# NVlabs/WarpConvNet

Measured on AMD Instinct MI355X. Metric: M active voxels/sec fwd+bwd, SparseConv3d 64→128 k=3, 1/2/4/8 MI355X, higher is better.
Workload: dtype bf16; 1 GPU; configs[1]: one 1000000-voxel uniform (U) scene per GPU, SparseConv3d 64->128 k=3, bf16 autocast, kernel-map build + AB fwd + ABt dgrad + AtB wgrad per step; voxels_per_gpu=1000000, coord_order=generator, parallelism=dp1 (scene-sharded, grad all-reduce)

## Files before the change

### include/wcn.h

```cpp
#ifndef WCN_H_
#define WCN_H_

#include <stddef.h>
#include <stdint.h>

#ifdef __cplusplus
extern "C" {
#endif

typedef void* wcn_stream_t;

enum wcn_status {
  WCN_SUCCESS = 0,
  WCN_ERROR_PROBLEM_NOT_SUPPORTED = -1,
  WCN_ERROR_KERNEL_INITIALIZATION = -2,
  WCN_ERROR_KERNEL_EXECUTION = -3,
  WCN_ERROR_UNSUPPORTED_CONFIG = -4,
  WCN_ERROR_INVALID_PARAMETERS = -5,
  WCN_ERROR_MIXED_INPUT_UNSUPPORTED = -6
};

enum wcn_dtype { WCN_F32 = 0, WCN_F16 = 1, WCN_BF16 = 2 };

enum wcn_kmap_flag {
  WCN_FLAG_TABLE_FULL = 1,
  WCN_FLAG_COORD_RANGE = 2,
  WCN_FLAG_PAIR_OVERFLOW = 4,
  WCN_FLAG_DUPLICATE_COORD = 8,
  WCN_FLAG_NEED_STRICT = 16,
  WCN_FLAG_ROW_OVERFLOW = 32
};

int wcn_abi_version(void);
const char* wcn_status_string(int status);

int wcn_hash_prepare(void* slots, int64_t capacity, wcn_stream_t stream);
int wcn_hash_insert(void* slots, int64_t capacity, const int32_t* coords, int64_t n, int32_t* status,
                    wcn_stream_t stream);
int wcn_hash_search(const void* slots, int64_t capacity, const int32_t* queries, int64_t m,
                    int32_t* results, wcn_stream_t stream);

int32_t wcn_kmap_row_pitch(int32_t num_offsets);
int32_t wcn_kmap_mask_words(int32_t num_offsets);
int64_t wcn_kmap_num_blocks(int64_t m);
size_t wcn_kmap_counts_bytes(int64_t m, int32_t num_offsets);

int wcn_kmap_probe(const void* slots, int64_t capacity, const int32_t* query, int64_t m,
                   const int32_t ksize[3], const int32_t stride[3], const int32_t dilation[3],
                   int32_t* nbr, uint32_t* mask, wcn_stream_t stream);
int wcn_batch_indexed_coords(const int32_t* coords, int64_t n, int32_t num_dims, const int32_t* offsets,
                             int32_t num_batches, int32_t* out, wcn_stream_t stream);

int wcn_morton_code(const int32_t* coords, int64_t n, int32_t num_dims, const int32_t* origin, const int32_t axis[3],
                    int64_t* codes, wcn_stream_t stream);

size_t wcn_kmap_binned_workspace(int64_t n, int64_t max_blocks);
int wcn_kmap_binned_supported(const int32_t ksize[3], const int32_t dilation[3]);
int wcn_kmap_compact_supported(int32_t num_offsets);
int wcn_kmap_build_binned(const int32_t* coords, int64_t n, const int32_t ksize[3], const int32_t dilation[3],
                          int64_t max_blocks, int32_t strict, int32_t compact, void* workspace, size_t workspace_bytes,
                          int32_t* nbr, uint32_t* mask, int32_t* status, wcn_stream_t stream);
int wcn_kmap_densify(const int32_t* nbr_compact, int64_t m, int32_t num_offsets, int32_t* nbr, wcn_stream_t stream);
size_t wcn_kmap_tally_sort_workspace(int64_t m);
int wcn_kmap_tally_sort(uint32_t* mask, int32_t* nbr, int64_t m, int32_t num_offsets, int32_t* counts, int32_t* offsets,
                        int32_t* status, int32_t* host_mirror, int32_t* perm, void* sort_workspace,
                        size_t sort_workspace_bytes, const int32_t* coords, void* binned_workspace, int64_t binned_n,
                        int64_t max_blocks, int32_t compact, int32_t* in_maps, int32_t* out_maps, int64_t pair_capacity,
                        wcn_stream_t stream);
int wcn_kmap_count(const uint32_t* mask, int64_t m, int32_t num_offsets, int32_t* counts, wcn_stream_t stream);
int wcn_kmap_scan(int32_t* counts, int64_t num_blocks, int32_t num_offsets, int32_t* offsets,
                  wcn_stream_t stream);
int wcn_kmap_scan_to_host(int32_t* counts, int64_t num_blocks, int32_t num_offsets, int32_t* offsets, const int32_t* status,
                          int32_t* host_mirror, wcn_stream_t stream);
int wcn_kmap_scatter(const int32_t* nbr, const uint32_t* mask, int64_t m, int32_t num_offsets,
                     const int32_t* counts, const int32_t* offsets, int32_t* in_maps, int32_t* out_maps, int64_t pair_capacity,
                     int32_t* status, int32_t compact, wcn_stream_t stream);
int wcn_kmap_cells_build(const int32_t* coords, int64_t n, int64_t max_blocks, void* workspace, size_t workspace_bytes,
                         uint32_t* scratch, int32_t* status, wcn_stream_t stream);
int wcn_cells_stride_supported(const int32_t stride[3]);
int64_t wcn_cells_stride_tiles(int64_t n);
int wcn_cells_stride_count(const void* cells_workspace, int64_t n, int64_t max_blocks, const int32_t* coords,
                           const int32_t stride[3], uint64_t* flags, int32_t* counts, int32_t num_batches,
                           int32_t* out_offsets, wcn_stream_t stream);
int wcn_cells_stride_emit(const void* cells_workspace, int64_t n, int64_t max_blocks, const int32_t* coords,
                          const int32_t stride[3], const uint64_t* flags, const int32_t* counts, int32_t* out_coords,
                          int32_t* first_rows, int32_t* nbr, uint32_t* mask, wcn_stream_t stream);
int wcn_kmap_probe_cells(const void* cells_workspace, int64_t n_in, int64_t max_blocks, const int32_t* query, int64_t m,
                         const int32_t ksize[3], const int32_t stride[3], const int32_t dilation[3], int32_t* nbr,
                         uint32_t* mask, wcn_stream_t stream);
int wcn_kmap_transpose(const int32_t* nbr, int64_t m, int32_t num_offsets, int32_t* pair_table,
                       wcn_stream_t stream);
int wcn_kmap_reverse(const int32_t* in_maps, const int32_t* out_maps, const int32_t* offsets,
                     int32_t num_offsets, int64_t max_pairs, int64_t n_in, int32_t* rev_nbr,
                     uint32_t* rev_mask, wcn_stream_t stream);
int wcn_kmap_from_csr(const int32_t* in_maps, const int32_t* out_maps, const int32_t* offsets,
                      int32_t num_offsets, int64_t max_pairs, int64_t n_out, int32_t* nbr, uint32_t* mask,
                      wcn_stream_t stream);
size_t wcn_mask_argsort_workspace(int64_t n);
int wcn_mask_argsort(const uint32_t* mask, int32_t mask_words, int32_t num_bits, int64_t n, int32_t* perm,
                     void* workspace, size_t workspace_bytes, wcn_stream_t stream);
int wcn_mask_tile_order(const uint32_t* mask, int32_t mask_words, int32_t num_offsets, int64_t n, int32_t* perm,
                        void* workspace, size_t workspace_bytes, wcn_stream_t stream);

enum wcn_algo { WCN_ALGO_AUTO = 0, WCN_ALGO_REF = 1, WCN_ALGO_MFMA = 2 };

int wcn_mfma_gather_supported(int32_t cin, int32_t cout, int32_t num_offsets, int32_t dtype);
int wcn_mfma_wgrad_supported(int32_t cin, int32_t cout, int32_t dtype);
int wcn_conv_identity_supported(int32_t cin, int32_t cout, int32_t dtype);
int wcn_dense_rows_supported(int32_t cin, int32_t cout, int32_t dtype);
int wcn_dense_rows(const void* x, int32_t x_is_f32, const void* w, int32_t w_is_f32, int32_t w_transposed, const float* bias,
                   void* y, int64_t n, int32_t cin, int32_t cout, int32_t dtype, wcn_stream_t stream);

size_t wcn_packed_weight_bytes(int32_t num_offsets, int32_t cin, int32_t cout, int32_t dtype, int32_t transpose);
int wcn_pack_weight(const void* w, int32_t num_offsets, int32_t cin, int32_t cout, int32_t dtype,
                    int32_t transpose, int32_t flip, void* packed, size_t packed_bytes, wcn_stream_t stream);
int wcn_pack_weight_f32(const float* w, int32_t num_offsets, int32_t cin, int32_t cout, int32_t dtype, int32_t transpose,
                        int32_t flip, void* packed, size_t packed_bytes, wcn_stream_t stream);
int wcn_pack_weight_pair_supported(int32_t num_offsets, int32_t cin, int32_t cout, int32_t dtype);
int wcn_pack_weight_f32_pair(const float* w, int32_t num_offsets, int32_t cin, int32_t cout, int32_t dtype, int32_t flip_dgrad,
                             void* packed_fwd, size_t packed_fwd_bytes, void* packed_dgrad, size_t packed_dgrad_bytes,
                             wcn_stream_t stream);

int wcn_conv_compact_table_supported(int32_t cin, int32_t cout, int32_t num_offsets, int32_t dtype);
int wcn_conv_gather_gemm(const void* in, const void* w, void* out, const int32_t* nbr,
                         const uint32_t* mask, const int32_t* perm, const float* bias, int64_t n_in,
                         int64_t n_out, int32_t cin, int32_t cout, int32_t num_offsets, int32_t dtype,
                         int32_t algo, int32_t w_transposed, int32_t k_flip, wcn_stream_t stream);

int wcn_mfma_grouped_supported(int32_t cin_g, int32_t cout_g, int32_t num_offsets, int32_t dtype);
int wcn_pack_weight_grouped(const void* w, int32_t w_is_f32, int32_t num_offsets, int32_t groups, int32_t cin_g,
                            int32_t cout_g, int32_t dtype, int32_t transpose, int32_t flip, void* packed, wcn_stream_t stream);
int wcn_conv_gather_gemm_grouped(const void* in, const void* w_packed, void* out, const int32_t* nbr, const uint32_t* mask,
                                 const int32_t* perm, const float* bias, int64_t n_in, int64_t n_out, int32_t cin_g,
                                 int32_t cout_g, int32_t groups, int32_t num_offsets, int32_t dtype, wcn_stream_t stream);
int wcn_conv_gather_gemm_f32out(const void* in, const void* w_packed, float* out, const int32_t* nbr,
                                const uint32_t* mask, const int32_t* perm, const float* bias, int64_t n_in,
                                int64_t n_out, int32_t cin, int32_t cout, int32_t num_offsets, int32_t dtype,
                                wcn_stream_t stream);

int wcn_conv_gather_gemm_fused(const void* in, const void* w_packed, void* out, const int32_t* nbr, const uint32_t* mask,
                               const int32_t* perm, const float* bias, const float* scale, const float* shift,
                               const void* residual, int32_t relu, int64_t n_in, int64_t n_out, int32_t cin, int32_t cout,
                               int32_t num_offsets, int32_t dtype, wcn_stream_t stream);

size_t wcn_colsum_workspace(int32_t channels);
int wcn_colsum(const void* in, int64_t n, int32_t channels, int32_t dtype, float* out, void* workspace,
               size_t workspace_bytes, wcn_stream_t stream);

size_t wcn_conv_wgrad_workspace(int32_t num_offsets, int32_t cin, int32_t cout, int32_t algo);
int wcn_conv_wgrad(const void* x, const void* dy, float* dw, const int32_t* in_maps,
                   const int32_t* out_maps, const int32_t* offsets, int64_t n_in, int64_t n_out,
                   int32_t cin, int32_t cout, int32_t num_offsets, int32_t dtype, int32_t algo,
                   void* workspace, size_t workspace_bytes, wcn_stream_t stream);

int wcn_mfma_wgrad_bias_supported(int32_t cin, int32_t cout, int32_t dtype);
int wcn_conv_wgrad_bias(const void* x, const void* dy, float* dw, const int32_t* in_maps, const int32_t* out_maps,
                        const int32_t* offsets, int64_t n_in, int64_t n_out, int32_t cin, int32_t cout,
                        int32_t num_offsets, int32_t dtype, int32_t self_offset, float* bias_grad, void* workspace,
                        size_t workspace_bytes, wcn_stream_t stream);

int wcn_dwconv_gather(const void* in, const void* w, void* out, const int32_t* nbr, const float* bias, int64_t n_in,
                      int64_t n_out, int32_t channels, int32_t num_offsets, int32_t dtype, int32_t k_flip,
                      wcn_stream_t stream);
size_t wcn_dwconv_wgrad_workspace(int32_t num_offsets, int32_t channels);
int wcn_dwconv_wgrad(const void* x, const void* dy, float* dw, const int32_t* in_maps, const int32_t* out_maps,
                     const int32_t* offsets, int64_t n_in, int64_t n_out, int32_t channels, int32_t num_offsets,
                     int32_t dtype, void* workspace, size_t workspace_bytes, wcn_stream_t stream);

int wcn_knn_grid(const float* ref_sorted, const int32_t* ref_ids, const int32_t* cell_start, const float origin[3],
                 float cell_size, const int32_t dims[3], const float* query, int64_t num_query, int32_t k,
                 int64_t* out_index, float* out_dist2, wcn_stream_t stream);
int wcn_radius_grid_count(const float* ref_sorted, const int32_t* ref_ids, const int32_t* cell_start, const float origin[3],
                          float cell_size, const int32_t dims[3], const float* query, int64_t num_query, float radius,
                          int32_t* counts, wcn_stream_t stream);
int wcn_radius_grid_write(const float* ref_sorted, const int32_t* ref_ids, const int32_t* cell_start, const float origin[3],
                          float cell_size, const int32_t dims[3], const float* query, int64_t num_query, float radius,
                          const int64_t* splits, int32_t* out_index, float* out_dist, wcn_stream_t stream);
int wcn_segment_reduce(const void* in, const int64_t* row_splits, int64_t num_segments, int32_t channels, int32_t dtype,
                       int32_t op, void* out, int64_t* arg_rows, wcn_stream_t stream);

int wcn_pointconv_supported(int32_t cin, int32_t cq, int32_t nrel, int32_t hidden, int32_t cout, int32_t k,
                            int32_t linear_shortcut);
int64_t wcn_pointconv_packed_floats(int32_t ein, int32_t hidden, int32_t cout);
int64_t wcn_pointconv_grad_floats(int32_t ein, int32_t hidden, int32_t cout, int32_t linear_shortcut);
size_t wcn_pointconv_backward_workspace(int64_t n_query, int32_t k, int32_t ein, int32_t hidden, int32_t cout,
                                        int32_t linear_shortcut);
int wcn_pointconv_pack(const float* w1, const float* b1, const float* g1, const float* be1, const float* w2,
                       const float* b2, const float* g2, const float* be2, const float* ws, const float* bs, int32_t ein,
                       int32_t hidden, int32_t cout, float* packed, wcn_stream_t stream);
int wcn_pointconv_edge_forward(const float* in_feats, const float* q_feats, const float* in_xyz, const float* q_xyz,
                               const int32_t* nbr, int64_t n_query, int32_t k, int32_t cin, int32_t cq, int32_t nrel,
                               const float* packed, int32_t hidden, int32_t cout, float eps1, float eps2, int32_t mean,
                               int32_t linear_shortcut, float* out, wcn_stream_t stream);
int wcn_pointconv_edge_backward(const float* in_feats, const float* q_feats, const float* in_xyz, const float* q_xyz,
                                const int32_t* nbr, int64_t n_query, int32_t k, int32_t cin, int32_t cq, int32_t nrel,
                                const float* packed, int32_t hidden, int32_t cout, float eps1, float eps2, int32_t mean,
                                int32_t linear_shortcut, const float* grad_out, float* d_in, float* d_q, float* d_params,
                                void* workspace, size_t workspace_bytes, wcn_stream_t stream);
int wcn_pointconv_edge_backward_peredge(const float* in_feats, const float* q_feats, const float* in_xyz, const float* q_xyz,
                                        const int32_t* nbr, int64_t n_query, int32_t k, int32_t cin, int32_t cq, int32_t nrel,
                                        const float* packed, int32_t hidden, int32_t cout, float eps1, float eps2, int32_t mean,
                                        int32_t linear_shortcut, const float* grad_out, float* d_edge, float* d_q,
                                        float* d_params, void* workspace, size_t workspace_bytes, wcn_stream_t stream);

int wcn_pointconv_edge_forward_ragged(const float* in_feats, const float* q_feats, const float* in_xyz, const float* q_xyz,
                                      const int32_t* nbr, const int32_t* edge_q, const float* q_scale, int64_t n_edges,
                                      int64_t n_query, int32_t cin, int32_t cq, int32_t nrel, const float* packed,
                                      int32_t hidden, int32_t cout, float eps1, float eps2, int32_t linear_shortcut,
                                      float* out, wcn_stream_t stream);
int wcn_pointconv_edge_backward_ragged(const float* in_feats, const float* q_feats, const float* in_xyz, const float* q_xyz,
                                       const int32_t* nbr, const int32_t* edge_q, const float* q_scale, int64_t n_edges,
                                       int64_t n_query, int32_t cin, int32_t cq, int32_t nrel, const float* packed,
                                       int32_t hidden, int32_t cout, float eps1, float eps2, int32_t linear_shortcut,
                                       const float* grad_out, float* d_in, float* d_q, float* d_params, void* workspace,
                                       size_t workspace_bytes, wcn_stream_t stream);

int wcn_pool_gather(const void* in, const int32_t* tbl, int64_t n_in, int64_t n_out, int32_t channels, int32_t num_offsets,
                    int32_t dtype, int32_t op, void* out, int32_t* arg, int32_t* count, wcn_stream_t stream);
int wcn_pool_gather_scaled(const void* in, const int32_t* tbl, const float* scale, int64_t n_in, int64_t n_out,
                           int32_t channels, int32_t num_offsets, int32_t dtype, int32_t op, void* out, int32_t* arg,
                           int32_t* count, wcn_stream_t stream);
int wcn_pool_row_vec(const void* src, const void* dst, int32_t channels, int32_t dtype);
int wcn_pool_select(const void* dy, const int32_t* arg, const int32_t* tbl, int64_t n_in, int64_t n_out, int32_t channels,
                    int32_t num_offsets, int32_t dtype, void* dx, wcn_stream_t stream);

size_t wcn_bn_workspace(int32_t channels);
int32_t wcn_bn_max_channels(void);
int wcn_bn_stats_fold(const void* x, int64_t n, int32_t channels, int32_t dtype, const float* gamma, const float* beta,
                      float* running_mean, float* running_var, float momentum, float eps, float* mean, float* var,
                      float* rstd, float* scale, float* shift, int64_t* num_batches_tracked, void* workspace,
                      size_t workspace_bytes, wcn_stream_t stream);
int wcn_bn_fold(const float* running_mean, const float* running_var, const float* gamma, const float* beta, float eps,
                int32_t channels, float* mean, float* rstd, float* scale, float* shift, wcn_stream_t stream);
int wcn_bn_stats(const void* x, int64_t n, int32_t channels, int32_t dtype, float* mean, float* var, void* workspace,
                 size_t workspace_bytes, wcn_stream_t stream);
int wcn_bn_apply(const void* x, int64_t n, int32_t channels, int32_t dtype, const float* scale, const float* shift,
                 int32_t relu, void* y, wcn_stream_t stream);
int wcn_bn_backward_reduce(const void* dy, const void* x, const float* relu_scale, const float* relu_shift, int64_t n,
                           int32_t channels, int32_t dtype, const float* mean, const float* rstd, float* sum_dy,
                           float* sum_dy_xhat, void* workspace, size_t workspace_bytes, wcn_stream_t stream);
int wcn_bn_backward_apply(const void* dy, const void* x, const float* relu_scale, const float* relu_shift, int64_t n,
                          int32_t channels, int32_t dtype, const float* mean, const float* rstd, const float* gamma,
                          const float* sum_dy, const float* sum_dy_xhat, void* dx, wcn_stream_t stream);
int wcn_bn_apply_residual(const void* x, const void* residual, int64_t n, int32_t channels, int32_t dtype, const float* scale,
                          const float* shift, int32_t relu, void* y, wcn_stream_t stream);
int wcn_bn_backward_reduce_masked(const void* dy, const void* x, const void* z, int64_t n, int32_t channels, int32_t dtype,
                                  const float* mean, const float* rstd, float* sum_dy, float* sum_dy_xhat, void* workspace,
                                  size_t workspace_bytes, wcn_stream_t stream);
int wcn_bn_backward_apply_masked(const void* dy, const void* x, const void* z, int64_t n, int32_t channels, int32_t dtype,
                                 const float* mean, const float* rstd, const float* gamma, const float* sum_dy,
                                 const float* sum_dy_xhat, void* dx, void* dres, wcn_stream_t stream);

int wcn_bn_train_forward(const void* x, const void* residual, int64_t n, int32_t channels, int32_t dtype, const float* gamma,
                         const float* beta, float* running_mean, float* running_var, float momentum, float eps,
                         int64_t* num_batches_tracked, int32_t relu, float* stats, void* y, void* workspace,
                         size_t workspace_bytes, wcn_stream_t stream);
int wcn_bn_train_backward(const void* dy, const void* x, const void* z, int32_t relu, int64_t n, int32_t channels, int32_t dtype,
                          const float* stats, const float* gamma, int32_t training, float* sums, void* dx, void* dres,
                          void* workspace, size_t workspace_bytes, wcn_stream_t stream);
int wcn_bn_train_backward_ld(const void* dy, int64_t dy_ld, const void* x, const void* z, int32_t relu, int64_t n, int32_t channels,
                             int32_t dtype, const float* stats, const float* gamma, int32_t training, float* sums, void* dx,
                             void* dres, void* workspace, size_t workspace_bytes, wcn_stream_t stream);

int wcn_conv_bn_backward(const void* grad_out, const void* x, const void* y, const void* z, int32_t relu, const float* stats,
                         const float* gamma, int32_t training, float* sums, void* dy_conv, void* dres, const void* w_packed_dgrad,
                         const int32_t* rev_nbr, const uint32_t* rev_mask, const int32_t* rev_perm, int32_t flip, void* dx,
                         const int32_t* in_maps, const int32_t* out_maps, const int32_t* offsets, float* dw, void* wgrad_workspace,
                         size_t wgrad_workspace_bytes, int64_t n_in, int64_t n_out, int32_t cin, int32_t cout, int32_t num_offsets,
                         int32_t dtype, void* bn_workspace, size_t bn_workspace_bytes, wcn_stream_t stream);
int wcn_conv_bn_backward_ld(const void* grad_out, int64_t grad_out_ld, const void* x, const void* y, const void* z, int32_t relu,
                            const float* stats, const float* gamma, int32_t training, float* sums, void* dy_conv, void* dres,
                            const void* w_packed_dgrad, const int32_t* rev_nbr, const uint32_t* rev_mask, const int32_t* rev_perm,
                            int32_t flip, void* dx, const int32_t* in_maps, const int32_t* out_maps, const int32_t* offsets,
                            float* dw, void* wgrad_workspace, size_t wgrad_workspace_bytes, int64_t n_in, int64_t n_out,
                            int32_t cin, int32_t cout, int32_t num_offsets, int32_t dtype, void* bn_workspace,
                            size_t bn_workspace_bytes, wcn_stream_t stream);

int wcn_attn_varlen_supported(int32_t head_dim, int32_t dtype);
size_t wcn_attn_varlen_workspace_bytes(int64_t total, int32_t heads);
int wcn_attn_varlen_fwd(const void* qkv, const int32_t* cu_seqlens, int64_t num_seqs, int64_t total, int32_t heads,
                        int32_t head_dim, int32_t max_seqlen, float softmax_scale, int32_t dtype, void* out, float* lse,
                        wcn_stream_t stream);
int wcn_attn_varlen_bwd(const void* dout, const void* qkv, const void* out, const float* lse, const int32_t* cu_seqlens,
                        int64_t num_seqs, int64_t total, int32_t heads, int32_t head_dim, int32_t max_seqlen,
                        float softmax_scale, int32_t dtype, void* dqkv, void* workspace, size_t workspace_bytes,
                        wcn_stream_t stream);

int32_t wcn_attn_varlen_kv_splits(int64_t num_seqs, int32_t max_seqlen_q, int32_t max_seqlen_k, int32_t heads);
size_t wcn_attn_varlen_kv_workspace_bytes(int64_t total_q, int64_t total_k, int32_t heads, int32_t head_dim, int32_t q_splits);
int wcn_attn_varlen_kv_fwd(const void* q, int64_t q_stride, const void* k, const void* v, int64_t kv_stride,
                           const int32_t* cu_q, const int32_t* cu_k, int64_t num_seqs, int64_t total_q, int64_t total_k,
                           int32_t heads, int32_t head_dim, int32_t max_seqlen_q, int32_t max_seqlen_k, float softmax_scale,
                           int32_t dtype, void* out, float* lse, wcn_stream_t stream);
int wcn_attn_varlen_kv_bwd(const void* dout, const void* q, int64_t q_stride, const void* k, const void* v, int64_t kv_stride,
                           const void* out, const float* lse, const int32_t* cu_q, const int32_t* cu_k, int64_t num_seqs,
                           int64_t total_q, int64_t total_k, int32_t heads, int32_t head_dim, int32_t max_seqlen_q,
                           int32_t max_seqlen_k, float softmax_scale, int32_t dtype, void* dq, int64_t dq_stride, void* dk,
                           void* dv, int64_t dkv_stride, int32_t q_splits, void* workspace, size_t workspace_bytes,
                           wcn_stream_t stream);

enum wcn_slot_order { WCN_SLOT_X_FASTEST = 0, WCN_SLOT_Z_FASTEST = 1 };
int wcn_resample_pack(const void* src, const int32_t* tbl, int64_t n_src, int64_t n_parent, int32_t channels, int32_t n_per,
                      int32_t factor, int32_t pitch, int32_t slot_order, int32_t dtype, void* dst, wcn_stream_t stream);
int wcn_resample_unpack(const void* src, const int32_t* tbl, int64_t n_parent, int64_t n_dst, int32_t channels, int32_t n_per,
                        int32_t factor, int32_t pitch, int32_t slot_order, int32_t broadcast, int32_t dtype, void* dst,
                        wcn_stream_t stream);
size_t wcn_resample_expand_workspace(int64_t n_parent);
int wcn_resample_expand(const int32_t* parents, const void* mask, int32_t mask_dtype, int64_t n_parent, int32_t n_per,
                        int32_t factor, int32_t slot_order, int32_t num_batches, void* workspace, size_t workspace_bytes,
                        int32_t* out_offsets, int64_t capacity, int32_t* child_coords, int32_t* tbl, int32_t pitch,
                        wcn_stream_t stream);

int wcn_rope_table(const void* coords, int32_t coords_float, int64_t total, const float* origin, float bias,
                   const float* freqs, int32_t num_freqs, float* table, wcn_stream_t stream);
int wcn_qk_prologue_supported(int32_t head_dim, int32_t in_dtype, int32_t out_dtype);
size_t wcn_qk_prologue_workspace_bytes(int64_t total, int32_t heads, int32_t head_dim);
int wcn_qk_prologue_fwd(const void* qkv, int32_t in_dtype, int64_t total, int32_t heads, int32_t head_dim, const float* table,
                        int32_t rot_pairs, int32_t conjugate, const float* gamma_q, const float* gamma_k, void* out,
                        int32_t out_dtype, float* inv_norm, wcn_stream_t stream);
int wcn_qk_prologue_bwd(const void* dout, int32_t dout_dtype, const void* qkv, int32_t in_dtype, int64_t total, int32_t heads,
                        int32_t head_dim, const float* table, int32_t rot_pairs, const float* gamma_q, const float* gamma_k,
                        const float* inv_norm, void* dqkv, float* dgamma_q, float* dgamma_k, void* workspace,
                        size_t workspace_bytes, wcn_stream_t stream);

int wcn_adaln_supported(int32_t channels, int32_t dtype);
size_t wcn_adaln_workspace_bytes(int64_t rows, int64_t num_segs, int32_t channels);
int wcn_adaln_fwd(const void* x, const void* h, const float* gate, const float* shift, const float* scale, int64_t mod_ld,
                  const int32_t* cu, int64_t num_segs, int64_t rows, int32_t channels, float eps, int32_t dtype, void* x1,
                  void* y, float* stats, wcn_stream_t stream);
int wcn_adaln_bwd(const void* dx1, const void* dy, const void* x, const void* h, const float* gate, const float* scale,
                  int64_t mod_ld, const float* stats, const int32_t* cu, int64_t num_segs, int64_t rows, int32_t channels,
                  int32_t dtype, void* dx, void* dh, float* dgate, float* dshift, float* dscale, int64_t dmod_ld,
                  void* workspace, size_t workspace_bytes, wcn_stream_t stream);

int wcn_ln_act_supported(int32_t channels, int32_t dtype);
size_t wcn_ln_act_workspace_bytes(int64_t rows, int32_t channels);
int wcn_ln_act_fwd(const void* x, const float* weight, const float* bias, int64_t rows, int32_t channels, float eps,
                   int32_t act, int32_t dtype, void* y, float* stats, wcn_stream_t stream);
int wcn_ln_act_bwd(const void* dy, const void* x, const float* weight, const float* bias, const float* stats, int64_t rows,
                   int32_t channels, int32_t act, int32_t dtype, void* dx, float* dweight, float* dbias, void* workspace,
                   size_t workspace_bytes, wcn_stream_t stream);
int wcn_channel_spread(const void* x, const void* h, int64_t rows, int32_t cx, int32_t r, float alpha, int32_t dtype,
                       void* out, wcn_stream_t stream);
int wcn_channel_fold(const void* x, const void* h, int64_t rows, int32_t cout, int32_t g, float alpha, int32_t dtype,
                     void* out, wcn_stream_t stream);

int32_t wcn_window_group_max_segment(void);
size_t wcn_window_group_workspace_bytes(int64_t n, int64_t num_bins);
int wcn_window_group(const int32_t* coords, int64_t n, const int32_t* batch_offsets, int32_t num_batches,
                     const int32_t window[3], const int32_t shift[3], const int32_t min_coord[3], const int32_t grid_shape[3],
                     int64_t* codes, int64_t* perm, int64_t* inverse_perm, int32_t* cu_seqlens, int64_t* counts,
                     int32_t* summary, void* workspace, size_t workspace_bytes, wcn_stream_t stream);

int32_t wcn_csr_chunk_rows(void);
int wcn_voxel_keys(const float* points, int64_t n, const int32_t* batch_offsets, int32_t num_batches, float inv_voxel_size,
                   int64_t* keys, int32_t* status, wcn_stream_t stream);
size_t wcn_voxel_map_workspace_bytes(int64_t n);
int wcn_voxel_map(const int64_t* sorted_keys, const int64_t* perm, int64_t n, int32_t num_batches, int64_t* unique_keys,
                  int32_t* unique_coords, int64_t* csr_offsets, int64_t* to_orig, int64_t* to_unique,
// ... 171 lines not shown
```

### warpconvnet_amd/_lib.py

```python
import ctypes
import os
import subprocess
import threading
from ctypes import c_char_p, c_int, c_int32, c_int64, c_size_t, c_void_p
from typing import Optional

import torch

_CSRC = os.path.join(os.path.dirname(os.path.abspath(__file__)), "csrc")
LIB_PATH = os.environ.get("WARPCONVNET_AMD_LIB") or os.path.join(_CSRC, "libwcn_hip.so")

WCN_F32, WCN_F16, WCN_BF16 = 0, 1, 2
WCN_ALGO_AUTO, WCN_ALGO_REF, WCN_ALGO_MFMA = 0, 1, 2
WCN_FLAG_TABLE_FULL, WCN_FLAG_COORD_RANGE, WCN_FLAG_PAIR_OVERFLOW, WCN_FLAG_DUPLICATE_COORD = 1, 2, 4, 8
WCN_FLAG_NEED_STRICT = 16
WCN_FLAG_ROW_OVERFLOW = 32
WCN_SLOT_X_FASTEST, WCN_SLOT_Z_FASTEST = 0, 1
WCN_MASK_U8 = 3
WCN_GRID_KEY_CELL, WCN_GRID_KEY_CORNER = 0, 1
WCN_SEG_MOMENTS, WCN_SEG_RANGE, WCN_SEG_DOT = 0, 1, 2
WCN_SEG_ADD, WCN_SEG_SUB, WCN_SEG_MUL, WCN_SEG_DIV, WCN_SEG_NORM, WCN_SEG_NORM_BWD = 0, 1, 2, 3, 4, 5
WCN_FPS_AUTO, WCN_FPS_RESIDENT, WCN_FPS_STREAMED = 0, 1, 2
WCN_ATTN_AUTO, WCN_ATTN_ONE_WAVE, WCN_ATTN_SHARED = 0, 1, 2

_I32P = c_void_p
_3I = c_int32 * 3
_EC_LISTS = [c_void_p, c_int64, c_void_p, c_int64, c_void_p, c_void_p, c_int32, c_int64, c_int64, c_int64, c_int32]

SIGNATURES = {
    "wcn_abi_version": (c_int, []),
    "wcn_status_string": (c_char_p, [c_int]),
    "wcn_hash_prepare": (c_int, [c_void_p, c_int64, c_void_p]),
    "wcn_hash_insert": (c_int, [c_void_p, c_int64, c_void_p, c_int64, c_void_p, c_void_p]),
    "wcn_hash_search": (c_int, [c_void_p, c_int64, c_void_p, c_int64, c_void_p, c_void_p]),
    "wcn_kmap_row_pitch": (c_int32, [c_int32]),
    "wcn_kmap_mask_words": (c_int32, [c_int32]),
    "wcn_kmap_num_blocks": (c_int64, [c_int64]),
    "wcn_kmap_probe": (
        c_int,
        [c_void_p, c_int64, c_void_p, c_int64, _3I, _3I, _3I, c_void_p, c_void_p, c_void_p],
    ),
    "wcn_batch_indexed_coords": (c_int, [c_void_p, c_int64, c_int32, c_void_p, c_int32, c_void_p, c_void_p]),
    "wcn_bn_workspace": (c_size_t, [c_int32]),
    "wcn_bn_max_channels": (c_int32, []),
    "wcn_bn_stats": (c_int, [c_void_p, c_int64, c_int32, c_int32, c_void_p, c_void_p, c_void_p, c_size_t, c_void_p]),
    "wcn_bn_stats_fold": (c_int, [c_void_p, c_int64, c_int32, c_int32, c_void_p, c_void_p, c_void_p, c_void_p, ctypes.c_float,
                                  ctypes.c_float, c_void_p, c_void_p, c_void_p, c_void_p, c_void_p, c_void_p, c_void_p, c_size_t,
                                  c_void_p]),
    "wcn_bn_fold": (c_int, [c_void_p, c_void_p, c_void_p, c_void_p, ctypes.c_float, c_int32, c_void_p, c_void_p, c_void_p,
                            c_void_p, c_void_p]),
    "wcn_bn_apply": (c_int, [c_void_p, c_int64, c_int32, c_int32, c_void_p, c_void_p, c_int32, c_void_p, c_void_p]),
    "wcn_bn_backward_reduce": (c_int, [c_void_p, c_void_p, c_void_p, c_void_p, c_int64, c_int32, c_int32, c_void_p, c_void_p,
                                       c_void_p, c_void_p, c_void_p, c_size_t, c_void_p]),
    "wcn_bn_backward_apply": (c_int, [c_void_p, c_void_p, c_void_p, c_void_p, c_int64, c_int32, c_int32, c_void_p, c_void_p,
                                      c_void_p, c_void_p, c_void_p, c_void_p, c_void_p]),
    "wcn_bn_apply_residual": (c_int, [c_void_p, c_void_p, c_int64, c_int32, c_int32, c_void_p, c_void_p, c_int32, c_void_p,
                                      c_void_p]),
    "wcn_bn_backward_reduce_masked": (c_int, [c_void_p, c_void_p, c_void_p, c_int64, c_int32, c_int32, c_void_p, c_void_p,
                                              c_void_p, c_void_p, c_void_p, c_size_t, c_void_p]),
    "wcn_bn_backward_apply_masked": (c_int, [c_void_p, c_void_p, c_void_p, c_int64, c_int32, c_int32, c_void_p, c_void_p,
                                             c_void_p, c_void_p, c_void_p, c_void_p, c_void_p, c_void_p]),
    "wcn_bn_train_forward": (c_int, [c_void_p, c_void_p, c_int64, c_int32, c_int32, c_void_p, c_void_p, c_void_p, c_void_p,
                                     ctypes.c_float, ctypes.c_float, c_void_p, c_int32, c_void_p, c_void_p, c_void_p, c_size_t,
                                     c_void_p]),
    "wcn_bn_train_backward": (c_int, [c_void_p, c_void_p, c_void_p, c_int32, c_int64, c_int32, c_int32, c_void_p, c_void_p,
                                      c_int32, c_void_p, c_void_p, c_void_p, c_void_p, c_size_t, c_void_p]),
    "wcn_bn_train_backward_ld": (c_int, [c_void_p, c_int64, c_void_p, c_void_p, c_int32, c_int64, c_int32, c_int32, c_void_p, c_void_p,
                                         c_int32, c_void_p, c_void_p, c_void_p, c_void_p, c_size_t, c_void_p]),
    "wcn_conv_bn_backward_ld": (c_int, [c_void_p, c_int64, c_void_p, c_void_p, c_void_p, c_int32, c_void_p, c_void_p, c_int32, c_void_p,
                                        c_void_p, c_void_p, c_void_p, c_void_p, c_void_p, c_void_p, c_int32, c_void_p, c_void_p, c_void_p,
                                        c_void_p, c_void_p, c_void_p, c_size_t, c_int64, c_int64, c_int32, c_int32, c_int32, c_int32,
                                        c_void_p, c_size_t, c_void_p]),
    "wcn_conv_bn_backward": (c_int, [c_void_p, c_void_p, c_void_p, c_void_p, c_int32, c_void_p, c_void_p, c_int32, c_void_p, c_void_p,
                                     c_void_p, c_void_p, c_void_p, c_void_p, c_void_p, c_int32, c_void_p, c_void_p, c_void_p, c_void_p,
                                     c_void_p, c_void_p, c_size_t, c_int64, c_int64, c_int32, c_int32, c_int32, c_int32, c_void_p,
                                     c_size_t, c_void_p]),
    "wcn_pool_gather": (c_int, [c_void_p, c_void_p, c_int64, c_int64, c_int32, c_int32, c_int32, c_int32, c_void_p, c_void_p,
                                c_void_p, c_void_p]),
    "wcn_pool_gather_scaled": (c_int, [c_void_p, c_void_p, c_void_p, c_int64, c_int64, c_int32, c_int32, c_int32, c_int32, c_void_p,
                                       c_void_p, c_void_p, c_void_p]),
    "wcn_pool_row_vec": (c_int, [c_void_p, c_void_p, c_int32, c_int32]),
    "wcn_pool_select": (c_int, [c_void_p, c_void_p, c_void_p, c_int64, c_int64, c_int32, c_int32, c_int32, c_void_p, c_void_p]),
    "wcn_morton_code": (c_int, [c_void_p, c_int64, c_int32, c_void_p, c_void_p, c_void_p, c_void_p]),
    "wcn_kmap_counts_bytes": (c_size_t, [c_int64, c_int32]),
    "wcn_kmap_binned_workspace": (c_size_t, [c_int64, c_int64]),
    "wcn_kmap_binned_supported": (c_int, [_3I, _3I]),
    "wcn_kmap_build_binned": (
        c_int,
        [c_void_p, c_int64, _3I, _3I, c_int64, c_int32, c_int32, c_void_p, c_size_t, c_void_p, c_void_p, c_void_p, c_void_p],
    ),
    "wcn_kmap_compact_supported": (c_int, [c_int32]),
    "wcn_kmap_densify": (c_int, [c_void_p, c_int64, c_int32, c_void_p, c_void_p]),
    "wcn_kmap_tally_sort_workspace": (c_size_t, [c_int64]),
    "wcn_kmap_tally_sort": (
        c_int,
        [c_void_p, c_void_p, c_int64, c_int32, c_void_p, c_void_p, c_void_p, c_void_p, c_void_p, c_void_p, c_size_t,
         c_void_p, c_void_p, c_int64, c_int64, c_int32, c_void_p, c_void_p, c_int64, c_void_p],
    ),
    "wcn_kmap_count": (c_int, [c_void_p, c_int64, c_int32, c_void_p, c_void_p]),
    "wcn_kmap_scan": (c_int, [c_void_p, c_int64, c_int32, c_void_p, c_void_p]),
    "wcn_kmap_scan_to_host": (c_int, [c_void_p, c_int64, c_int32, c_void_p, c_void_p, c_void_p, c_void_p]),
    "wcn_kmap_scatter": (
        c_int,
        [c_void_p, c_void_p, c_int64, c_int32, c_void_p, c_void_p, c_void_p, c_void_p, c_int64, c_void_p, c_int32, c_void_p],
    ),
    "wcn_kmap_cells_build": (c_int, [c_void_p, c_int64, c_int64, c_void_p, c_size_t, c_void_p, c_void_p, c_void_p]),
    "wcn_cells_stride_supported": (c_int, [_3I]),
    "wcn_cells_stride_tiles": (c_int64, [c_int64]),
    "wcn_cells_stride_count": (c_int, [c_void_p, c_int64, c_int64, c_void_p, _3I, c_void_p, c_void_p, c_int32, c_void_p,
                                       c_void_p]),
    "wcn_cells_stride_emit": (c_int, [c_void_p, c_int64, c_int64, c_void_p, _3I, c_void_p, c_void_p, c_void_p, c_void_p,
                                      c_void_p, c_void_p, c_void_p]),
    "wcn_kmap_probe_cells": (c_int, [c_void_p, c_int64, c_int64, c_void_p, c_int64, _3I, _3I, _3I, c_void_p, c_void_p,
                                     c_void_p]),
    "wcn_kmap_transpose": (c_int, [c_void_p, c_int64, c_int32, c_void_p, c_void_p]),
    "wcn_kmap_reverse": (
        c_int,
        [c_void_p, c_void_p, c_void_p, c_int32, c_int64, c_int64, c_void_p, c_void_p, c_void_p],
    ),
    "wcn_kmap_from_csr": (
        c_int,
        [c_void_p, c_void_p, c_void_p, c_int32, c_int64, c_int64, c_void_p, c_void_p, c_void_p],
    ),
    "wcn_mask_argsort_workspace": (c_size_t, [c_int64]),
    "wcn_mask_argsort": (c_int, [c_void_p, c_int32, c_int32, c_int64, c_void_p, c_void_p, c_size_t, c_void_p]),
    "wcn_mask_tile_order": (c_int, [c_void_p, c_int32, c_int32, c_int64, c_void_p, c_void_p, c_size_t, c_void_p]),
    "wcn_mfma_gather_supported": (c_int, [c_int32, c_int32, c_int32, c_int32]),
    "wcn_mfma_wgrad_supported": (c_int, [c_int32, c_int32, c_int32]),
    "wcn_conv_identity_supported": (c_int, [c_int32, c_int32, c_int32]),
    "wcn_dense_rows_supported": (c_int, [c_int32, c_int32, c_int32]),
    "wcn_dense_rows": (
        c_int,
        [c_void_p, c_int32, c_void_p, c_int32, c_int32, c_void_p, c_void_p, c_int64, c_int32, c_int32, c_int32, c_void_p],
    ),
    "wcn_packed_weight_bytes": (c_size_t, [c_int32, c_int32, c_int32, c_int32, c_int32]),
    "wcn_pack_weight": (
        c_int,
        [c_void_p, c_int32, c_int32, c_int32, c_int32, c_int32, c_int32, c_void_p, c_size_t, c_void_p],
    ),
    "wcn_pack_weight_f32": (
        c_int,
        [c_void_p, c_int32, c_int32, c_int32, c_int32, c_int32, c_int32, c_void_p, c_size_t, c_void_p],
    ),
    "wcn_pack_weight_pair_supported": (c_int, [c_int32, c_int32, c_int32, c_int32]),
    "wcn_conv_compact_table_supported": (c_int, [c_int32, c_int32, c_int32, c_int32]),
    "wcn_pack_weight_f32_pair": (c_int, [c_void_p, c_int32, c_int32, c_int32, c_int32, c_int32, c_void_p, c_size_t, c_void_p, c_size_t,
                                         c_void_p]),
    "wcn_conv_gather_gemm": (
        c_int,
        [c_void_p, c_void_p, c_void_p, c_void_p, c_void_p, c_void_p, c_void_p, c_int64, c_int64, c_int32, c_int32,
         c_int32, c_int32, c_int32, c_int32, c_int32, c_void_p],
    ),
    "wcn_mfma_grouped_supported": (c_int, [c_int32, c_int32, c_int32, c_int32]),
    "wcn_pack_weight_grouped": (
        c_int,
        [c_void_p, c_int32, c_int32, c_int32, c_int32, c_int32, c_int32, c_int32, c_int32, c_void_p, c_void_p],
    ),
    "wcn_conv_gather_gemm_grouped": (
        c_int,
        [c_void_p, c_void_p, c_void_p, c_void_p, c_void_p, c_void_p, c_void_p, c_int64, c_int64, c_int32, c_int32,
         c_int32, c_int32, c_int32, c_void_p],
    ),
    "wcn_conv_gather_gemm_f32out": (
        c_int,
        [c_void_p, c_void_p, c_void_p, c_void_p, c_void_p, c_void_p, c_void_p, c_int64, c_int64, c_int32, c_int32,
         c_int32, c_int32, c_void_p],
    ),
# ... 102 lines not shown
    ),
    "wcn_attn_varlen_kv_bwd_v": (
        c_int,
        [c_void_p, c_void_p, c_int64, c_void_p, c_void_p, c_int64, c_void_p, c_void_p, c_void_p, c_void_p, c_int64, c_int64,
         c_int64, c_int32, c_int32, c_int32, c_int32, ctypes.c_float, c_int32, c_void_p, c_int64, c_void_p, c_void_p, c_int64,
         c_int32, c_void_p, c_size_t, c_int32, c_void_p],
    ),
    "wcn_attn_varlen_k_splits": (c_int32, [c_int64, c_int32, c_int32, c_int32, c_int32]),
    "wcn_attn_varlen_ksplit_workspace_bytes": (c_size_t, [c_int64, c_int64, c_int32, c_int32, c_int32, c_int32, c_int32]),
    "wcn_attn_varlen_kv_fwd_s": (
        c_int,
        [c_void_p, c_int64, c_void_p, c_void_p, c_int64, c_void_p, c_void_p, c_int64, c_int64, c_int64, c_int32, c_int32,
         c_int32, c_int32, ctypes.c_float, c_int32, c_void_p, c_void_p, c_int32, c_int32, c_void_p, c_size_t, c_void_p],
    ),
    "wcn_attn_varlen_kv_bwd_s": (
        c_int,
        [c_void_p, c_void_p, c_int64, c_void_p, c_void_p, c_int64, c_void_p, c_void_p, c_void_p, c_void_p, c_int64, c_int64,
         c_int64, c_int32, c_int32, c_int32, c_int32, ctypes.c_float, c_int32, c_void_p, c_int64, c_void_p, c_void_p, c_int64,
         c_int32, c_int32, c_void_p, c_size_t, c_int32, c_void_p],
    ),
    "wcn_rope_table": (c_int, [c_void_p, c_int32, c_int64, c_void_p, ctypes.c_float, c_void_p, c_int32, c_void_p, c_void_p]),
    "wcn_rope_table_axes": (c_int, [c_void_p, c_int32, c_int64, c_void_p, ctypes.c_float, c_void_p, _3I, c_void_p, c_void_p]),
    "wcn_qk_prologue_supported": (c_int, [c_int32, c_int32, c_int32]),
    "wcn_qk_prologue_workspace_bytes": (c_size_t, [c_int64, c_int32, c_int32]),
    "wcn_qk_prologue_fwd": (
        c_int,
        [c_void_p, c_int32, c_int64, c_int32, c_int32, c_void_p, c_int32, c_int32, c_void_p, c_void_p, c_void_p, c_int32,
         c_void_p, c_void_p],
    ),
    "wcn_qk_prologue_bwd": (
        c_int,
        [c_void_p, c_int32, c_void_p, c_int32, c_int64, c_int32, c_int32, c_void_p, c_int32, c_void_p, c_void_p, c_void_p,
         c_void_p, c_void_p, c_void_p, c_void_p, c_size_t, c_void_p],
    ),
    "wcn_adaln_supported": (c_int, [c_int32, c_int32]),
    "wcn_adaln_workspace_bytes": (c_size_t, [c_int64, c_int64, c_int32]),
    "wcn_adaln_fwd": (
        c_int,
        [c_void_p] * 5 + [c_int64, c_void_p, c_int64, c_int64, c_int32, ctypes.c_float, c_int32, c_void_p, c_void_p, c_void_p,
                          c_void_p],
    ),
    "wcn_adaln_bwd": (
        c_int,
        [c_void_p] * 6 + [c_int64, c_void_p, c_void_p, c_int64, c_int64, c_int32, c_int32] + [c_void_p] * 5 +
        [c_int64, c_void_p, c_size_t, c_void_p],
    ),
    "wcn_ln_act_supported": (c_int, [c_int32, c_int32]),
    "wcn_ln_act_workspace_bytes": (c_size_t, [c_int64, c_int32]),
    "wcn_ln_act_fwd": (c_int, [c_void_p] * 3 + [c_int64, c_int32, ctypes.c_float, c_int32, c_int32, c_void_p, c_void_p,
                                                 c_void_p]),
    "wcn_ln_act_bwd": (c_int, [c_void_p] * 5 + [c_int64, c_int32, c_int32, c_int32] + [c_void_p] * 4 + [c_size_t, c_void_p]),
    "wcn_channel_spread": (c_int, [c_void_p, c_void_p, c_int64, c_int32, c_int32, ctypes.c_float, c_int32, c_void_p,
                                   c_void_p]),
    "wcn_channel_fold": (c_int, [c_void_p, c_void_p, c_int64, c_int32, c_int32, ctypes.c_float, c_int32, c_void_p, c_void_p]),
    "wcn_window_group_max_segment": (c_int32, []),
    "wcn_window_group_workspace_bytes": (c_size_t, [c_int64, c_int64]),
    "wcn_window_group": (c_int, [c_void_p, c_int64, c_void_p, c_int32, _3I, _3I, _3I, _3I] + [c_void_p] * 7 +
                         [c_size_t, c_void_p]),
    "wcn_csr_chunk_rows": (c_int32, []),
    "wcn_voxel_keys": (c_int, [c_void_p, c_int64, c_void_p, c_int32, ctypes.c_float, c_void_p, c_void_p, c_void_p]),
    "wcn_voxel_map_workspace_bytes": (c_size_t, [c_int64]),
    "wcn_voxel_map": (c_int, [c_void_p, c_void_p, c_int64, c_int32] + [c_void_p] * 7 + [c_void_p, c_size_t, c_void_p]),
    "wcn_csr_gather_reduce_workspace_bytes": (c_size_t, [c_int64, c_int32, c_int32]),
    "wcn_csr_gather_reduce": (
        c_int,
        [c_void_p, c_int64, c_int64, c_void_p, c_void_p, c_int64, c_int64, c_int32, c_int32, c_int32, c_int64, c_void_p,
         c_void_p, c_void_p, c_size_t, c_void_p],
    ),
    "wcn_row_spread": (c_int, [c_void_p, c_void_p, c_int64, c_int64, c_int32, c_void_p, c_int32, c_int64, c_int32, c_void_p,
                               c_void_p, c_int32, c_void_p, c_void_p]),
    "wcn_resample_pack": (c_int, [c_void_p, c_void_p, c_int64, c_int64, c_int32, c_int32, c_int32, c_int32, c_int32, c_int32,
                                  c_void_p, c_void_p]),
    "wcn_resample_unpack": (c_int, [c_void_p, c_void_p, c_int64, c_int64, c_int32, c_int32, c_int32, c_int32, c_int32, c_int32,
                                    c_int32, c_void_p, c_void_p]),
    "wcn_resample_expand_workspace": (c_size_t, [c_int64]),
    "wcn_resample_expand": (c_int, [c_void_p, c_void_p, c_int32, c_int64, c_int32, c_int32, c_int32, c_int32, c_void_p, c_size_t,
                                    c_void_p, c_int64, c_void_p, c_void_p, c_int32, c_void_p]),
    "wcn_mfma_wgrad_bias_supported": (c_int, [c_int32, c_int32, c_int32]),
    "wcn_conv_wgrad_bias": (
        c_int,
        [c_void_p, c_void_p, c_void_p, c_void_p, c_void_p, c_void_p, c_int64, c_int64, c_int32, c_int32, c_int32,
         c_int32, c_int32, c_void_p, c_void_p, c_size_t, c_void_p],
    ),
    "wcn_lattice_chunk_rows": (c_int32, []),
    "wcn_hash128_insert": (c_int, [c_void_p, c_void_p, c_int64, c_void_p, c_int64, c_int32, c_void_p, c_void_p]),
    "wcn_hash128_search": (c_int, [c_void_p, c_void_p, c_int64, c_void_p, c_void_p, c_int64, c_int32, c_int32, c_void_p,
                                   c_void_p]),
    "wcn_permuto_simplex": (c_int, [c_void_p, c_int64, c_int32, ctypes.c_float * 6] + [c_void_p] * 6),
    "wcn_grid_corners": (c_int, [c_void_p, c_int64, c_int32] + [c_void_p] * 7),
    "wcn_lattice_map_workspace_bytes": (c_size_t, [c_int64]),
    "wcn_lattice_map": (c_int, [c_void_p, c_void_p, c_void_p, c_int64, c_int32] + [c_void_p] * 5 + [c_size_t, c_void_p]),
    "wcn_lattice_plan_items": (c_int64, [c_int64]),
    "wcn_lattice_plan_ints": (c_int64, [c_int64]),
    "wcn_lattice_plan": (c_int, [c_void_p, c_int64, c_int64, c_void_p, c_void_p]),
    "wcn_lattice_splat": (c_int, [c_void_p] * 4 + [c_int64, c_int64, c_int32, c_int32, ctypes.c_float] + [c_void_p] * 4),
    "wcn_lattice_blur": (c_int, [c_void_p] * 3 + [ctypes.c_float] * 3 + [c_int64, c_int32, c_void_p, c_void_p]),
    "wcn_lattice_slice": (c_int, [c_void_p] * 3 + [c_int64, c_int32, c_int64, c_int32, ctypes.c_float, c_void_p, c_void_p]),
    "wcn_lattice_max_grid": (c_int32, []),
    "wcn_lattice_row_grid": (c_int32, [c_int64, c_int32]),
    "wcn_bilateral_matvec": (c_int, [c_void_p, c_int32, c_int64, c_int32] + [ctypes.c_float] * 3 + [c_void_p, c_void_p,
                                                                                                   ctypes.c_float] + [c_void_p] * 5),
    "wcn_bilateral_pcg": (c_int, [c_void_p, c_int32, c_int64, c_int32] + [ctypes.c_float] * 3 + [c_void_p] * 3 + [ctypes.c_float] +
                          [c_void_p] * 5 + [c_int32, ctypes.c_double, c_void_p]),
    "wcn_bilateral_knn_weights": (c_int, [c_void_p] * 5 + [c_int64, c_int64, c_int32, c_int32, c_int32, ctypes.c_float,
                                                           ctypes.c_float, c_void_p, c_void_p]),
    "wcn_grid_max_grid": (c_int32, []),
    "wcn_grid_chunk_points": (c_int32, []),
    "wcn_grid_point_keys": (c_int, [c_void_p, c_int64, c_void_p, c_int32, _3I, ctypes.c_float * 3, ctypes.c_float * 3, c_int32,
                                    c_void_p, c_void_p, c_void_p]),
    "wcn_grid_sample": (c_int, [c_void_p, c_int64 * 5, _3I, c_int32, c_int32, c_int64, c_void_p, c_void_p, c_void_p, c_int64,
                                c_void_p, c_int64, c_int64, c_void_p]),
    "wcn_grid_sample_backward_workspace_bytes": (c_size_t, [c_int64, c_int32]),
    "wcn_grid_sample_backward": (c_int, [c_void_p, c_int64, c_int64, c_int64 * 5, _3I, c_int32, c_int32, c_int64, c_void_p,
                                         c_void_p, c_void_p, c_void_p, c_int64, c_int64, c_void_p, c_void_p, c_size_t,
                                         c_void_p]),
    "wcn_seg_chunk_rows": (c_int32, []),
    "wcn_seg_max_grid": (c_int32, []),
    "wcn_seg_stats_workspace_bytes": (c_size_t, [c_int64, c_int64, c_int32, c_int32]),
    "wcn_seg_stats": (c_int, [c_int32] + [c_void_p] * 4 + [c_int64, c_int64, c_int32, c_int32] + [c_void_p] * 5 +
                      [c_size_t, c_void_p]),
    "wcn_seg_apply": (c_int, [c_int32] + [c_void_p] * 3 + [c_int32] + [c_void_p] * 7 + [c_int64, c_int64, c_int32, c_int32,
                                                                                       c_void_p, c_void_p]),
    "wcn_fps_resident_max_points": (c_int64, []),
    "wcn_fps_block_threads": (c_int32, []),
    "wcn_fps_blocks_per_segment": (c_int32, []),
    "wcn_fps_max_grid": (c_int32, []),
    "wcn_fps_workspace_bytes": (c_size_t, [c_int64, c_int64, c_int32]),
    "wcn_fps": (c_int, [c_void_p, c_void_p, c_int64, c_void_p, c_int64, c_int64, c_int32, c_int64, c_void_p, c_int32, c_void_p,
                        c_size_t, c_void_p, c_void_p]),
    "wcn_fdg_supported": (c_int, [c_int32, c_int32]),
    "wcn_fdg_workspace": (c_size_t, [c_int64]),
    "wcn_fdg_count": (c_int, [c_void_p, c_int32, c_void_p, c_int64, c_void_p, c_int32, c_void_p, c_size_t, c_void_p, c_void_p]),
    "wcn_fdg_emit": (c_int, [c_void_p, c_int32, c_void_p, c_void_p, c_int64, c_void_p, c_int32, c_void_p, c_int32, c_void_p,
                             c_int32, ctypes.c_float, ctypes.c_float * 3, c_void_p, c_size_t, c_int64, c_void_p, c_void_p,
                             c_void_p, c_void_p]),
    "wcn_pad_max_grid": (c_int32, []),
    "wcn_pad_block_threads": (c_int32, []),
    "wcn_pad_repack": (c_int, [c_void_p, c_void_p, c_void_p, c_int64, c_void_p, c_int64, c_int64, c_void_p, c_int64, c_int64,
                               c_int64, c_int32, ctypes.c_uint64, c_void_p]),
    "wcn_seg_bmm_max_channels": (c_int32, []),
    "wcn_seg_bmm_tile_rows": (c_int32, []),
    "wcn_seg_bmm_chunk_rows": (c_int32, []),
    "wcn_seg_bmm_workspace_bytes": (c_size_t, [c_int64, c_int64, c_int32, c_int32, c_int32]),
    "wcn_seg_bmm": (c_int, [c_void_p, c_void_p, c_void_p, c_int64, c_int64, c_int32, c_int32, c_int32, c_int32, c_void_p,
                            c_void_p, c_size_t, c_void_p]),
    "wcn_seg_bmm_wgrad": (c_int, [c_void_p, c_void_p, c_void_p, c_int64, c_int64, c_int32, c_int32, c_int32, c_void_p,
                                  c_void_p, c_size_t, c_void_p]),
    "wcn_edgeconv_max_channels": (c_int32, []),
    "wcn_edgeconv_sum_blocks": (c_int32, []),
    "wcn_edgeconv_arg_bytes": (c_int32, [c_int64]),
    "wcn_edgeconv_sums_workspace_bytes": (c_size_t, [c_int32]),
    "wcn_edgeconv_backward_input_workspace_bytes": (c_size_t, [c_int64, c_int32]),
    "wcn_edgeconv_stats": (c_int, _EC_LISTS + [c_void_p, c_void_p, c_void_p, c_size_t, c_void_p]),
    "wcn_edgeconv_forward": (c_int, _EC_LISTS + [c_void_p, c_void_p, ctypes.c_float, c_void_p, c_void_p, c_int32, c_void_p]),
    "wcn_edgeconv_backward_sums": (c_int, _EC_LISTS + [c_void_p] * 4 + [ctypes.c_float, c_void_p, c_void_p, c_int32, c_void_p,
                                                                        c_void_p, c_void_p, c_size_t, c_void_p]),
    "wcn_edgeconv_backward_query": (c_int, _EC_LISTS + [c_void_p] * 6 + [ctypes.c_float, c_void_p, c_void_p, c_int32, c_void_p,
                                                                         c_void_p]),
    "wcn_edgeconv_backward_input": (c_int, _EC_LISTS + [c_void_p] * 3 + [c_void_p] * 6 +
                                    [ctypes.c_float, c_void_p, c_void_p, c_int32, c_void_p, c_void_p, c_size_t, c_void_p]),
}

_LIB = None


class _GuardedLib:

    def __init__(self, handle: ctypes.CDLL):
        self._h = handle

    def __getattr__(self, name):
        fn = getattr(self._h, name)
        argtypes = fn.argtypes or []
        if not argtypes or argtypes[-1] is not c_void_p or name in _HOST_ONLY or _single_gpu():
            setattr(self, name, fn)
            return fn

        def guarded(*args, _fn=fn):
            dev = getattr(_CALL_DEVICE, "dev", None)
            if dev is None or dev == torch.cuda.current_device():
                return _fn(*args)
            with torch.cuda.device(dev):
                return _fn(*args)

        guarded.__name__ = name
        setattr(self, name, guarded)
        return guarded


def _single_gpu() -> bool:
    try:
        return torch.cuda.is_available() and torch.cuda.device_count() == 1
    except Exception:
        return False


_HOST_ONLY = {"wcn_status_string"}
_CALL_DEVICE = threading.local()


def build(verbose: bool = False) -> str:
    cmd = ["make", "-C", _CSRC, "-j", str(min(8, os.cpu_count() or 1))]
    res = subprocess.run(cmd, capture_output=True, text=True)
    if res.returncode != 0:
        raise RuntimeError(f"building libwcn_hip.so failed:\n{res.stdout[-4000:]}\n{res.stderr[-4000:]}")
    if verbose:
        print(res.stdout[-2000:])
    return LIB_PATH


def lib() -> ctypes.CDLL:
    global _LIB
    if _LIB is None:
        if not os.path.exists(LIB_PATH):
            raise RuntimeError(
                f"{LIB_PATH} not found: the HIP extension is not built. Run "
                "`python -c 'import __graft_entry__ as g; g.build()'` (or `make -C warpconvnet_amd/csrc`). "
                "There is no CPU fallback for the HIP paths."
            )
        handle = ctypes.CDLL(LIB_PATH)
        for name, (restype, argtypes) in SIGNATURES.items():
            fn = getattr(handle, name)
            fn.restype = restype
            fn.argtypes = argtypes
        _LIB = _GuardedLib(handle)
    return _LIB


def status_string(code: int) -> str:
    return lib().wcn_status_string(int(code)).decode()


def check(code: int, what: str) -> None:
    if code != 0:
        raise RuntimeError(f"{what} error: {status_string(code)} ({code})")


def ptr(t: Optional[torch.Tensor]) -> Optional[int]:
    if t is None:
        return None
    return t.data_ptr()


_RAW_STREAM = getattr(torch._C, "_cuda_getCurrentRawStream", None)


def stream_handle(device: torch.device) -> int:
    idx = device.index
    if idx is None:
        idx = torch.cuda.current_device()
    _CALL_DEVICE.dev = idx
    if _RAW_STREAM is not None:
        return _RAW_STREAM(idx)
    return torch.cuda.current_stream(device).cuda_stream


def dtype_code(dtype: torch.dtype) -> int:
    if dtype == torch.float32:
        return WCN_F32
    if dtype == torch.float16:
        return WCN_F16
    if dtype == torch.bfloat16:
        return WCN_BF16
    raise TypeError(f"unsupported feature dtype {dtype} (supported: float32, float16, bfloat16)")


def torch_dtype(code: int) -> torch.dtype:
    return {WCN_F32: torch.float32, WCN_F16: torch.float16, WCN_BF16: torch.bfloat16}[code]


def i3(v) -> "ctypes.Array":
    return _3I(int(v[0]), int(v[1]), int(v[2]))


def require_gpu_tensor(t: torch.Tensor, name: str) -> None:
    if not t.is_cuda:
        raise RuntimeError(f"{name} must live on a GPU for the HIP path (got {t.device}); there is no CPU fallback")
    if not t.is_contiguous():
        raise RuntimeError(f"{name} must be contiguous")
```

### warpconvnet_amd/csrc/conv_api.hip

```cpp
#include "gather_gemm.h"

namespace wcn {
int conv_gather_gemm_ref(const void* in, const void* w, void* out, const int32_t* nbr, const float* bias, int64_t n_out,
                         int cin, int cout, int K, int dtype, int w_transposed, int k_flip, hipStream_t s);
size_t colsum_workspace(int c);
int colsum(const void* in, int64_t n, int c, int dtype, float* out, void* workspace, size_t workspace_bytes, hipStream_t s);
int conv_wgrad_ref(const void* x, const void* dy, float* dw, const int32_t* in_maps, const int32_t* out_maps,
                   const int32_t* offsets, int cin, int cout, int K, int dtype, hipStream_t s);
bool mfma_wgrad_supported(int cin, int cout, int dtype);
size_t wgrad_mfma_workspace(int K, int cin, int cout);
bool mfma_wgrad_bias_supported(int cin, int cout, int dtype);
int conv_wgrad_mfma(const void* x, const void* dy, float* dw, const int32_t* in_maps, const int32_t* out_maps,
                    const int32_t* offsets, int cin, int cout, int K, int dtype, void* workspace, size_t workspace_bytes,
                    int cs_k, float* bias_grad, int64_t pair_bound, hipStream_t s);
int dwconv_gather(const void* in, const void* w, void* out, const int32_t* tbl, const float* bias, int64_t n_out, int C,
                  int K, int dtype, int k_flip, hipStream_t s);
size_t dwconv_wgrad_workspace(int K, int C);
int dwconv_wgrad(const void* x, const void* dy, float* dw, const int32_t* in_maps, const int32_t* out_maps,
                 const int32_t* offsets, int C, int K, int dtype, void* workspace, size_t workspace_bytes, hipStream_t s);
int knn_grid(const float* ref, const int32_t* ref_id, const int32_t* cell_start, const float origin[3], float h,
             const int32_t dims[3], const float* query, int64_t m, int k, int64_t* out_idx, float* out_d2, hipStream_t s);
int radius_grid_count(const float* ref, const int32_t* ref_id, const int32_t* cell_start, const float origin[3], float h,
                      const int32_t dims[3], const float* query, int64_t m, float radius, int32_t* counts, hipStream_t s);
int radius_grid_write(const float* ref, const int32_t* ref_id, const int32_t* cell_start, const float origin[3], float h,
                      const int32_t dims[3], const float* query, int64_t m, float radius, const int64_t* splits,
                      int32_t* out_idx, float* out_dist, hipStream_t s);
int segment_reduce(const void* in, const int64_t* splits, int64_t m, int c, int dtype, int op, void* out, int64_t* arg,
                   hipStream_t s);
}

using namespace wcn;

static inline size_t dtype_size(int dtype) { return dtype == WCN_F32 ? 4 : 2; }

extern "C" {

int wcn_mfma_gather_supported(int32_t cin, int32_t cout, int32_t num_offsets, int32_t dtype) {
  return mfma_gather_supported(cin, cout, num_offsets, dtype) ? 1 : 0;
}
int wcn_conv_identity_supported(int32_t cin, int32_t cout, int32_t dtype) {
  return gather_gemm_cs_supported(cin, cout, 1, dtype) ? 1 : 0;
}
int wcn_mfma_wgrad_supported(int32_t cin, int32_t cout, int32_t dtype) {
  return mfma_wgrad_supported(cin, cout, dtype) ? 1 : 0;
}

size_t wcn_packed_weight_bytes(int32_t num_offsets, int32_t cin, int32_t cout, int32_t dtype, int32_t transpose) {
  (void)transpose;
  if (num_offsets < 1 || cin < 1 || cout < 1 || !dtype_ok(dtype)) return 0;
  return (size_t)num_offsets * ((cin + 63) / 64 * 64) * cout * dtype_size(dtype);
}

int wcn_pack_weight(const void* w, int32_t num_offsets, int32_t cin, int32_t cout, int32_t dtype, int32_t transpose,
                    int32_t flip, void* packed, size_t packed_bytes, wcn_stream_t stream) {
  if (!w || !packed || num_offsets < 1 || cin < 1 || cout < 1) return WCN_ERROR_INVALID_PARAMETERS;
  if (packed_bytes < wcn_packed_weight_bytes(num_offsets, cin, cout, dtype, transpose)) return WCN_ERROR_INVALID_PARAMETERS;
  return pack_weight_mfma(w, 0, num_offsets, cin, cout, dtype, transpose, flip, packed, (hipStream_t)stream);
}

int wcn_pack_weight_f32(const float* w, int32_t num_offsets, int32_t cin, int32_t cout, int32_t dtype, int32_t transpose,
                        int32_t flip, void* packed, size_t packed_bytes, wcn_stream_t stream) {
  if (!w || !packed || num_offsets < 1 || cin < 1 || cout < 1) return WCN_ERROR_INVALID_PARAMETERS;
  if (packed_bytes < wcn_packed_weight_bytes(num_offsets, cin, cout, dtype, transpose)) return WCN_ERROR_INVALID_PARAMETERS;
  return pack_weight_mfma(w, 1, num_offsets, cin, cout, dtype, transpose, flip, packed, (hipStream_t)stream);
}

static bool compact_table_ok(int cin, int cout, int K, int dtype) {
  return wcn_kmap_compact_supported(K) && gather_gemm_cs_supported(cin, cout, K, dtype);
}
int wcn_conv_compact_table_supported(int32_t cin, int32_t cout, int32_t num_offsets, int32_t dtype) {
  return compact_table_ok(cin, cout, num_offsets, dtype) ? 1 : 0;
}

int wcn_pack_weight_pair_supported(int32_t num_offsets, int32_t cin, int32_t cout, int32_t dtype) {
  return (gather_gemm_cs_supported(cin, cout, num_offsets, dtype) && gather_gemm_cs_supported(cout, cin, num_offsets, dtype)) ? 1 : 0;
}

int wcn_pack_weight_f32_pair(const float* w, int32_t num_offsets, int32_t cin, int32_t cout, int32_t dtype, int32_t flip_dgrad,
                             void* packed_fwd, size_t packed_fwd_bytes, void* packed_dgrad, size_t packed_dgrad_bytes,
                             wcn_stream_t stream) {
  if (!w || !packed_fwd || !packed_dgrad || num_offsets < 1 || cin < 1 || cout < 1) return WCN_ERROR_INVALID_PARAMETERS;
  if (!wcn_pack_weight_pair_supported(num_offsets, cin, cout, dtype)) return WCN_ERROR_UNSUPPORTED_CONFIG;
  if (packed_fwd_bytes < wcn_packed_weight_bytes(num_offsets, cin, cout, dtype, 0) ||
      packed_dgrad_bytes < wcn_packed_weight_bytes(num_offsets, cout, cin, dtype, 1))
    return WCN_ERROR_INVALID_PARAMETERS;
  return pack_weight_cs_pair(w, num_offsets, cin, cout, dtype, flip_dgrad, packed_fwd, packed_dgrad, (hipStream_t)stream);
}

int wcn_conv_gather_gemm(const void* in, const void* w, void* out, const int32_t* nbr, const uint32_t* mask,
                         const int32_t* perm, const float* bias, int64_t n_in, int64_t n_out, int32_t cin,
                         int32_t cout, int32_t num_offsets, int32_t dtype, int32_t algo, int32_t w_transposed,
                         int32_t k_flip, wcn_stream_t stream) {
  if (n_in < 0 || n_out < 0 || cin < 1 || cout < 1 || num_offsets < 1 || !dtype_ok(dtype))
    return WCN_ERROR_INVALID_PARAMETERS;
  if (n_out == 0) return WCN_SUCCESS;
  const bool identity = !nbr && !mask && !perm && num_offsets == 1 && algo == WCN_ALGO_MFMA && n_in == n_out &&
                        gather_gemm_cs_supported(cin, cout, 1, dtype);
// ... 12 lines not shown
    default:
      return WCN_ERROR_INVALID_PARAMETERS;
  }
}

int wcn_mfma_grouped_supported(int32_t cin_g, int32_t cout_g, int32_t num_offsets, int32_t dtype) {
  return mfma_grouped_supported(cin_g, cout_g, num_offsets, dtype) ? 1 : 0;
}

int wcn_pack_weight_grouped(const void* w, int32_t w_is_f32, int32_t num_offsets, int32_t groups, int32_t cin_g,
                            int32_t cout_g, int32_t dtype, int32_t transpose, int32_t flip, void* packed, wcn_stream_t stream) {
  if (!w || !packed || num_offsets < 1 || groups < 1 || cin_g < 1 || cout_g < 1) return WCN_ERROR_INVALID_PARAMETERS;
  return pack_weight_grouped(w, w_is_f32, num_offsets, groups, cin_g, cout_g, dtype, transpose, flip, packed,
                             (hipStream_t)stream);
}

int wcn_conv_gather_gemm_grouped(const void* in, const void* w_packed, void* out, const int32_t* nbr, const uint32_t* mask,
                                 const int32_t* perm, const float* bias, int64_t n_in, int64_t n_out, int32_t cin_g,
                                 int32_t cout_g, int32_t groups, int32_t num_offsets, int32_t dtype, wcn_stream_t stream) {
  if (n_in < 0 || n_out < 0 || cin_g < 1 || cout_g < 1 || groups < 1 || num_offsets < 1) return WCN_ERROR_INVALID_PARAMETERS;
  if (n_out == 0) return WCN_SUCCESS;
  if (!w_packed || !out || !nbr || !mask || (n_in > 0 && !in)) return WCN_ERROR_INVALID_PARAMETERS;
  ConvEpilogue epi;
  epi.bias = bias;
  return conv_gather_gemm_grouped(in, w_packed, out, nbr, mask, perm, epi, n_out, cin_g, cout_g, groups, num_offsets, dtype,
                                  (hipStream_t)stream);
}

int wcn_conv_gather_gemm_f32out(const void* in, const void* w, float* out, const int32_t* nbr, const uint32_t* mask,
                                const int32_t* perm, const float* bias, int64_t n_in, int64_t n_out, int32_t cin,
                                int32_t cout, int32_t num_offsets, int32_t dtype, wcn_stream_t stream) {
  if (n_in < 0 || n_out < 0 || cin < 1 || cout < 1 || num_offsets < 1 || (dtype != WCN_F16 && dtype != WCN_BF16))
    return WCN_ERROR_INVALID_PARAMETERS;
  if (n_out == 0) return WCN_SUCCESS;
  if (!w || !out || !nbr || (!mask && !compact_table_ok(cin, cout, num_offsets, dtype)) || (n_in > 0 && !in))
    return WCN_ERROR_INVALID_PARAMETERS;
  ConvEpilogue epi;
  epi.bias = bias;
  return conv_gather_gemm_mfma(in, w, nullptr, nbr, mask, perm, epi, n_out, cin, cout, num_offsets, dtype, out,
                               (hipStream_t)stream);
}

int wcn_conv_gather_gemm_fused(const void* in, const void* w_packed, void* out, const int32_t* nbr, const uint32_t* mask,
                               const int32_t* perm, const float* bias, const float* scale, const float* shift,
                               const void* residual, int32_t relu, int64_t n_in, int64_t n_out, int32_t cin, int32_t cout,
                               int32_t num_offsets, int32_t dtype, wcn_stream_t stream) {
  if (n_in < 0 || n_out < 0 || cin < 1 || cout < 1 || num_offsets < 1 || (dtype != WCN_F16 && dtype != WCN_BF16) ||
      ((scale == nullptr) != (shift == nullptr)))
    return WCN_ERROR_INVALID_PARAMETERS;
  if (n_out == 0) return WCN_SUCCESS;
  if (!w_packed || !out || !nbr || (!mask && !compact_table_ok(cin, cout, num_offsets, dtype)) || (n_in > 0 && !in) || residual == out)
    return WCN_ERROR_INVALID_PARAMETERS;
  ConvEpilogue epi;
  epi.bias = bias; epi.scale = scale; epi.shift = shift; epi.residual = residual; epi.relu = relu ? 1 : 0;
  return conv_gather_gemm_mfma(in, w_packed, out, nbr, mask, perm, epi, n_out, cin, cout, num_offsets, dtype, nullptr,
                               (hipStream_t)stream);
}

size_t wcn_colsum_workspace(int32_t channels) { return channels > 0 ? colsum_workspace(channels) : 0; }

int wcn_colsum(const void* in, int64_t n, int32_t channels, int32_t dtype, float* out, void* workspace,
               size_t workspace_bytes, wcn_stream_t stream) {
  if (n < 0 || channels < 1 || !dtype_ok(dtype) || !out) return WCN_ERROR_INVALID_PARAMETERS;
  if (n > 0 && !in) return WCN_ERROR_INVALID_PARAMETERS;
  return colsum(in, n, channels, dtype, out, workspace, workspace_bytes, (hipStream_t)stream);
}

size_t wcn_conv_wgrad_workspace(int32_t num_offsets, int32_t cin, int32_t cout, int32_t algo) {
  if (algo == WCN_ALGO_MFMA) return wgrad_mfma_workspace(num_offsets, cin, cout);
  return 256;
}

int wcn_conv_wgrad(const void* x, const void* dy, float* dw, const int32_t* in_maps, const int32_t* out_maps,
                   const int32_t* offsets, int64_t n_in, int64_t n_out, int32_t cin, int32_t cout, int32_t num_offsets,
                   int32_t dtype, int32_t algo, void* workspace, size_t workspace_bytes, wcn_stream_t stream) {
  if (n_in < 0 || n_out < 0 || cin < 1 || cout < 1 || num_offsets < 1 || !dtype_ok(dtype) || !dw || !offsets)
    return WCN_ERROR_INVALID_PARAMETERS;
  hipStream_t s = (hipStream_t)stream;
  switch (algo) {
    case WCN_ALGO_REF:
      return conv_wgrad_ref(x, dy, dw, in_maps, out_maps, offsets, cin, cout, num_offsets, dtype, s);
    case WCN_ALGO_MFMA:
      return conv_wgrad_mfma(x, dy, dw, in_maps, out_maps, offsets, cin, cout, num_offsets, dtype, workspace,
                             workspace_bytes, -1, nullptr, (int64_t)num_offsets * (n_in < n_out ? n_in : n_out), s);
    default:
      return WCN_ERROR_INVALID_PARAMETERS;
  }
}

int wcn_conv_bn_backward(const void* grad_out, const void* x, const void* y, const void* z, int32_t relu, const float* stats,
                         const float* gamma, int32_t training, float* sums, void* dy_conv, void* dres, const void* w_packed_dgrad,
                         const int32_t* rev_nbr, const uint32_t* rev_mask, const int32_t* rev_perm, int32_t flip, void* dx,
                         const int32_t* in_maps, const int32_t* out_maps, const int32_t* offsets, float* dw, void* wgrad_workspace,
                         size_t wgrad_workspace_bytes, int64_t n_in, int64_t n_out, int32_t cin, int32_t cout, int32_t num_offsets,
                         int32_t dtype, void* bn_workspace, size_t bn_workspace_bytes, wcn_stream_t stream) {
  return wcn_conv_bn_backward_ld(grad_out, 0, x, y, z, relu, stats, gamma, training, sums, dy_conv, dres, w_packed_dgrad, rev_nbr,
                                 rev_mask, rev_perm, flip, dx, in_maps, out_maps, offsets, dw, wgrad_workspace, wgrad_workspace_bytes,
                                 n_in, n_out, cin, cout, num_offsets, dtype, bn_workspace, bn_workspace_bytes, stream);
}

int wcn_conv_bn_backward_ld(const void* grad_out, int64_t grad_out_ld, const void* x, const void* y, const void* z, int32_t relu,
                            const float* stats, const float* gamma, int32_t training, float* sums, void* dy_conv, void* dres,
                            const void* w_packed_dgrad, const int32_t* rev_nbr, const uint32_t* rev_mask, const int32_t* rev_perm,
                            int32_t flip, void* dx, const int32_t* in_maps, const int32_t* out_maps, const int32_t* offsets,
                            float* dw, void* wgrad_workspace, size_t wgrad_workspace_bytes, int64_t n_in, int64_t n_out,
                            int32_t cin, int32_t cout, int32_t num_offsets, int32_t dtype, void* bn_workspace,
                            size_t bn_workspace_bytes, wcn_stream_t stream) {
  if (!dy_conv || (dtype != WCN_F16 && dtype != WCN_BF16)) return WCN_ERROR_INVALID_PARAMETERS;
  int rc = wcn_bn_train_backward_ld(grad_out, grad_out_ld, y, z, relu, n_out, cout, dtype, stats, gamma, training, sums, dy_conv, dres,
                                    bn_workspace, bn_workspace_bytes, stream);
  if (rc != WCN_SUCCESS) return rc;
  if (dx) {
    if (!w_packed_dgrad || !rev_nbr) return WCN_ERROR_INVALID_PARAMETERS;
    rc = wcn_conv_gather_gemm(dy_conv, w_packed_dgrad, dx, rev_nbr, rev_mask, rev_perm, nullptr, n_out, n_in, cout, cin, num_offsets,
                              dtype, WCN_ALGO_MFMA, 1, flip, stream);
    if (rc != WCN_SUCCESS) return rc;
  }
  if (dw)
    rc = wcn_conv_wgrad(x, dy_conv, dw, in_maps, out_maps, offsets, n_in, n_out, cin, cout, num_offsets, dtype, WCN_ALGO_MFMA,
                        wgrad_workspace, wgrad_workspace_bytes, stream);
  return rc;
}

int wcn_mfma_wgrad_bias_supported(int32_t cin, int32_t cout, int32_t dtype) {
  return mfma_wgrad_bias_supported(cin, cout, dtype) ? 1 : 0;
}

int wcn_conv_wgrad_bias(const void* x, const void* dy, float* dw, const int32_t* in_maps, const int32_t* out_maps,
                        const int32_t* offsets, int64_t n_in, int64_t n_out, int32_t cin, int32_t cout,
                        int32_t num_offsets, int32_t dtype, int32_t self_offset, float* bias_grad, void* workspace,
                        size_t workspace_bytes, wcn_stream_t stream) {
  if (n_in < 0 || n_out < 0 || cin < 1 || cout < 1 || num_offsets < 1 || !dtype_ok(dtype) || !dw || !offsets || !bias_grad)
    return WCN_ERROR_INVALID_PARAMETERS;
  if (self_offset < 0 || self_offset >= num_offsets) return WCN_ERROR_INVALID_PARAMETERS;
  return conv_wgrad_mfma(x, dy, dw, in_maps, out_maps, offsets, cin, cout, num_offsets, dtype, workspace, workspace_bytes,
                         self_offset, bias_grad, (int64_t)num_offsets * (n_in < n_out ? n_in : n_out), (hipStream_t)stream);
}

int wcn_dwconv_gather(const void* in, const void* w, void* out, const int32_t* nbr, const float* bias, int64_t n_in,
                      int64_t n_out, int32_t channels, int32_t num_offsets, int32_t dtype, int32_t k_flip,
                      wcn_stream_t stream) {
  if (n_in < 0 || n_out < 0 || channels < 1 || num_offsets < 1 || !dtype_ok(dtype)) return WCN_ERROR_INVALID_PARAMETERS;
  if (n_out == 0) return WCN_SUCCESS;
  if (!w || !out || !nbr || (n_in > 0 && !in)) return WCN_ERROR_INVALID_PARAMETERS;
  return dwconv_gather(in, w, out, nbr, bias, n_out, channels, num_offsets, dtype, k_flip, (hipStream_t)stream);
}

size_t wcn_dwconv_wgrad_workspace(int32_t num_offsets, int32_t channels) {
  return (num_offsets > 0 && channels > 0) ? dwconv_wgrad_workspace(num_offsets, channels) : 0;
}

int wcn_dwconv_wgrad(const void* x, const void* dy, float* dw, const int32_t* in_maps, const int32_t* out_maps,
                     const int32_t* offsets, int64_t n_in, int64_t n_out, int32_t channels, int32_t num_offsets,
                     int32_t dtype, void* workspace, size_t workspace_bytes, wcn_stream_t stream) {
  if (n_in < 0 || n_out < 0 || channels < 1 || num_offsets < 1 || !dtype_ok(dtype) || !dw || !offsets)
    return WCN_ERROR_INVALID_PARAMETERS;
  return dwconv_wgrad(x, dy, dw, in_maps, out_maps, offsets, channels, num_offsets, dtype, workspace, workspace_bytes,
                      (hipStream_t)stream);
}

int wcn_knn_grid(const float* ref_sorted, const int32_t* ref_ids, const int32_t* cell_start, const float origin[3],
                 float cell_size, const int32_t dims[3], const float* query, int64_t num_query, int32_t k,
                 int64_t* out_index, float* out_dist2, wcn_stream_t stream) {
  if (num_query < 0 || !origin || !dims) return WCN_ERROR_INVALID_PARAMETERS;
  if (num_query == 0) return WCN_SUCCESS;
  if (!ref_sorted || !ref_ids || !cell_start || !query || !out_index) return WCN_ERROR_INVALID_PARAMETERS;
  return knn_grid(ref_sorted, ref_ids, cell_start, origin, cell_size, dims, query, num_query, k, out_index, out_dist2,
                  (hipStream_t)stream);
}

int wcn_radius_grid_count(const float* ref_sorted, const int32_t* ref_ids, const int32_t* cell_start, const float origin[3],
                          float cell_size, const int32_t dims[3], const float* query, int64_t num_query, float radius,
                          int32_t* counts, wcn_stream_t stream) {
  if (num_query < 0 || !origin || !dims) return WCN_ERROR_INVALID_PARAMETERS;
  if (num_query == 0) return WCN_SUCCESS;
  if (!ref_sorted || !ref_ids || !cell_start || !query || !counts) return WCN_ERROR_INVALID_PARAMETERS;
  return radius_grid_count(ref_sorted, ref_ids, cell_start, origin, cell_size, dims, query, num_query, radius, counts,
                           (hipStream_t)stream);
}

int wcn_radius_grid_write(const float* ref_sorted, const int32_t* ref_ids, const int32_t* cell_start, const float origin[3],
                          float cell_size, const int32_t dims[3], const float* query, int64_t num_query, float radius,
                          const int64_t* splits, int32_t* out_index, float* out_dist, wcn_stream_t stream) {
  if (num_query < 0 || !origin || !dims) return WCN_ERROR_INVALID_PARAMETERS;
  if (num_query == 0) return WCN_SUCCESS;
  if (!ref_sorted || !ref_ids || !cell_start || !query || !splits || !out_index) return WCN_ERROR_INVALID_PARAMETERS;
  return radius_grid_write(ref_sorted, ref_ids, cell_start, origin, cell_size, dims, query, num_query, radius, splits,
                           out_index, out_dist, (hipStream_t)stream);
}

int wcn_segment_reduce(const void* in, const int64_t* row_splits, int64_t num_segments, int32_t channels, int32_t dtype,
                       int32_t op, void* out, int64_t* arg_rows, wcn_stream_t stream) {
  if (num_segments < 0 || channels < 0 || !dtype_ok(dtype)) return WCN_ERROR_INVALID_PARAMETERS;
  if (num_segments == 0 || channels == 0) return WCN_SUCCESS;
  if (!row_splits || !out) return WCN_ERROR_INVALID_PARAMETERS;
  return segment_reduce(in, row_splits, num_segments, channels, dtype, op, out, arg_rows, (hipStream_t)stream);
}

}
```

### warpconvnet_amd/csrc/kmap_bucket.hip

```cpp
#include "kmap_cells.h"
#include "mask_sort.h"

namespace wcn {

constexpr int kTileRows = 256;
constexpr int kBkThreads = 256;
constexpr int kTallyThreads = (kRsTile / kTileRows) * 64;
constexpr int kStageCap = 3072;

static_assert(kRsTile % kTileRows == 0, "a sort tile is a whole number of bucket tiles");
static_assert(kBkThreads == kRsThreads, "the scan launch runs rs_scan_body (mask_sort.h) in its digit workgroups");

__device__ __noinline__ void repair_row(int64_t row, const int4* __restrict__ coords, const CellTable& t, uint32_t cmask,
                                        int kp, int mw, int32_t* __restrict__ nbr, uint32_t* __restrict__ mask,
                                        int32_t* __restrict__ status) {
  const int4 c = coords[row];
  const int id = block_id_of(t.slots, cmask, c);
  const int w = id >= 0 ? t.cells[(int64_t)id * kCells + cell_of(c)] : -1;
  const bool compact = kp < 0;
  kp &= 0x7FFFFFFF;
  if (w >= 0 && w != row && !(mask[(int64_t)w * mw + (mw - 1)] & kMaskUnwritten)) {
    atomicOr(status, (int)(WCN_FLAG_DUPLICATE_COORD | (w > row ? WCN_FLAG_NEED_STRICT : 0)));
    for (int k = 0; k < kp; ++k) nbr[row * kp + k] = nbr[(int64_t)w * kp + k];
    for (int q = 0; q < mw; ++q) mask[row * mw + q] = mask[(int64_t)w * mw + q];
  } else {
    for (int k = 0; k < kp; ++k) nbr[row * kp + k] = compact ? 0 : -1;
    for (int q = 0; q < mw; ++q) mask[row * mw + q] = 0u;
  }
}

template <bool HIST, bool REPAIR>
__global__ __launch_bounds__(kTallyThreads) void kmap_tally_kernel(uint32_t* __restrict__ mask, int32_t* __restrict__ nbr,
                                                                int64_t m, int K, int kp, int mw, int64_t ntile,
                                                                int32_t* __restrict__ counts, int32_t* __restrict__ ticket,
                                                                int nblk_sort, int32_t* __restrict__ dcounts,
                                                                const int4* __restrict__ coords, CellTable t,
                                                                uint32_t cmask, int32_t* __restrict__ status, int kc,
                                                                int sort_shift, int sort_bits) {
  __shared__ int s_hist[kRsMaxBins];
  const int sort_bins = 1 << sort_bits;
  const int tid = threadIdx.x, lane = tid & 63, wave = tid >> 6;
  if (HIST) {
    for (int i = tid; i < sort_bins; i += kTallyThreads) s_hist[i] = 0;
    __syncthreads();
  }
  if (blockIdx.x == 0 && tid == 0) *ticket = 0;
  constexpr int kTilesPerBlock = kRsTile / kTileRows;
  for (int tt = 0; tt < 1; ++tt) {
    const int64_t tile = (int64_t)blockIdx.x * kTilesPerBlock + wave;
    if (tile >= ntile) break;
    const int64_t row0 = tile * kTileRows;
    uint32_t last[kTileRows / 64];
#pragma unroll
    for (int sb = 0; sb < kTileRows / 64; ++sb) {
      const int64_t row = row0 + sb * 64 + lane;
      last[sb] = row < m ? mask[row * mw + (mw - 1)] : 0u;
    }
    if (REPAIR) {
#pragma unroll
      for (int sb = 0; sb < kTileRows / 64; ++sb) {
        const int64_t row = row0 + sb * 64 + lane;
        if (last[sb] & kMaskUnwritten) {
          repair_row(row, coords, t, cmask, kp, mw, nbr, mask, status);
          last[sb] = mask[row * mw + (mw - 1)];
        }
      }
    }
    for (int w = 0; w < mw; ++w) {
      const int kend = (K - w * 32) < 32 ? (K - w * 32) : 32;
      int mine = 0;
#pragma unroll
      for (int sb = 0; sb < kTileRows / 64; ++sb) {
        const int64_t row = row0 + sb * 64 + lane;
        const uint32_t bits = (w == mw - 1) ? last[sb] : (row < m ? mask[row * mw + w] : 0u);
        if (HIST && w == 0 && row < m) atomicAdd(&s_hist[rs_digit(tile_key(bits, kc), sort_shift, sort_bits)], 1);
        for (int b = 0; b < kend; ++b) {
          const int c = __popcll(__ballot((bits >> b) & 1u));
          if (lane == b) mine += c;
        }
      }
      if (lane < kend) counts[(int64_t)(w * 32 + lane) * ntile + tile] = mine;
    }
  }
  if (HIST) {
    __syncthreads();
    if ((int)blockIdx.x < nblk_sort)
      for (int i = tid; i < sort_bins; i += kTallyThreads) dcounts[(int64_t)blockIdx.x * sort_bins + i] = s_hist[i];
  }
}

__global__ __launch_bounds__(kBkThreads) void kmap_scan_kernel(int32_t* __restrict__ counts, int64_t ntile, int K,
                                                               int32_t* __restrict__ totals, int32_t* __restrict__ ticket,
                                                               int32_t* __restrict__ offsets,
                                                               const int32_t* __restrict__ status,
                                                               int32_t* __restrict__ mirror, int32_t* __restrict__ dcounts,
                                                               int nblk_sort, int32_t* __restrict__ dtotals, int sort_bins) {
  __shared__ int s_wave[kBkThreads / 64];
  __shared__ int s_last;
  const int tid = threadIdx.x;
  if ((int)blockIdx.x >= K) {
    __shared__ int s_cols[kBkThreads];
    rs_scan_body(dcounts, dtotals, nblk_sort, sort_bins, (int)blockIdx.x - K, reinterpret_cast<char*>(s_cols));
    return;
  }
  const int total = scan_counts_in_place<kBkThreads, 16>(counts + (int64_t)blockIdx.x * ntile, ntile, s_wave);
  if (tid == 0) {
    __hip_atomic_store(&totals[blockIdx.x], total, __ATOMIC_RELAXED, __HIP_MEMORY_SCOPE_AGENT);
    __threadfence();
    s_last = (atomicAdd(ticket, 1) == K - 1);
  }
  __syncthreads();
  if (!s_last) return;
  __threadfence();
  int carry = 0;
  for (int base = 0; base < K; base += kBkThreads) {
    const int k = base + tid;
    const int v = k < K ? __hip_atomic_load(&totals[k], __ATOMIC_RELAXED, __HIP_MEMORY_SCOPE_AGENT) : 0;
    int trip;
    const int o = carry + block_excl_scan<kBkThreads>(v, s_wave, &trip) + v;
    if (k < K) {
      offsets[k + 1] = o;
      if (mirror) mirror[k + 1] = o;
    }
    carry += trip;
    __syncthreads();
  }
  if (tid == 0) {
    offsets[0] = 0;
    if (mirror) {
      mirror[0] = 0;
      mirror[K + 1] = status ? __hip_atomic_load(status, __ATOMIC_RELAXED, __HIP_MEMORY_SCOPE_AGENT) : 0;
      __threadfence_system();
      __hip_atomic_store(&mirror[K + 2], 1, __ATOMIC_RELEASE, __HIP_MEMORY_SCOPE_SYSTEM);
    }
  }
}

struct KsArgs {
  const int32_t* nbr;
  const uint32_t* mask;
  int64_t m;
  int K, kp, mw;
  int64_t ntile;
  const int32_t* counts;
  const int32_t* offsets;
  int32_t* in_maps;
  int32_t* out_maps;
  int64_t pair_capacity;
  int32_t* status;
  int compact;
};
static KsArgs ks_args(const int32_t* nbr, const uint32_t* mask, int64_t m, int32_t K, const int32_t* counts,
                      const int32_t* offsets, int32_t* in_maps, int32_t* out_maps, int64_t pair_capacity, int32_t* status,
                      int compact) {
  KsArgs q;
  q.compact = compact;
  q.nbr = nbr; q.mask = mask; q.m = m; q.K = K; q.kp = wcn_kmap_row_pitch(K); q.mw = wcn_kmap_mask_words(K);
  q.ntile = wcn_kmap_num_blocks(m); q.counts = counts; q.offsets = offsets; q.in_maps = in_maps; q.out_maps = out_maps;
  q.pair_capacity = pair_capacity; q.status = status;
  return q;
}

__device__ __forceinline__ void place_pair(int32_t* __restrict__ in_maps, int32_t* __restrict__ out_maps, int64_t pos,
                                           int64_t pair_capacity, int in_row, int out_row, bool& overflow) {
  if (pos < pair_capacity) {
    in_maps[pos] = in_row;
    out_maps[pos] = out_row;
  } else {
    overflow = true;
  }
}

constexpr size_t kKsLds = (size_t)2 * kStageCap * 4 + 32 * 8 + (size_t)(kBkThreads / 64) * 32 * 12 + 36 * 4 + kStageCap;

__device__ __forceinline__ void kmap_scatter_body(const KsArgs& q, int64_t tile_id, char* smem) {
  const int32_t* __restrict__ nbr = q.nbr;
  const uint32_t* __restrict__ mask = q.mask;
  const int64_t m = q.m, ntile = q.ntile, pair_capacity = q.pair_capacity;
  const int K = q.K, kp = q.kp, mw = q.mw;
  const int32_t* __restrict__ counts = q.counts;
  const int32_t* __restrict__ offsets = q.offsets;
  int32_t* __restrict__ in_maps = q.in_maps;
  int32_t* __restrict__ out_maps = q.out_maps;
  int32_t* s_in = reinterpret_cast<int32_t*>(smem);
  int32_t* s_out = s_in + kStageCap;
  int64_t* s_gbase = reinterpret_cast<int64_t*>(s_out + kStageCap);
  unsigned long long(*s_ball)[32] = reinterpret_cast<unsigned long long(*)[32]>(s_gbase + 32);
  int(*s_cnt)[32] = reinterpret_cast<int(*)[32]>(s_ball + kBkThreads / 64);
// ... 174 lines not shown
  const bool staged = total <= kStageCap;
  bool overflow = false;
  const int c = lane & 3;
#pragma unroll
  for (int j = 0; j < 4; ++j) {
    const int r = (lane >> 2) + 16 * j;
    uint32_t rem = s_rowmask[wave * 64 + r];
    for (int sk = 4 * c - 1; sk > 0; --sk) rem &= rem - 1u;
    const unsigned long long below = (1ull << r) - 1ull;
    const int vals[4] = {piece[j].x, piece[j].y, piece[j].z, piece[j].w};
#pragma unroll
    for (int t = 0; t < 4; ++t) {
      if (c == 0 && t == 0) continue;
      if (rem == 0u) break;
      const int b = __builtin_ctz(rem);
      rem &= rem - 1u;
      const uint4 slot = *reinterpret_cast<const uint4*>(&s_wb[wave][b]);
      const unsigned long long ball = ((unsigned long long)slot.y << 32) | slot.x;
      const int at = (int)slot.z + __popcll(ball & below);
      if (staged) {
        s_pair[at] = make_uint2((uint32_t)vals[t], (uint32_t)(((wave * 64 + r) << 8) | b));
      } else {
        place_pair(in_maps, out_maps, s_delta[b] + at, pair_capacity, vals[t], (int32_t)(row0 + r), overflow);
      }
    }
  }
  __syncthreads();
  if (staged) {
    for (int e = tid; e < total; e += kBkThreads) {
      const uint2 pr = s_pair[e];
      const int64_t pos = s_delta[pr.y & 31u] + e;
      if (pos < pair_capacity) {
        in_maps[pos] = (int32_t)pr.x;
        out_maps[pos] = (int32_t)(tile_row0 + (pr.y >> 8));
      } else {
        overflow = true;
      }
    }
  }
  if (overflow) atomicOr(q.status, (int)WCN_FLAG_PAIR_OVERFLOW);
}

__global__ __launch_bounds__(kBkThreads) void kmap_scatter_kernel(KsArgs q) {
  extern __shared__ char s_ks[];
  kmap_scatter_body(q, blockIdx.x, s_ks);
}

static void launch_scatter(const KsArgs& q, hipStream_t s) {
  const dim3 grid((unsigned)ceil_div(q.m, kTileRows)), block(kBkThreads);
  if (q.compact) hipLaunchKernelGGL(kmap_scatter_compact_kernel, grid, block, kKcLds, s, q);
  else hipLaunchKernelGGL(kmap_scatter_kernel, grid, block, kKsLds, s, q);
}

__global__ __launch_bounds__(256) void kmap_densify_kernel(const int32_t* __restrict__ nbrc, int64_t m, int kp,
                                                           int32_t* __restrict__ nbr) {
  const int cols4 = kp >> 2;
  const int64_t e = (int64_t)blockIdx.x * blockDim.x + threadIdx.x;
  if (e >= m * cols4) return;
  const int64_t row = e / cols4;
  const int c = (int)(e - row * cols4);
  const int32_t* src = nbrc + row * kCompactPitch;
  uint32_t bits = (uint32_t)src[0];
  if (__popc(bits) > kCompactIds) bits = 0u;
  int at = 1 + __popc(bits & ((1u << (4 * c)) - 1u));
  int v[4];
#pragma unroll
  for (int t = 0; t < 4; ++t) {
    const bool has = (bits >> (4 * c + t)) & 1u;
    v[t] = has ? src[at] : -1;
    at += has ? 1 : 0;
  }
  *reinterpret_cast<int4*>(nbr + row * kp + 4 * c) = make_int4(v[0], v[1], v[2], v[3]);
}

}

using namespace wcn;

extern "C" {

int64_t wcn_kmap_num_blocks(int64_t m) { return (ceil_div(m > 0 ? m : 0, kTileRows) + 3) & ~(int64_t)3; }

size_t wcn_kmap_counts_bytes(int64_t m, int32_t num_offsets) {
  return ((size_t)num_offsets * (size_t)(wcn_kmap_num_blocks(m) + 1) + 64) * 4;
}

static void launch_tally(uint32_t* mask, int32_t* nbr, int64_t m, int K, int32_t* counts, bool hist, int nblk_sort,
                         int32_t* dcounts, const int32_t* coords, const CellTable* cells, int32_t* status, int kc, int sort_shift,
                         int sort_bits, hipStream_t s, bool compact = false) {
  const int kp = compact ? (kCompactPitch | kCompactFlag) : wcn_kmap_row_pitch(K), mw = wcn_kmap_mask_words(K);
  const int64_t ntile = wcn_kmap_num_blocks(m);
  int32_t* ticket = counts + (int64_t)K * (ntile + 1);
  const dim3 grid((unsigned)ceil_div(m, kRsTile)), block(kTallyThreads);
  CellTable none{};
  const CellTable& t = cells ? *cells : none;
  const uint32_t cmask = cells ? (uint32_t)(cells->capacity - 1) : 0u;
#define WCN_TALLY(H, R)                                                                                                \
  hipLaunchKernelGGL((kmap_tally_kernel<H, R>), grid, block, 0, s, mask, nbr, m, K, kp, mw, ntile, counts, ticket,       \
                     nblk_sort, dcounts, (const int4*)coords, t, cmask, status, kc, sort_shift, sort_bits)
  if (hist && cells) WCN_TALLY(true, true);
  else if (hist) WCN_TALLY(true, false);
  else if (cells) WCN_TALLY(false, true);
  else WCN_TALLY(false, false);
#undef WCN_TALLY
}

static void launch_scan(int32_t* counts, int64_t ntile, int K, int32_t* offsets, const int32_t* status, int32_t* mirror,
                        int nblk_sort, int32_t* dcounts, int32_t* dtotals, int sort_bins, hipStream_t s) {
  int32_t* totals = counts + (int64_t)K * ntile;
  int32_t* ticket = totals + K;
  hipLaunchKernelGGL(kmap_scan_kernel, dim3((unsigned)(K + (nblk_sort > 0 ? (sort_bins + kRsScanCols - 1) / kRsScanCols : 0))), dim3(kBkThreads), 0,
                     s, counts, ntile, K, totals, ticket, offsets, status, mirror, dcounts, nblk_sort, dtotals, sort_bins);
}

int wcn_kmap_count(const uint32_t* mask, int64_t m, int32_t num_offsets, int32_t* counts, wcn_stream_t stream) {
  if (m < 0 || !valid_k(num_offsets)) return WCN_ERROR_INVALID_PARAMETERS;
  if (m == 0) return WCN_SUCCESS;
  if (!mask || !counts) return WCN_ERROR_INVALID_PARAMETERS;
  launch_tally(const_cast<uint32_t*>(mask), nullptr, m, num_offsets, counts, false, 0, nullptr, nullptr, nullptr, nullptr, 0, 0,
               kRsBits, (hipStream_t)stream);
  return launch_status();
}

static int scan_impl(int32_t* counts, int64_t num_blocks, int32_t K, int32_t* offsets, const int32_t* status,
                     int32_t* mirror, wcn_stream_t stream) {
  if (num_blocks < 0 || (num_blocks & 3) || !valid_k(K) || !offsets || !counts) return WCN_ERROR_INVALID_PARAMETERS;
  launch_scan(counts, num_blocks, K, offsets, status, mirror, 0, nullptr, nullptr, 0, (hipStream_t)stream);
  return launch_status();
}

int wcn_kmap_scan(int32_t* counts, int64_t num_blocks, int32_t num_offsets, int32_t* offsets, wcn_stream_t stream) {
  return scan_impl(counts, num_blocks, num_offsets, offsets, nullptr, nullptr, stream);
}

int wcn_kmap_scan_to_host(int32_t* counts, int64_t num_blocks, int32_t num_offsets, int32_t* offsets, const int32_t* status,
                          int32_t* host_mirror, wcn_stream_t stream) {
  if (!host_mirror) return WCN_ERROR_INVALID_PARAMETERS;
  return scan_impl(counts, num_blocks, num_offsets, offsets, status, host_mirror, stream);
}

size_t wcn_kmap_tally_sort_workspace(int64_t m) { return wcn_mask_argsort_workspace(m); }

int wcn_kmap_tally_sort(uint32_t* mask, int32_t* nbr, int64_t m, int32_t num_offsets, int32_t* counts, int32_t* offsets,
                        int32_t* status, int32_t* host_mirror, int32_t* perm, void* sort_workspace,
                        size_t sort_workspace_bytes, const int32_t* coords, void* binned_workspace, int64_t binned_n,
                        int64_t max_blocks, int32_t compact, int32_t* in_maps, int32_t* out_maps, int64_t pair_capacity,
                        wcn_stream_t stream) {
  if (m < 0 || !valid_k(num_offsets) || !counts || !offsets || !status) return WCN_ERROR_INVALID_PARAMETERS;
  if (pair_capacity < 0 || ((in_maps == nullptr) != (out_maps == nullptr))) return WCN_ERROR_INVALID_PARAMETERS;
  if (compact && !wcn_kmap_compact_supported(num_offsets)) return WCN_ERROR_INVALID_PARAMETERS;
  hipStream_t s = (hipStream_t)stream;
  if (m == 0) {
    if (hipMemsetAsync(offsets, 0, (size_t)(num_offsets + 1) * 4, s) != hipSuccess) return WCN_ERROR_KERNEL_EXECUTION;
    if (host_mirror) {
      if (hipMemsetAsync(host_mirror, 0, (size_t)(num_offsets + 1) * 4, s) != hipSuccess ||
          hipMemcpyAsync(host_mirror + num_offsets + 1, status, 4, hipMemcpyDeviceToHost, s) != hipSuccess)
        return WCN_ERROR_KERNEL_EXECUTION;
    }
    return WCN_SUCCESS;
  }
  if (m >= (1ll << 31) || !mask || !nbr || !perm || !sort_workspace ||
      sort_workspace_bytes < wcn_kmap_tally_sort_workspace(m))
    return WCN_ERROR_INVALID_PARAMETERS;
  if (binned_workspace && (!coords || binned_n != m || max_blocks < 1)) return WCN_ERROR_INVALID_PARAMETERS;
  const int kc = tile_key_centre(num_offsets, wcn_kmap_mask_words(num_offsets));
  const SortPlan plan = sort_plan(sort_workspace, m, num_offsets < 32 ? num_offsets : 32, kc > 0);
  CellTable cells{};
// ... 40 lines not shown
```

### warpconvnet_amd/csrc/wgrad_mfma.hip

```cpp
#include "wcn_common.h"

namespace wcn {

typedef __attribute__((ext_vector_type(8))) __bf16 bf16x8;
typedef __attribute__((ext_vector_type(8))) _Float16 f16x8;
typedef __attribute__((ext_vector_type(4))) short s16x4;
typedef __attribute__((ext_vector_type(8))) short s16x8;
typedef __attribute__((ext_vector_type(16))) float f32x16;

constexpr int kWgradGrid = 512;
constexpr int kPairs = 64;
constexpr int kZeroPage = 1024;
__device__ uint4 g_wgrad_zero_page[64];

template <typename T> struct WFrag;
template <> struct WFrag<__bf16> {
  static __device__ __forceinline__ f32x16 mfma(s16x8 a, s16x8 b, f32x16 c) {
    return __builtin_amdgcn_mfma_f32_32x32x16_bf16(__builtin_bit_cast(bf16x8, a), __builtin_bit_cast(bf16x8, b), c, 0, 0, 0);
  }
};
template <> struct WFrag<_Float16> {
  static __device__ __forceinline__ f32x16 mfma(s16x8 a, s16x8 b, f32x16 c) {
    return __builtin_amdgcn_mfma_f32_32x32x16_f16(__builtin_bit_cast(f16x8, a), __builtin_bit_cast(f16x8, b), c, 0, 0, 0);
  }
};

template <int CH>
__device__ __forceinline__ int chunk_swizzle(int p) {
  if (CH >= 16) return (p & 3) << 2;
  if (CH == 8) return ((p >> 1) & 1) << 2;
  return 0;
}

template <int CH>
__device__ __forceinline__ s16x8 read_frag_tr(const char* tile, int p0, int c0, int lane) {
  const int g = lane >> 4, i = lane & 15;
  const int col = c0 + 16 * (g & 1) + 4 * (i & 3);
  const int chunk = col >> 3, within = (col & 7) * 2;
  s16x8 out;
#pragma unroll
  for (int t = 0; t < 2; ++t) {
    const int p = p0 + 8 * (g >> 1) + 4 * t + (i >> 2);
    const char* addr = tile + p * (CH * 16) + ((chunk ^ chunk_swizzle<CH>(p)) << 4) + within;
    const s16x4 v = __builtin_amdgcn_ds_read_tr16_b64_v4i16((s16x4 __attribute__((address_space(3)))*)addr);
    out[4 * t + 0] = v[0]; out[4 * t + 1] = v[1]; out[4 * t + 2] = v[2]; out[4 * t + 3] = v[3];
  }
  return out;
}

template <typename T> __device__ __forceinline__ s16x8 ones_row_frag(int lane) {
  const short one = sizeof(T) == 2 && __is_same(T, __bf16) ? (short)0x3F80 : (short)0x3C00;
  const short v = ((lane & 31) == 0) ? one : (short)0;
  s16x8 f;
#pragma unroll
  for (int q = 0; q < 8; ++q) f[q] = v;
  return f;
}

constexpr int kStages = 3;
constexpr int kIdxSlots = 4;

template <typename T, int CIT, int COT>
struct Wgrad {
  static constexpr int CHX = CIT / 8;
  static constexpr int CHY = COT / 8;
  static constexpr int XT_BYTES = kPairs * CIT * 2;
  static constexpr int YT_BYTES = kPairs * COT * 2;
  static constexpr int STAGE_BYTES = XT_BYTES + YT_BYTES;
  static constexpr int X_UNITS = XT_BYTES / 1024, Y_UNITS = YT_BYTES / 1024;
  static constexpr int DATA_OPS = (X_UNITS + Y_UNITS) / 4;
  static constexpr int MBLK = CIT / 32, NBLK = COT / 32;
  static constexpr int BLOCKS = MBLK * NBLK;
  static constexpr bool GRID = (MBLK % 2 == 0) && (NBLK % 2 == 0);
  static constexpr int MB = GRID ? MBLK / 2 : 1, NB = GRID ? NBLK / 2 : 1;
  static constexpr int PER_WAVE = GRID ? MB * NB : (BLOCKS + 3) / 4;
  static constexpr int IDX_BYTES = kIdxSlots * 2 * kPairs * 4;
  static constexpr size_t LDS_BYTES = (size_t)kStages * STAGE_BYTES + IDX_BYTES;
  static_assert(CIT % 32 == 0 && COT % 32 == 0, "tile must be a multiple of 32 channels");
  static_assert(X_UNITS % 4 == 0 && Y_UNITS % 4 == 0, "every wave must issue the same number of DMA instructions");
};

template <typename T, int CIT, int COT, bool CS>
__global__ __launch_bounds__(256, 2) void wgrad_mfma_kernel(const T* __restrict__ x, const T* __restrict__ dy,
                                                         const int32_t* __restrict__ in_maps,
                                                         const int32_t* __restrict__ out_maps,
                                                         const int32_t* __restrict__ offsets, int K, int cin, int cout,
                                                         const char* __restrict__ zero_page, float* __restrict__ slabs,
                                                         float* __restrict__ cs_slabs, int cs_k) {
  typedef Wgrad<T, CIT, COT> W;
  extern __shared__ __attribute__((aligned(16))) char smem[];
  char* s_idx = smem + (size_t)kStages * W::STAGE_BYTES;
  const int tid = threadIdx.x, lane = tid & 63, wave = tid >> 6;
  const int G = gridDim.x, g = blockIdx.x;
  const int tiles_co = cout / COT;
  const int ci0 = (blockIdx.y / tiles_co) * CIT, co0 = (blockIdx.y % tiles_co) * COT;

  const int64_t L = offsets[K];
  int64_t Q = (L + G - 1) / G;
  Q = ((Q + kPairs - 1) / kPairs) * kPairs;
  const int64_t r_begin = (int64_t)g * Q;
  const int64_t r_end = (r_begin + Q < L) ? (r_begin + Q) : L;
  if (r_begin >= r_end) return;

  int k = 0;
  {
    int lo = 0, hi = K;
    while (hi - lo > 1) {
      const int mid = (lo + hi) >> 1;
      if ((int64_t)offsets[mid] <= r_begin) lo = mid; else hi = mid;
    }
    k = lo;
  }

  static_assert(!CS || W::GRID, "the fused bias gradient needs the 2 x 2 wave layout");
  f32x16 acc[W::PER_WAVE];
  f32x16 acc1[CS ? W::NB : 1];
  auto zero_acc = [&]() {
#pragma unroll
    for (int j = 0; j < W::PER_WAVE; ++j)
#pragma unroll
      for (int q = 0; q < 16; ++q) acc[j][q] = 0.f;
    if (CS) {
#pragma unroll
      for (int b = 0; b < W::NB; ++b)
#pragma unroll
        for (int q = 0; q < 16; ++q) acc1[b][q] = 0.f;
    }
  };
  const bool cs_tile = CS && (blockIdx.y / tiles_co) == 0;
  const s16x8 ones = ones_row_frag<T>(lane);
  auto flush = [&](int kk) {
    float* slab = slabs + (int64_t)(g + kk) * cin * cout;
    const int h = lane >> 5, n = lane & 31;
#pragma unroll
    for (int j = 0; j < W::PER_WAVE; ++j) {
      const int blk = W::GRID ? ((wave >> 1) * W::MB + j / W::NB) * W::NBLK + (wave & 1) * W::NB + j % W::NB
                              : wave + 4 * j;
      if (blk < W::BLOCKS) {
        const int a = blk / W::NBLK, b = blk % W::NBLK;
#pragma unroll
        for (int q = 0; q < 16; ++q) {
          const int ci = ci0 + a * 32 + (q & 3) + 8 * (q >> 2) + 4 * h;
          const int co = co0 + b * 32 + n;
          slab[(int64_t)ci * cout + co] = acc[j][q];
        }
      }
    }
  };

  auto dma_idx = [&](int st, int64_t seg_begin, int64_t seg_end) {
    char* slot = s_idx + (size_t)(st % kIdxSlots) * (2 * kPairs * 4);
    int64_t p = seg_begin + (int64_t)st * kPairs + wave * 16 + (lane & 15);
    if (p >= seg_end) p = seg_end - 1;
    const uint32_t d_in = __builtin_amdgcn_readfirstlane(lds_addr_of(slot + wave * 64));
    const uint32_t d_out = __builtin_amdgcn_readfirstlane(lds_addr_of(slot + kPairs * 4 + wave * 64));
    if (lane < 16) {
      glds4(in_maps + p, d_in);
      glds4(out_maps + p, d_out);
    }
  };
  auto dma_data = [&](int st, int64_t seg_begin, int64_t seg_end) {
    char* xt = smem + (size_t)(st % kStages) * W::STAGE_BYTES;
    char* yt = xt + W::XT_BYTES;
    const int* idx_in = reinterpret_cast<const int*>(s_idx + (size_t)(st % kIdxSlots) * (2 * kPairs * 4));
    const int* idx_out = idx_in + kPairs;
    const int64_t p0 = seg_begin + (int64_t)st * kPairs;
#pragma unroll
    for (int it = 0; it < W::X_UNITS / 4; ++it) {
      const int u = it * 4 + wave;
      const int piece = u * 64 + lane;
      const int p = piece / W::CHX, qs = piece % W::CHX;
      const int q = qs ^ chunk_swizzle<W::CHX>(p);
      const char* src = zero_page;
      if (p0 + p < seg_end) src = reinterpret_cast<const char*>(x + (int64_t)idx_in[p] * cin + ci0) + q * 16;
      glds16(src, __builtin_amdgcn_readfirstlane(lds_addr_of(xt + u * 1024)));
    }
#pragma unroll
    for (int it = 0; it < W::Y_UNITS / 4; ++it) {
      const int u = it * 4 + wave;
      const int piece = u * 64 + lane;
      const int p = piece / W::CHY, qs = piece % W::CHY;
      const int q = qs ^ chunk_swizzle<W::CHY>(p);
      const char* src = zero_page;
      if (p0 + p < seg_end) src = reinterpret_cast<const char*>(dy + (int64_t)idx_out[p] * cout + co0) + q * 16;
      glds16(src, __builtin_amdgcn_readfirstlane(lds_addr_of(yt + u * 1024)));
    }
  };
  auto compute = [&](int st, bool do_cs) {
    const char* xt = smem + (size_t)(st % kStages) * W::STAGE_BYTES;
    const char* yt = xt + W::XT_BYTES;
#pragma unroll
    for (int ks = 0; ks < kPairs / 16; ++ks) {
      if constexpr (W::GRID) {
        s16x8 af[W::MB], bf[W::NB];
#pragma unroll
        for (int a = 0; a < W::MB; ++a) af[a] = read_frag_tr<W::CHX>(xt, ks * 16, ((wave >> 1) * W::MB + a) * 32, lane);
#pragma unroll
        for (int b = 0; b < W::NB; ++b) bf[b] = read_frag_tr<W::CHY>(yt, ks * 16, ((wave & 1) * W::NB + b) * 32, lane);
#pragma unroll
        for (int a = 0; a < W::MB; ++a)
#pragma unroll
          for (int b = 0; b < W::NB; ++b) acc[a * W::NB + b] = WFrag<T>::mfma(af[a], bf[b], acc[a * W::NB + b]);
        if (CS && do_cs && (wave >> 1) == 0) {
#pragma unroll
          for (int b = 0; b < W::NB; ++b) acc1[b] = WFrag<T>::mfma(ones, bf[b], acc1[b]);
        }
      } else {
#pragma unroll
        for (int j = 0; j < W::PER_WAVE; ++j) {
          const int blk = wave + 4 * j;
          if (blk < W::BLOCKS) {
            const s16x8 af = read_frag_tr<W::CHX>(xt, ks * 16, (blk / W::NBLK) * 32, lane);
            const s16x8 bf = read_frag_tr<W::CHY>(yt, ks * 16, (blk % W::NBLK) * 32, lane);
            acc[j] = WFrag<T>::mfma(af, bf, acc[j]);
          }
        }
      }
    }
  };
  auto barrier = [&]() {
    asm volatile("s_waitcnt lgkmcnt(0)" ::: "memory");
    __builtin_amdgcn_s_barrier();
  };

  int64_t pos = r_begin;
  while (pos < r_end) {
    while ((int64_t)offsets[k + 1] <= pos) ++k;
    const int64_t seg_end = ((int64_t)offsets[k + 1] < r_end) ? (int64_t)offsets[k + 1] : r_end;
    const int nsteps = (int)((seg_end - pos + kPairs - 1) / kPairs);
    const bool do_cs = cs_tile && k == cs_k;
    zero_acc();
    dma_idx(0, pos, seg_end);
    if (nsteps > 1) dma_idx(1, pos, seg_end);
    if (nsteps > 2) dma_idx(2, pos, seg_end);
    wait_vmcnt<0>();
    barrier();
    dma_data(0, pos, seg_end);
    if (nsteps > 1) {
      dma_data(1, pos, seg_end);
      wait_vmcnt<W::DATA_OPS>();
    } else {
      wait_vmcnt<0>();
    }
    barrier();
    for (int i = 0; i < nsteps; ++i) {
      if (i + 3 < nsteps) dma_idx(i + 3, pos, seg_end);
      const bool more = i + 2 < nsteps;
      if (more) dma_data(i + 2, pos, seg_end);
      compute(i, do_cs);
      if (more) {
        wait_vmcnt<W::DATA_OPS>();
      } else {
        wait_vmcnt<0>();
      }
      barrier();
    }
    flush(k);
    if (CS && do_cs && (wave >> 1) == 0 && lane < 32) {
#pragma unroll
      for (int b = 0; b < W::NB; ++b)
        cs_slabs[(int64_t)g * cout + co0 + ((wave & 1) * W::NB + b) * 32 + lane] = acc1[b][0];
    }
    pos = seg_end;
  }
}

__global__ __launch_bounds__(256) void wgrad_reduce_kernel(const float* __restrict__ slabs,
                                                           const int32_t* __restrict__ offsets, int K, int64_t ce, int G,
                                                           float* __restrict__ dw, const float* __restrict__ cs_slabs,
                                                           int cs_k, int cout, float* __restrict__ bias_grad) {
  __shared__ float4 s_part[16][16];
  const int part = threadIdx.x >> 4, el = threadIdx.x & 15;
  const int64_t e = (int64_t)blockIdx.x * 64 + el * 4;
  const int k = blockIdx.y;
  const int64_t L = offsets[K];
  int64_t Q = (L + G - 1) / G;
  Q = ((Q + kPairs - 1) / kPairs) * kPairs;
  if (k == K) {
    const int co = blockIdx.x * 4 + (threadIdx.x >> 6), lane = threadIdx.x & 63;
    if (co >= cout) return;
    const int64_t b = offsets[cs_k], en = offsets[cs_k + 1];
    float s = 0.f;
    if (en > b && Q > 0) {
      const int g_lo = (int)(b / Q), g_hi = (int)((en - 1) / Q);
      for (int g = g_lo + lane; g <= g_hi; g += 64) s += cs_slabs[(int64_t)g * cout + co];
    }
#pragma unroll
    for (int d = 32; d >= 1; d >>= 1) s += __shfl_xor(s, d);
    if (lane == 0) bias_grad[co] = s;
    return;
  }
  const int64_t b = offsets[k], en = offsets[k + 1];
  float4 s = make_float4(0.f, 0.f, 0.f, 0.f);
  if (e < ce && en > b && Q > 0) {
    const int g_lo = (int)(b / Q), g_hi = (int)((en - 1) / Q);
    for (int g = g_lo + part; g <= g_hi; g += 16) {
      const float4 v = *reinterpret_cast<const float4*>(slabs + (int64_t)(g + k) * ce + e);
      s.x += v.x; s.y += v.y; s.z += v.z; s.w += v.w;
    }
  }
  s_part[part][el] = s;
  __syncthreads();
  if (part == 0 && e < ce) {
    float4 t = s_part[0][el];
#pragma unroll
    for (int p = 1; p < 16; ++p) {
      const float4 v = s_part[p][el];
      t.x += v.x; t.y += v.y; t.z += v.z; t.w += v.w;
    }
    *reinterpret_cast<float4*>(dw + (int64_t)k * ce + e) = t;
  }
}

static int wgrad_tile(int c) {
  if (c % 128 == 0) return 128;
  if (c % 96 == 0) return 96;
  if (c % 64 == 0) return 64;
  if (c % 32 == 0) return 32;
  return 0;
}

bool mfma_wgrad_supported(int cin, int cout, int dtype) {
  if (dtype != WCN_F16 && dtype != WCN_BF16) return false;
  return wgrad_tile(cin) != 0 && wgrad_tile(cout) != 0;
}

bool mfma_wgrad_bias_supported(int cin, int cout, int dtype) {
  if (!mfma_wgrad_supported(cin, cout, dtype)) return false;
  return (wgrad_tile(cin) / 32) % 2 == 0 && (wgrad_tile(cout) / 32) % 2 == 0;
}

size_t wgrad_mfma_workspace(int K, int cin, int cout) {
  return (size_t)kZeroPage + (size_t)(kWgradGrid + K) * cin * cout * sizeof(float) + (size_t)kWgradGrid * cout * sizeof(float);
}

static int wgrad_ranges(int64_t pair_bound, int tiles) {
#ifdef WCN_WGRAD_FIXED_G
  return kWgradGrid;
#endif
  if (pair_bound <= 0) return kWgradGrid;
  int64_t g = (pair_bound + 511) / 512;
  const int64_t g_min = (kWgradGrid + tiles - 1) / tiles;
  if (g < g_min) g = g_min;
  if (g > kWgradGrid) g = kWgradGrid;
  return (int)g;
}

template <typename T, int CIT, int COT>
static int launch_wgrad(const void* x, const void* dy, float* dw, const int32_t* in_maps, const int32_t* out_maps,
                        const int32_t* offsets, int cin, int cout, int K, void* workspace, int cs_k, float* bias_grad,
                        int64_t pair_bound, hipStream_t s) {
  typedef Wgrad<T, CIT, COT> W;
  static unsigned long long attr_done = 0ull;
  const int rc = once_per_device(attr_done, [] {
    if (hipFuncSetAttribute(reinterpret_cast<const void*>(wgrad_mfma_kernel<T, CIT, COT, false>),
                            hipFuncAttributeMaxDynamicSharedMemorySize, (int)W::LDS_BYTES) != hipSuccess)
      return false;
    if constexpr (W::GRID) {
      if (hipFuncSetAttribute(reinterpret_cast<const void*>(wgrad_mfma_kernel<T, CIT, COT, true>),
                              hipFuncAttributeMaxDynamicSharedMemorySize, (int)W::LDS_BYTES) != hipSuccess)
        return false;
    }
    return true;
  });
  if (rc != WCN_SUCCESS) return rc;
  static char* zero_pages[64] = {};
  int dev = 0;
  if (hipGetDevice(&dev) != hipSuccess) return WCN_ERROR_KERNEL_INITIALIZATION;
  char* zero_page = (dev >= 0 && dev < 64) ? __atomic_load_n(&zero_pages[dev], __ATOMIC_RELAXED) : nullptr;
  if (!zero_page) {
    if (hipGetSymbolAddress((void**)&zero_page, HIP_SYMBOL(g_wgrad_zero_page)) != hipSuccess)
      return WCN_ERROR_KERNEL_INITIALIZATION;
    if (dev >= 0 && dev < 64) __atomic_store_n(&zero_pages[dev], zero_page, __ATOMIC_RELAXED);
  }
  float* slabs = (float*)((char*)workspace + kZeroPage);
  float* cs_slabs = slabs + (size_t)(kWgradGrid + K) * cin * cout;
  const int G = wgrad_ranges(pair_bound, (cin / CIT) * (cout / COT));
  const dim3 grid(G, (cin / CIT) * (cout / COT));
  if (bias_grad) {
    if constexpr (W::GRID) {
      hipLaunchKernelGGL((wgrad_mfma_kernel<T, CIT, COT, true>), grid, dim3(256), W::LDS_BYTES, s, (const T*)x,
                         (const T*)dy, in_maps, out_maps, offsets, K, cin, cout, (const char*)zero_page, slabs, cs_slabs,
                         cs_k);
    } else {
      return WCN_ERROR_UNSUPPORTED_CONFIG;
    }
  } else {
    hipLaunchKernelGGL((wgrad_mfma_kernel<T, CIT, COT, false>), grid, dim3(256), W::LDS_BYTES, s, (const T*)x,
                       (const T*)dy, in_maps, out_maps, offsets, K, cin, cout, (const char*)zero_page, slabs, nullptr, -1);
  }
  const int64_t ce = (int64_t)cin * cout;
  const unsigned gx = (unsigned)ceil_div(ce, 64);
  if (bias_grad && (int64_t)gx * 4 < cout) return WCN_ERROR_UNSUPPORTED_CONFIG;
  hipLaunchKernelGGL(wgrad_reduce_kernel, dim3(gx, bias_grad ? K + 1 : K), dim3(256), 0, s, (const float*)slabs, offsets, K, ce,
                     G, dw, (const float*)cs_slabs, cs_k, cout, bias_grad);
  return launch_status();
}

template <typename T, int CIT>
static int dispatch_wgrad_co(int cot, const void* x, const void* dy, float* dw, const int32_t* in_maps,
                             const int32_t* out_maps, const int32_t* offsets, int cin, int cout, int K, void* workspace,
                             int cs_k, float* bias_grad, int64_t pair_bound, hipStream_t s) {
  switch (cot) {
    case 32: return launch_wgrad<T, CIT, 32>(x, dy, dw, in_maps, out_maps, offsets, cin, cout, K, workspace, cs_k, bias_grad, pair_bound, s);
    case 64: return launch_wgrad<T, CIT, 64>(x, dy, dw, in_maps, out_maps, offsets, cin, cout, K, workspace, cs_k, bias_grad, pair_bound, s);
    case 96: return launch_wgrad<T, CIT, 96>(x, dy, dw, in_maps, out_maps, offsets, cin, cout, K, workspace, cs_k, bias_grad, pair_bound, s);
    default: return launch_wgrad<T, CIT, 128>(x, dy, dw, in_maps, out_maps, offsets, cin, cout, K, workspace, cs_k, bias_grad, pair_bound, s);
  }
}

template <typename T>
static int dispatch_wgrad(const void* x, const void* dy, float* dw, const int32_t* in_maps, const int32_t* out_maps,
                          const int32_t* offsets, int cin, int cout, int K, void* workspace, int cs_k, float* bias_grad,
                          int64_t pair_bound, hipStream_t s) {
  const int cot = wgrad_tile(cout);
  int cit = wgrad_tile(cin);
  if (cit == 128) cit = 64;
  switch (cit) {
    case 32: return dispatch_wgrad_co<T, 32>(cot, x, dy, dw, in_maps, out_maps, offsets, cin, cout, K, workspace, cs_k, bias_grad, pair_bound, s);
    case 64: return dispatch_wgrad_co<T, 64>(cot, x, dy, dw, in_maps, out_maps, offsets, cin, cout, K, workspace, cs_k, bias_grad, pair_bound, s);
    case 96: return dispatch_wgrad_co<T, 96>(cot, x, dy, dw, in_maps, out_maps, offsets, cin, cout, K, workspace, cs_k, bias_grad, pair_bound, s);
    default: return dispatch_wgrad_co<T, 128>(cot, x, dy, dw, in_maps, out_maps, offsets, cin, cout, K, workspace, cs_k, bias_grad, pair_bound, s);
  }
}

int conv_wgrad_mfma(const void* x, const void* dy, float* dw, const int32_t* in_maps, const int32_t* out_maps,
                    const int32_t* offsets, int cin, int cout, int K, int dtype, void* workspace, size_t workspace_bytes,
                    int cs_k, float* bias_grad, int64_t pair_bound, hipStream_t s) {
  if (!mfma_wgrad_supported(cin, cout, dtype)) return WCN_ERROR_UNSUPPORTED_CONFIG;
  if (bias_grad && (!mfma_wgrad_bias_supported(cin, cout, dtype) || cs_k < 0 || cs_k >= K)) return WCN_ERROR_UNSUPPORTED_CONFIG;
  if (!workspace || workspace_bytes < wgrad_mfma_workspace(K, cin, cout)) return WCN_ERROR_INVALID_PARAMETERS;
  return with_dtype16(dtype, [&](auto t) {
    return dispatch_wgrad<decltype(t)>(x, dy, dw, in_maps, out_maps, offsets, cin, cout, K, workspace, cs_k, bias_grad, pair_bound,
                                       s);
  });
}

}
```

### warpconvnet_amd/geometry/coords/search/search_results.py

```python
from typing import List, Literal, Optional, Tuple

import torch
from torch import Tensor


class RealSearchResult:

    def __init__(self, *args):
        if len(args) == 2:
            self.neighbor_indices = args[0].long()
            self.neighbor_row_splits = args[1].long()
        elif len(args) == 1:
            knn = args[0]
            assert isinstance(knn, Tensor) and knn.ndim == 2, "expected an [M, k] index tensor"
            M, k = knn.shape
            self.neighbor_indices = knn.long()
            self.neighbor_row_splits = torch.arange(0, M * k + 1, k, device=knn.device, dtype=torch.long)
        else:
            raise ValueError("RealSearchResult takes (indices, row_splits) or a single [M, k] tensor")
        self.neighbor_distances = None
        self._transposed = None

    def to(self, device):
        self.neighbor_indices = self.neighbor_indices.to(device)
        self.neighbor_row_splits = self.neighbor_row_splits.to(device)
        self._transposed = None
        return self

    def transposed(self, num_inputs: int):
        if self._transposed is None or self._transposed[0] != int(num_inputs):
            import importlib

            edge_conv = importlib.import_module("warpconvnet_amd.nn.functional.edge_conv")
            uniform = self.neighbor_indices.ndim == 2
            view = edge_conv.transposed_lists(self.neighbor_indices, int(num_inputs),
                                              None if uniform else self.neighbor_row_splits)
            self._transposed = (int(num_inputs), view)
        return self._transposed[1]

    def __repr__(self):
        return (
            f"{self.__class__.__name__}(neighbor_indices={tuple(self.neighbor_indices.shape)}, "
            f"neighbor_row_splits={tuple(self.neighbor_row_splits.shape)})"
        )


class IntSearchResult:

    def __init__(
        self,
        in_maps: Tensor,
        out_maps: Tensor,
        offsets: Tensor,
        identity_map_index: Optional[int] = None,
    ):
        offsets_cpu = offsets.detach().cpu()
        assert len(in_maps) == len(out_maps) == int(offsets_cpu[-1]), (
            f"in_maps ({len(in_maps)}), out_maps ({len(out_maps)}) and offsets[-1] ({int(offsets_cpu[-1])}) disagree"
        )
        self._in_maps = in_maps
        self._out_maps = out_maps
        self._offsets = offsets_cpu
        self._lazy_pairs = None
        self._num_offsets = len(offsets_cpu) - 1
        self._init_tables()
        self.identity_map_index = identity_map_index

    def _init_tables(self):
        self._nbr_dense: Optional[Tensor] = None
        self._nbrc: Optional[Tensor] = None
        self._mask: Optional[Tensor] = None
        self._perm: Optional[Tensor] = None
        self._offsets_dev: Optional[Tensor] = None
        self._symmetric: bool = False
        self._self_exact: bool = False
        self._has_duplicates: bool = False
        self._dup_symmetric: bool = False
        self._rev: Optional[Tuple[Tensor, Tensor, Tensor]] = None
        self._num_in: Optional[int] = None
        self._num_out: Optional[int] = None
        self._pair_table_cache: Optional[Tensor] = None
        self._validate_fn = None
        self._stride_window = False
        self._validating = False
        self._identity: Optional[int] = None
        self._validate_error: Optional[Exception] = None
        self._on_invalid = None
        self._twin = None
        self._device: Optional[torch.device] = None
        self._kernel_size: Optional[Tuple[int, ...]] = None
        self._hashtable = None
        self._keepalive = None
        self._pool_swapped: Optional["IntSearchResult"] = None

    @property
    def has_tables(self) -> bool:
        return self._nbr_dense is not None or self._nbrc is not None

    @property
    def _nbr(self) -> Optional[Tensor]:
        if self._nbr_dense is None and self._nbrc is not None:
            from warpconvnet_amd import _lib

            c = self._nbrc
            K = self._num_offsets
            dense = torch.empty((c.shape[0], _lib.lib().wcn_kmap_row_pitch(K)), dtype=torch.int32, device=c.device)
            _lib.check(_lib.lib().wcn_kmap_densify(_lib.ptr(c), c.shape[0], K, _lib.ptr(dense), _lib.stream_handle(c.device)),
                       "wcn_kmap_densify")
            self._nbr_dense = dense
        return self._nbr_dense

    @_nbr.setter
    def _nbr(self, value: Optional[Tensor]) -> None:
        self._nbr_dense = value
        self._nbrc = None

    @classmethod
    def _blank(cls, num_offsets: int, device) -> "IntSearchResult":
        self = object.__new__(cls)
        self._in_maps = self._out_maps = None
        self._offsets = None
        self._lazy_pairs = None
        self._num_offsets = num_offsets
        self._init_tables()
        self._device = torch.device(device)
        self.identity_map_index = None
        return self

    @classmethod
    def _from_deferred_pairs(cls, scatter, offsets_host: Tensor, device, identity_map_index: Optional[int]) -> "IntSearchResult":
        self = cls._blank(len(offsets_host) - 1, device)
        self._offsets = offsets_host.detach().cpu()
        self._lazy_pairs = scatter
        self.identity_map_index = identity_map_index
        return self

    @property
    def identity_map_index(self) -> Optional[int]:
        if (self._validate_fn is not None or self._validate_error is not None) and not self._validating:
            self.validate()
        return self._identity

    @identity_map_index.setter
    def identity_map_index(self, value: Optional[int]) -> None:
        self._identity = value

    def validate(self) -> bool:
        if self._validate_error is not None:
            raise self._validate_error
        fn = self._validate_fn
        if fn is None or self._validating:
            return False
        self._validating = True
        try:
            rebuilt = bool(fn(self))
        except Exception as e:
# ... 114 lines not shown
```

### warpconvnet_amd/geometry/coords/search/torch_discrete.py

```python
import ctypes
import os
from typing import Literal, Optional, Sequence, Tuple

import numpy as np
import torch

from warpconvnet_amd.utils.compile_guard import eager_unless_compiling
from torch import Tensor

from warpconvnet_amd import _lib
from warpconvnet_amd.geometry.coords.search.cell_handle import attach_cells, cells_of, stride_map_of
from warpconvnet_amd.geometry.coords.search.packed_hashmap import PackedHashTable, _next_power_of_2
from warpconvnet_amd.geometry.coords.search.search_results import IntSearchResult
from warpconvnet_amd.utils.ntuple import ntuple


@torch.no_grad()
def kernel_offsets_from_size(
    kernel_size: Tuple[int, ...],
    kernel_dilation: Tuple[int, ...],
    center_offset: Optional[Tuple[int, ...]] = None,
    device: Optional[torch.device] = None,
) -> Tensor:
    assert len(kernel_size) == len(kernel_dilation)
# ... 282 lines not shown
                                        stream),
                "wcn_kmap_build_binned",
            )
        elif prebuilt is not None:
            nbr, mask = prebuilt
        elif cells is not None:
            _lib.check(
                L.wcn_kmap_probe_cells(_lib.ptr(cells[0]), N, cells[2], _lib.ptr(out_coords), M, _lib.i3(ksize), _lib.i3(stride),
                                       _lib.i3(dilation), _lib.ptr(nbr), _lib.ptr(mask), stream),
                "wcn_kmap_probe_cells",
            )
        else:
            table = PackedHashTable(max(16, 2 * N), device=dev)
            table._launch_insert(in_coords, meta[K + 1 :])
            _lib.check(
                L.wcn_kmap_probe(_lib.ptr(table.slots_tensor), table.capacity, _lib.ptr(out_coords), M, _lib.i3(ksize),
                                 _lib.i3(stride), _lib.i3(dilation), _lib.ptr(nbr), _lib.ptr(mask), stream),
                "wcn_kmap_probe",
            )
        meta_host = torch.empty(K + 3, dtype=torch.int32, pin_memory=True)
        ready = ctypes.c_int32.from_address(meta_host.data_ptr() + 4 * (K + 2))
        ready.value = 0
        sort_bytes = L.wcn_kmap_tally_sort_workspace(M)
        sort_ws = torch.empty(sort_bytes, dtype=torch.uint8, device=dev)
        spec_capacity = max(int(spec_capacity), 0) if M > 0 else 0
        spec_in = torch.empty(spec_capacity, dtype=torch.int32, device=dev) if spec_capacity else None
        spec_out = torch.empty(spec_capacity, dtype=torch.int32, device=dev) if spec_capacity else None
        _lib.check(
            L.wcn_kmap_tally_sort(_lib.ptr(mask), _lib.ptr(nbr), M, K, _lib.ptr(block_counts), _lib.ptr(meta),
                                  _lib.ptr(meta[K + 1 :]), ctypes.c_void_p(meta_host.data_ptr()), _lib.ptr(perm),
                                  _lib.ptr(sort_ws), sort_bytes, _lib.ptr(in_coords) if use_binned else None,
                                  _lib.ptr(bin_ws), N if use_binned else 0, max_blocks if use_binned else 0, int(compact),
                                  _lib.ptr(spec_in), _lib.ptr(spec_out), spec_capacity, stream),
            "wcn_kmap_tally_sort",
        )
        event = torch.cuda.Event()
        event.record(torch.cuda.current_stream(dev))
        return dict(nbr=nbr, mask=mask, perm=perm, block_counts=block_counts, meta=meta, meta_host=meta_host, ready=ready,
                    event=event, table=table, keep=(bin_ws, sort_ws, cells), max_blocks=max_blocks, compact=compact,
                    spec_pairs=(spec_in, spec_out, spec_capacity) if spec_capacity else None)

    def scatter(b, capacity):
        capacity = max(int(capacity), 0)
        in_maps = torch.empty(capacity, dtype=torch.int32, device=dev)
        out_maps = torch.empty(capacity, dtype=torch.int32, device=dev)
        _lib.check(
            L.wcn_kmap_scatter(_lib.ptr(b["nbr"]), _lib.ptr(b["mask"]), M, K, _lib.ptr(b["block_counts"]), _lib.ptr(b["meta"]),
                               _lib.ptr(in_maps), _lib.ptr(out_maps), capacity, _lib.ptr(b["meta"][K + 1 :]), int(b["compact"]),
                               _lib.stream_handle(dev)),
            "wcn_kmap_scatter",
        )
        return in_maps, out_maps, capacity

    def settle(b):
        rebuilt = False
        while True:
            if M > 0:
                for _ in range(_SPIN_POLLS):
                    if b["ready"].value:
                        break
            if not b["ready"].value:
                b["event"].synchronize()
            flags = int(b["meta_host"][K + 1])
            if use_binned and (flags & _lib.WCN_FLAG_TABLE_FULL) and state["max_blocks"] < N:
                hints.div = 4 if hints.div > 4 else 1
                state["max_blocks"] = max(1024, N // 4) if hints.div == 4 and state["max_blocks"] < max(1024, N // 4) else N
            elif use_binned and (flags & _lib.WCN_FLAG_ROW_OVERFLOW) and state["compact"]:
                hints.observe_row_overflow(K)
                state["compact"] = False
            elif use_binned and (flags & _lib.WCN_FLAG_NEED_STRICT) and not state["strict"]:
                state["strict"] = 1
            else:
                return b, flags, rebuilt
            hints.stats["rebuilds"] += 1
            b, rebuilt = launch(), True

    def attach_tables(result, b):
        result._nbr, result._mask, result._perm = None, b["mask"], b["perm"]
        if b["compact"]:
            result._nbrc = b["nbr"]
        else:
            result._nbr = b["nbr"]
        result._offsets_dev = b["meta"][: K + 1]
        result._hashtable = b["table"]
        result._keepalive = b

    def finalize(result, b, flags):
        PackedHashTable.raise_for_flags(flags, N, table_capacity)
        offsets_host = torch.from_numpy(b["meta_host"].numpy()[: K + 1].copy())
        pair_capacity = int(offsets_host[-1])
        has_duplicates = bool(flags & _lib.WCN_FLAG_DUPLICATE_COORD)
        identity = K // 2 if (odd and unit_stride and N == M) else None
        if has_duplicates and same_tensor:
            identity = None
        hints.observe_pairs(M, pair_capacity, K)
        if use_binned and not (flags & (_lib.WCN_FLAG_TABLE_FULL | _lib.WCN_FLAG_NEED_STRICT | _lib.WCN_FLAG_ROW_OVERFLOW)):
            attach_cells(in_coords, b["keep"][0], N, b["max_blocks"])
            if batch_indexed_in_coords is not in_coords and batch_indexed_in_coords.data_ptr() == in_coords.data_ptr():
                attach_cells(batch_indexed_in_coords, b["keep"][0], N, b["max_blocks"])
        attach_tables(result, b)
        result._offsets = offsets_host
        result.identity_map_index = identity
        result._device = torch.device(dev)
        spec = b.get("spec_pairs")
        if spec is not None and spec[2] < pair_capacity:
            spec = None
            hints.stats["pair_rewrites"] += 1
        if spec is not None:
            in_full, out_full, cap = spec
            if cap > 2 * pair_capacity + 65536:
                in_full, out_full = in_full[:pair_capacity].clone(), out_full[:pair_capacity].clone()
            result._in_maps, result._out_maps = in_full[:pair_capacity], out_full[:pair_capacity]
            result._lazy_pairs = None
            b["spec_pairs"] = None
        elif need_pairs:
            result._in_maps, result._out_maps = scatter(b, pair_capacity)[:2]
            result._lazy_pairs = None
        else:
            result._in_maps = result._out_maps = None
            result._lazy_pairs = lambda: scatter(b, pair_capacity)[:2]
        result._symmetric = bool(same_tensor and odd and unit_stride and not has_duplicates)
        result._self_exact = result._symmetric
        result._has_duplicates = bool(same_tensor and has_duplicates)
        result._dup_symmetric = bool(result._has_duplicates and odd and unit_stride)

    result = IntSearchResult._blank(K, dev)
    result._num_in, result._num_out = N, M
    result._kernel_size = ksize
    result._stride_window = prebuilt is not None
    spec = 0
    if optimistic and need_pairs and M > 0:
        spec = min(N, K * M) if prebuilt is not None else hints.pair_capacity(M, K)
    hints.stats["builds"] += 1
    first = launch(spec)
    if optimistic:
        if need_pairs and first.get("spec_pairs") is None:
            first["spec_pairs"] = scatter(first, 0)
        attach_tables(result, first)

        def validate_fn(res, b=first):
            b2, flags, rebuilt = settle(b)
            finalize(res, b2, flags)
            return rebuilt

        result._validate_fn = validate_fn
        return result
    b, flags, _ = settle(first)
    finalize(result, b, flags)
    return result
```

### warpconvnet_amd/nn/functional/sparse_conv/block.py

```python
import os
from typing import Optional

import torch
from torch import Tensor
from torch.autograd import Function

from warpconvnet_amd import _lib
from warpconvnet_amd.dist import claim_grad_slot
from warpconvnet_amd.nn.functional.normalizations import (bn_affine_grads, bn_backward, bn_forward, bn_grad_rows, bn_module_state,
                                                          bn_workspace)

from .detail import hip_gemm


_OBSERVER = None


class _Plan:

    __slots__ = ("km", "num_in", "num_out", "cin", "cout", "K", "code", "relu", "bn")


class _ConvBnAct(Function):

    @staticmethod
    def forward(ctx, x: Tensor, w: Tensor, gamma: Optional[Tensor], beta: Optional[Tensor], plan: _Plan,
                residual: Optional[Tensor] = None) -> Tensor:
        L = _lib.lib()
        dev = x.device
        stream = _lib.stream_handle(dev)
        km, M, cin, cout, K, code = plan.km, plan.num_out, plan.cin, plan.cout, plan.K, plan.code
        wp = hip_gemm.pack_weight(w, False, False, dtype=x.dtype,
                                  dgrad_flip=hip_gemm.predict_dgrad_flip(km) if ctx.needs_input_grad[0] else None)
        y = torch.empty((M, cout), dtype=x.dtype, device=dev)
        xp, wpp, yp = _lib.ptr(x), _lib.ptr(wp), _lib.ptr(y)

        def launch():
            tb, mk = hip_gemm.own_tables(km, cin, cout, K, x.dtype)
            _lib.check(L.wcn_conv_gather_gemm(xp, wpp, yp, _lib.ptr(tb), _lib.ptr(mk), _lib.ptr(km._perm), None,
                                              plan.num_in, M, cin, cout, K, code, _lib.WCN_ALGO_MFMA, 0, 0, stream),
                       "wcn_conv_gather_gemm")

        launch()
        if km.validate():
            launch()
        if _OBSERVER is not None:
            _OBSERVER("forward", dict(x=x, w=w, km=km, y=y, num_in=plan.num_in, num_out=M))
        out, stats = bn_forward(y, residual, gamma, beta, plan.bn, plan.relu)
        ctx.has_res = residual is not None
        if ctx.has_res and plan.relu:
            ctx.save_for_backward(x, w, y, stats, gamma, out)
        else:
            ctx.save_for_backward(x, w, y, stats, gamma)
        ctx.plan = plan
        ctx.gdtype = gamma.dtype if gamma is not None else None
        ctx.bdtype = beta.dtype if beta is not None else None
        return out

    @staticmethod
    def backward(ctx, grad_out: Tensor):
        saved = ctx.saved_tensors
        x, w, y, stats, gamma = saved[:5]
        z = saved[5] if len(saved) > 5 else None
        plan = ctx.plan
        km, M, cin, cout, K, code = plan.km, plan.num_out, plan.cin, plan.cout, plan.K, plan.code
        L = _lib.lib()
        dev = y.device
        stream = _lib.stream_handle(dev)
        need_dx, need_dw = ctx.needs_input_grad[0], ctx.needs_input_grad[1]
        need_dres = ctx.has_res and ctx.needs_input_grad[5]
        if km._has_duplicates or not (need_dx or need_dw):
            dyc, sums, dres = bn_backward(grad_out, y, z if ctx.has_res else None, stats, gamma, plan.relu, plan.bn[0],
                                          need_dx or need_dw, need_dres)
            dx = hip_gemm.hip_dgrad(dyc, w, km, plan.num_in, "auto") if need_dx else None
            dw = hip_gemm.hip_wgrad(x, dyc, km, (K, cin, cout), "auto").to(w.dtype) if need_dw else None
            if _OBSERVER is not None:
                _OBSERVER("backward", dict(x=x, w=w, km=km, dy=dyc, dx=dx, dw=dw, num_in=plan.num_in, num_out=M))
            dgamma, dbeta = bn_affine_grads(ctx, sums, 2)
            ctx.plan = None
            return dx, dw, dgamma, dbeta, None, dres
        g, g_ld = bn_grad_rows(grad_out, y)
        masked = z is not None and plan.relu
        sums = torch.empty((2, cout), dtype=torch.float32, device=dev)
        dyc = torch.empty_like(y)
        dres = torch.empty_like(y) if (masked and need_dres) else None
        tbl = msk = perm = wpd = dx = None
        flip = False
        if need_dx:
            tbl, msk, perm, flip = hip_gemm.dgrad_tables(km, plan.num_in, cout, cin, K, y.dtype)
            wpd = hip_gemm.pack_weight(w, True, flip, dtype=y.dtype)
            dx = torch.empty((plan.num_in, cin), dtype=y.dtype, device=dev)
        dw = wws = None
        ws_bytes = 0
        if need_dw:
            slot = getattr(w, "_wcn_grad_slot", None)
            if slot is not None and slot.dtype == torch.float32 and slot.shape == w.shape:
                slot = claim_grad_slot(w)
            else:
                slot = None
            if slot is not None:
                dw = slot.detach()
            else:
                dw = torch.empty((K, cin, cout), dtype=torch.float32, device=dev)
            ws_bytes = hip_gemm._wgrad_workspace(K, cin, cout, _lib.WCN_ALGO_MFMA)
            wws = torch.empty(ws_bytes, dtype=torch.uint8, device=dev)
        bws = bn_workspace(cout, dev)
        _lib.check(L.wcn_conv_bn_backward_ld(
            _lib.ptr(g), g_ld, _lib.ptr(x), _lib.ptr(y), _lib.ptr(z) if masked else None, int(plan.relu), stats.data_ptr(), _lib.ptr(gamma),
            int(plan.bn[0]), sums.data_ptr(), _lib.ptr(dyc), _lib.ptr(dres), _lib.ptr(wpd), _lib.ptr(tbl), _lib.ptr(msk),
            _lib.ptr(perm), int(flip), _lib.ptr(dx), _lib.ptr(km.in_maps_device) if need_dw else None,
            _lib.ptr(km.out_maps_device) if need_dw else None, _lib.ptr(km._offsets_dev) if need_dw else None, _lib.ptr(dw),
            _lib.ptr(wws), ws_bytes, plan.num_in, M, cin, cout, K, code, _lib.ptr(bws), bws.numel(), stream), "wcn_conv_bn_backward_ld")
        if need_dres and not masked:
            dres = g
        if dw is not None and dw.dtype != w.dtype:
            dw = dw.to(w.dtype)
        if _OBSERVER is not None:
            _OBSERVER("backward", dict(x=x, w=w, km=km, dy=dyc, dx=dx, dw=dw, num_in=plan.num_in, num_out=M))
        dgamma, dbeta = bn_affine_grads(ctx, sums, 2)
        ctx.plan = None
        return dx, dw, dgamma, dbeta, None, dres


class _PointwiseBnAct(Function):

    @staticmethod
    def forward(ctx, x: Tensor, w: Tensor, gamma: Optional[Tensor], beta: Optional[Tensor], plan: _Plan) -> Tensor:
        from .pointwise import dense_rows, narrow_rows

        y = narrow_rows(x, w, False, dtype=_lib.torch_dtype(plan.code)) if x.dtype == torch.float32 else dense_rows(x, w, False)
        if y is None:
            xc = x if x.dtype == _lib.torch_dtype(plan.code) else x.to(_lib.torch_dtype(plan.code))
            y = xc @ (w[0] if w.dtype == xc.dtype else w[0].to(xc.dtype))
        out, stats = bn_forward(y, None, gamma, beta, plan.bn, plan.relu)
        ctx.save_for_backward(x, y, stats, gamma, w)
        ctx.plan, ctx.wdtype = plan, w.dtype
        ctx.gdtype = gamma.dtype if gamma is not None else None
        ctx.bdtype = beta.dtype if beta is not None else None
        return out

    @staticmethod
    def backward(ctx, grad_out: Tensor):
        from .pointwise import dense_wgrad

        x, y, stats, gamma, w3 = ctx.saved_tensors
        plan = ctx.plan
        need_dx, need_dw = ctx.needs_input_grad[0], ctx.needs_input_grad[1]
        dyc, sums, _ = bn_backward(grad_out, y, None, stats, gamma, plan.relu, plan.bn[0], need_dx or need_dw)
        dx = dw = None
        if need_dx:
            from .pointwise import dense_rows

            dx = dense_rows(dyc, w3, True)
            if dx is None:
                dx = dyc @ (w3[0] if w3.dtype == dyc.dtype else w3[0].to(dyc.dtype)).t()
        if need_dw:
            dw = dense_wgrad(x, dyc).unsqueeze(0)
            if dw.dtype != ctx.wdtype:
                dw = dw.to(ctx.wdtype)
        dgamma, dbeta = bn_affine_grads(ctx, sums, 2)
        ctx.plan = None
        return dx, dw, dgamma, dbeta, None


def _static_ok(conv, norm) -> int:
    from warpconvnet_amd.nn.functional.sparse_conv.helper import STRIDED_CONV_MODE
    from warpconvnet_amd.nn.modules.sparse_conv import SpatiallySparseConv

    if type(norm) is not torch.nn.BatchNorm1d or not isinstance(conv, SpatiallySparseConv):
        return 0
    if conv.groups != 1 or conv.bias is not None or conv.generative or conv.weight.ndim != 3:
        return 0
    if conv.num_spatial_dims != 3 or conv.order is not None or conv.compute_dtype is not None:
        return 0
    if conv.stride_mode != STRIDED_CONV_MODE.STRIDE_ONLY:
        return 0
    for a in (conv.fwd_algo, conv.dgrad_algo, conv.wgrad_algo):
        if str(getattr(a, "value", a)).lower() not in ("auto", "hip_mfma"):
            return 0
    if conv.weight.dtype != torch.float32 or norm.num_features != conv.out_channels:
        return 0
    if all(k == 1 for k in conv.kernel_size):
        return 2 if all(s == 1 for s in conv.stride) and not conv.transposed else 0
    return 3 if conv.transposed else 1


def conv_bn_act(x, conv, norm, relu: bool, residual=None, out_spatial=None):
    from warpconvnet_amd.geometry.types.voxels import Voxels
    from warpconvnet_amd.nn.functional.sparse_conv.helper import generate_output_coords_and_kernel_map, wrap_conv_output

    if os.environ.get("WARPCONVNET_AMD_FUSED_BLOCK", "1") == "0":
        return None
    ok = conv.__dict__.get("_wcn_block_ok")
    if ok is None or ok[0] is not norm:
        ok = conv.__dict__["_wcn_block_ok"] = (norm, _static_ok(conv, norm))
# ... 78 lines not shown
```

### warpconvnet_amd/nn/functional/sparse_conv/detail/hip_gemm.py

```python
import functools
from typing import Optional, Tuple

import torch
from torch import Tensor

from warpconvnet_amd import _lib
from warpconvnet_amd.geometry.coords.search.search_results import IntSearchResult
from warpconvnet_amd.geometry.coords.search.torch_discrete import attach_tables_from_csr, reverse_tables


def _prep(t: Tensor, name: str) -> Tensor:
    t = t.contiguous()
    _lib.require_gpu_tensor(t, name)
    return t


_FP16_RESCALE_TARGET = 32768.0


@functools.lru_cache(maxsize=None)
def _gather_ok(cin: int, cout: int, K: int, code: int) -> bool:
    return bool(_lib.lib().wcn_mfma_gather_supported(cin, cout, K, code))


@functools.lru_cache(maxsize=None)
def _wgrad_ok(cin: int, cout: int, code: int) -> bool:
    return bool(_lib.lib().wcn_mfma_wgrad_supported(cin, cout, code))


@functools.lru_cache(maxsize=None)
def _wgrad_bias_ok(cin: int, cout: int, code: int) -> bool:
    return bool(_lib.lib().wcn_mfma_wgrad_bias_supported(cin, cout, code))


@functools.lru_cache(maxsize=None)
def _wgrad_workspace(K: int, cin: int, cout: int, code: int) -> int:
    return int(_lib.lib().wcn_conv_wgrad_workspace(K, cin, cout, code))


_FP16_RESCALE_MIN_EXP = -126.0


def fp16_safe_cast(t: Tensor) -> Tuple[Tensor, Tensor]:
    if t.numel() == 0:
        return t.half(), torch.ones((), dtype=torch.float32, device=t.device)
    m = t.abs().max().float()
    exp = torch.ceil(torch.log2(m / _FP16_RESCALE_TARGET))
    exp = torch.where(m == 0, torch.zeros_like(exp), torch.clamp(exp, min=_FP16_RESCALE_MIN_EXP))
    return (t * torch.exp2(-exp)).half(), torch.exp2(exp)


def _via_fp16(a: Tensor, b: Tensor, launch) -> Tensor:
    a16, sa = fp16_safe_cast(a)
    b16, sb = fp16_safe_cast(b)
    return launch(a16, b16) * (sa * sb)


_NATIVE, _REF, _VIA_FP16, _PADDED = "native", "ref", "via_fp16", "padded"
_MFMA_COUTS = (16, 32, 48, 64, 96, 128, 160, 192, 256, 384, 512)


def _code16(dtype: torch.dtype) -> int:
    return _lib.WCN_F16 if dtype == torch.float32 else _lib.dtype_code(dtype)


def _resolve(algo: str, ok: bool, what: str, shape: str):
    if algo == "hip_mfma" and not ok:
        raise RuntimeError(f"hip_mfma {what}: {_lib.status_string(-4)} ({shape})")
    return (_NATIVE, _lib.WCN_ALGO_MFMA) if ok and algo != "hip_ref" else (_REF, _lib.WCN_ALGO_REF)


@functools.lru_cache(maxsize=None)
def _gather_plan(algo: str, kin: int, kout: int, K: int, dtype: torch.dtype, on_gpu: bool):
    if algo == "auto" and on_gpu and not _gather_ok(kin, kout, K, _code16(dtype)) and dtype in (torch.float16, torch.bfloat16):
        kin_p = max(32, (kin + 31) // 32 * 32)
        for kout_p in _MFMA_COUTS:
            if kout_p >= kout and _gather_ok(kin_p, kout_p, K, _lib.dtype_code(dtype)):
                return _PADDED, _lib.WCN_ALGO_MFMA, kin_p, kout_p
    if dtype == torch.float32 and algo != "hip_ref" and _gather_ok(kin, kout, K, _lib.WCN_F16):
        return _VIA_FP16, _lib.WCN_ALGO_MFMA, kin, kout
    return _resolve(algo, _gather_ok(kin, kout, K, _lib.dtype_code(dtype)), "error",
                    f"cin={kin}, cout={kout}, K={K}, {dtype}") + (kin, kout)

# ... 210 lines not shown
    ws_bytes = L.wcn_colsum_workspace(c)
    ws = torch.empty(ws_bytes, dtype=torch.uint8, device=t.device)
    _lib.check(
        L.wcn_colsum(_lib.ptr(t), n, c, _lib.dtype_code(t.dtype), _lib.ptr(out), _lib.ptr(ws), ws_bytes,
                     _lib.stream_handle(t.device)),
        "wcn_colsum",
    )
    return out


def _dgrad_pair_lists(dy: Tensor, w: Tensor, kernel_map: IntSearchResult, num_in: int) -> Tensor:
    K, cin, cout = w.shape
    dx = torch.zeros(num_in, cin, dtype=torch.float32, device=dy.device)
    wf = w.float()
    for k in range(K):
        in_map, out_map = kernel_map[k]
        if in_map.shape[0]:
            dx.index_add_(0, in_map.long(), dy[out_map.long()].float() @ wf[k].T)
    return dx.to(dy.dtype)


def _dgrad_duplicates(dy: Tensor, w: Tensor, kernel_map: IntSearchResult, num_in: int, algo: str) -> Tensor:
    K = len(kernel_map)
    n = num_in
    winner = kernel_map._nbr[:, K // 2].long()
    dyp = torch.zeros((n, dy.shape[1]), dtype=torch.float32, device=dy.device).index_add_(0, winner, dy.float()).to(dy.dtype)
    shadow = IntSearchResult._blank(K, dy.device)
    shadow._nbr, shadow._mask, shadow._perm = kernel_map._nbr, kernel_map._mask, kernel_map._perm
    shadow._nbrc = kernel_map._nbrc
    shadow._offsets_dev, shadow._offsets = kernel_map._offsets_dev, kernel_map._offsets
    shadow._symmetric, shadow._has_duplicates = True, False
    shadow._in_maps, shadow._out_maps = kernel_map._in_maps, kernel_map._out_maps
    dx = hip_dgrad(dyp, w, shadow, n, algo)
    keep = winner == torch.arange(n, device=dy.device)
    return dx * keep.unsqueeze(1).to(dx.dtype)


def hip_dgrad(grad_output: Tensor, weight: Tensor, kernel_map: IntSearchResult, num_in_coords: int,
              algo: str = "auto") -> Tensor:
    dy, w = _prep(grad_output, "grad_output"), _prep(weight, "weight")
    if dy.dtype != w.dtype and not master_weight_ok(dy.dtype, w, algo, True):
        raise RuntimeError(f"hip dgrad error: {_lib.status_string(-6)} ({dy.dtype} vs {w.dtype})")
    K, cin, cout = w.shape
    kernel_map.validate()
    if kernel_map._has_duplicates:
        if kernel_map._dup_symmetric and kernel_map.has_tables and dy.shape[0] == num_in_coords:
            return _dgrad_duplicates(dy, w, kernel_map, num_in_coords, algo)
        return _dgrad_pair_lists(dy, w, kernel_map, num_in_coords)
    how, code, cout_p, cin_p = _gather_plan(algo, cout, cin, K, dy.dtype, dy.is_cuda)
    if how == _PADDED:
        dy, w = _fit(dy, cout_p), _fit(w, cin_p, cout_p)
    attach_tables_from_csr(kernel_map, num_in_coords, dy.shape[0])
    tbl, mask, perm, flip = dgrad_tables(kernel_map, num_in_coords, cout_p, cin_p, K,
                                         torch.float16 if how == _VIA_FP16 else dy.dtype, mfma=code == _lib.WCN_ALGO_MFMA)
    if how == _VIA_FP16:
        return _via_fp16(dy, w, lambda g16, w16: _gather_gemm(g16, w16, tbl, mask, perm, num_in_coords, cout, cin, K, code,
                                                              transposed=True, flip=flip, f32_out=True))
    dx = _gather_gemm(dy, w, tbl, mask, perm, num_in_coords, cout_p, cin_p, K, code, transposed=True, flip=flip)
    return _fit(dx, cin) if how == _PADDED else dx


def hip_wgrad(in_features: Tensor, grad_output: Tensor, kernel_map: IntSearchResult, weight_shape, algo: str = "auto",
              want_bias_grad: bool = False, out: Optional[Tensor] = None):
    x, dy = _prep(in_features, "in_features"), _prep(grad_output, "grad_output")
    if x.dtype != dy.dtype:
        raise RuntimeError(f"hip wgrad error: {_lib.status_string(-6)} ({x.dtype} vs {dy.dtype})")
    K, cin, cout = weight_shape
    how, code, cin_p, cout_p = _wgrad_plan(algo, cin, cout, x.dtype, x.is_cuda)
    if how == _PADDED:
        x, dy = _fit(x, cin_p), _fit(dy, cout_p)
    kernel_map.validate()
    if how == _VIA_FP16:
        dw = _via_fp16(x, dy, lambda x16, g16: _wgrad_launch(x16, g16, kernel_map, K, cin, cout, code, None, False)[0])
        return (dw, None) if want_bias_grad else dw
    if out is not None and (how == _PADDED or out.shape != (K, cin, cout) or out.dtype != torch.float32
                            or not out.is_contiguous() or out.device != x.device):
        out = None
    dw, db = _wgrad_launch(x, dy, kernel_map, K, cin_p, cout_p, code, out, want_bias_grad)
    if how == _PADDED:
        dw, db = _fit(dw, cin, cout), _fit(db, cout)
    return (dw, db) if want_bias_grad else dw


def _wgrad_launch(x: Tensor, dy: Tensor, kernel_map: IntSearchResult, K: int, cin: int, cout: int, code: int,
                  out: Optional[Tensor], want_bias_grad: bool):
    dev = x.device
    dw = out if out is not None else torch.empty((K, cin, cout), dtype=torch.float32, device=dev)
    if kernel_map._offsets_dev is None:
        kernel_map._offsets_dev = kernel_map.offsets.to(device=dev, dtype=torch.int32)
    L = _lib.lib()
    ws_bytes = _wgrad_workspace(K, cin, cout, code)
    ws = torch.empty(ws_bytes, dtype=torch.uint8, device=dev)
    fuse = (want_bias_grad and code == _lib.WCN_ALGO_MFMA and kernel_map._self_exact
            and x.shape[0] == dy.shape[0] and dy.shape[0] > 0
            and _wgrad_bias_ok(cin, cout, _lib.dtype_code(x.dtype)))
    if fuse:
        db = torch.empty(cout, dtype=torch.float32, device=dev)
        _lib.check(
            L.wcn_conv_wgrad_bias(_lib.ptr(x), _lib.ptr(dy), _lib.ptr(dw), _lib.ptr(kernel_map.in_maps_device),
                                  _lib.ptr(kernel_map.out_maps_device), _lib.ptr(kernel_map._offsets_dev), x.shape[0],
                                  dy.shape[0], cin, cout, K, _lib.dtype_code(x.dtype), K // 2, _lib.ptr(db), _lib.ptr(ws),
                                  ws_bytes, _lib.stream_handle(dev)),
            "wcn_conv_wgrad_bias",
        )
        return dw, db
    _lib.check(
        L.wcn_conv_wgrad(_lib.ptr(x), _lib.ptr(dy), _lib.ptr(dw), _lib.ptr(kernel_map.in_maps_device),
                         _lib.ptr(kernel_map.out_maps_device), _lib.ptr(kernel_map._offsets_dev), x.shape[0], dy.shape[0], cin,
                         cout, K, _lib.dtype_code(x.dtype), code, _lib.ptr(ws), ws_bytes, _lib.stream_handle(dev)),
        "wcn_conv_wgrad",
    )
    return dw, None


@functools.lru_cache(maxsize=None)
def _grouped_ok(kin: int, kout: int, K: int, code: int) -> bool:
    return bool(_lib.lib().wcn_mfma_grouped_supported(kin, kout, K, code))


def grouped_supported(weight: Tensor, dtype: torch.dtype, transposed: bool) -> bool:
    if weight.ndim != 4 or not weight.is_cuda or dtype not in (torch.float16, torch.bfloat16):
        return False
    K, G, cg_in, cg_out = weight.shape
    kin, kout = (cg_out, cg_in) if transposed else (cg_in, cg_out)
    return _grouped_ok(kin, kout, K, _lib.dtype_code(dtype))


def _pack_grouped(weight: Tensor, transpose: bool, flip: bool, dtype: torch.dtype) -> Tensor:
    K, G, cg_in, cg_out = weight.shape
    kin, kout = (cg_out, cg_in) if transpose else (cg_in, cg_out)

    def make(keep: bool):
        w = weight.contiguous()
        if w.dtype not in (torch.float32, dtype):
            w = w.to(dtype)
        packed = torch.empty(w.numel(), dtype=dtype, device=w.device)
        _lib.check(
            _lib.lib().wcn_pack_weight_grouped(_lib.ptr(w), int(w.dtype == torch.float32), K, G, kin, kout, _lib.dtype_code(dtype),
                                               int(transpose), int(flip), _lib.ptr(packed), _lib.stream_handle(w.device)),
            "wcn_pack_weight_grouped",
        )
        return {key: packed}

    key = ("grouped", dtype, bool(transpose), bool(flip))
    return _cached_image(weight, key, make)


def _grouped_gather(x: Tensor, packed: Tensor, tbl: Tensor, mask: Tensor, perm: Tensor, n_out: int, kin: int, kout: int,
                    G: int, K: int, bias: Optional[Tensor]) -> Tensor:
    out = torch.empty((n_out, G * kout), dtype=x.dtype, device=x.device)
    if n_out == 0:
        return out
    _lib.check(
        _lib.lib().wcn_conv_gather_gemm_grouped(_lib.ptr(x), _lib.ptr(packed), _lib.ptr(out), _lib.ptr(tbl), _lib.ptr(mask),
                                                _lib.ptr(perm), _lib.ptr(bias), x.shape[0], n_out, kin, kout, G, K,
                                                _lib.dtype_code(x.dtype), _lib.stream_handle(x.device)),
        "wcn_conv_gather_gemm_grouped",
    )
    return out


def hip_forward_grouped(in_features: Tensor, weight: Tensor, kernel_map: IntSearchResult, num_out_coords: int,
                        bias: Optional[Tensor] = None) -> Tensor:
    x = _prep(in_features, "in_features")
    K, G, cg_in, cg_out = weight.shape
    assert K == len(kernel_map) and x.shape[1] == G * cg_in
    if bias is not None:
        bias = _prep(bias.detach().float(), "bias")
    kernel_map.validate()
    attach_tables_from_csr(kernel_map, x.shape[0], num_out_coords)
    packed = _pack_grouped(weight, False, False, x.dtype)
    return _grouped_gather(x, packed, kernel_map._nbr, kernel_map._mask, kernel_map._perm, num_out_coords, cg_in, cg_out, G, K, bias)


def hip_dgrad_grouped(grad_output: Tensor, weight: Tensor, kernel_map: IntSearchResult, num_in_coords: int) -> Tensor:
    dy = _prep(grad_output, "grad_output")
    K, G, cg_in, cg_out = weight.shape
    kernel_map.validate()
# ... 8 lines not shown
```

Measured before the change: 1106 M voxels/s.

## Partition wgrad work into per-offset slab teams using kmap-emitted bounds

The kernel-map tally now writes per-offset slab boundaries, 16 slabs per offset, into the counts buffer. A new teams path for the MFMA wgrad assigns each workgroup its own offset-local slab plus a balanced share of the centre offset. The goal is to cut cross-offset mixing and the reduction cost of the flat pair split. It only activates for K=27 and large pair counts, and it adds a block-level feasibility check plus a fallback.

```diff
diff --git a/include/wcn.h b/include/wcn.h
--- a/include/wcn.h
+++ b/include/wcn.h
@@ -44,6 +44,7 @@
 int32_t wcn_kmap_mask_words(int32_t num_offsets);
 int64_t wcn_kmap_num_blocks(int64_t m);
 size_t wcn_kmap_counts_bytes(int64_t m, int32_t num_offsets);
+int64_t wcn_kmap_slab_bounds_offset(int64_t m, int32_t num_offsets);
 
 int wcn_kmap_probe(const void* slots, int64_t capacity, const int32_t* query, int64_t m,
                    const int32_t ksize[3], const int32_t stride[3], const int32_t dilation[3],
@@ -159,6 +160,13 @@
                         int32_t num_offsets, int32_t dtype, int32_t self_offset, float* bias_grad, void* workspace,
                         size_t workspace_bytes, wcn_stream_t stream);
 
+int wcn_conv_wgrad_teams(const void* x, const void* dy, float* dw, const int32_t* in_maps, const int32_t* out_maps,
+                         const int32_t* offsets, const int32_t* slab_bounds, int64_t n_in, int64_t n_out, int32_t cin,
+                         int32_t cout, int32_t num_offsets, int32_t dtype, int32_t self_offset, float* bias_grad,
+                         void* workspace, size_t workspace_bytes, wcn_stream_t stream);
+int wcn_wgrad_plan_host(const int32_t* offsets, const int32_t* slab_bounds, int32_t num_offsets, int32_t grid, int32_t tiles,
+                        int32_t mode, int32_t g, int64_t* out);
+
 int wcn_dwconv_gather(const void* in, const void* w, void* out, const int32_t* nbr, const float* bias, int64_t n_in,
                       int64_t n_out, int32_t channels, int32_t num_offsets, int32_t dtype, int32_t k_flip,
                       wcn_stream_t stream);
@@ -275,6 +283,15 @@
                             float* dw, void* wgrad_workspace, size_t wgrad_workspace_bytes, int64_t n_in, int64_t n_out,
                             int32_t cin, int32_t cout, int32_t num_offsets, int32_t dtype, void* bn_workspace,
                             size_t bn_workspace_bytes, wcn_stream_t stream);
+
+int wcn_conv_bn_backward_teams(const void* grad_out, int64_t grad_out_ld, const void* x, const void* y, const void* z, int32_t relu,
+                               const float* stats, const float* gamma, int32_t training, float* sums, void* dy_conv, void* dres,
+                               const void* w_packed_dgrad, const int32_t* rev_nbr, const uint32_t* rev_mask,
+                               const int32_t* rev_perm, int32_t flip, void* dx, const int32_t* in_maps, const int32_t* out_maps,
+                               const int32_t* offsets, const int32_t* slab_bounds, float* dw, void* wgrad_workspace,
+                               size_t wgrad_workspace_bytes, int64_t n_in, int64_t n_out, int32_t cin, int32_t cout,
+                               int32_t num_offsets, int32_t dtype, void* bn_workspace, size_t bn_workspace_bytes,
+                               wcn_stream_t stream);
 
 int wcn_attn_varlen_supported(int32_t head_dim, int32_t dtype);
 size_t wcn_attn_varlen_workspace_bytes(int64_t total, int32_t heads);
diff --git a/warpconvnet_amd/_lib.py b/warpconvnet_amd/_lib.py
--- a/warpconvnet_amd/_lib.py
+++ b/warpconvnet_amd/_lib.py
@@ -71,6 +71,10 @@
                                         c_void_p, c_void_p, c_void_p, c_void_p, c_void_p, c_void_p, c_int32, c_void_p, c_void_p, c_void_p,
                                         c_void_p, c_void_p, c_void_p, c_size_t, c_int64, c_int64, c_int32, c_int32, c_int32, c_int32,
                                         c_void_p, c_size_t, c_void_p]),
+    "wcn_conv_bn_backward_teams": (c_int, [c_void_p, c_int64, c_void_p, c_void_p, c_void_p, c_int32, c_void_p, c_void_p, c_int32, c_void_p,
+                                           c_void_p, c_void_p, c_void_p, c_void_p, c_void_p, c_void_p, c_int32, c_void_p, c_void_p, c_void_p,
+                                           c_void_p, c_void_p, c_void_p, c_void_p, c_size_t, c_int64, c_int64, c_int32, c_int32, c_int32,
+                                           c_int32, c_void_p, c_size_t, c_void_p]),
     "wcn_conv_bn_backward": (c_int, [c_void_p, c_void_p, c_void_p, c_void_p, c_int32, c_void_p, c_void_p, c_int32, c_void_p, c_void_p,
                                      c_void_p, c_void_p, c_void_p, c_void_p, c_void_p, c_int32, c_void_p, c_void_p, c_void_p, c_void_p,
                                      c_void_p, c_void_p, c_size_t, c_int64, c_int64, c_int32, c_int32, c_int32, c_int32, c_void_p,
@@ -83,6 +87,7 @@
     "wcn_pool_select": (c_int, [c_void_p, c_void_p, c_void_p, c_int64, c_int64, c_int32, c_int32, c_int32, c_void_p, c_void_p]),
     "wcn_morton_code": (c_int, [c_void_p, c_int64, c_int32, c_void_p, c_void_p, c_void_p, c_void_p]),
     "wcn_kmap_counts_bytes": (c_size_t, [c_int64, c_int32]),
+    "wcn_kmap_slab_bounds_offset": (c_int64, [c_int64, c_int32]),
     "wcn_kmap_binned_workspace": (c_size_t, [c_int64, c_int64]),
     "wcn_kmap_binned_supported": (c_int, [_3I, _3I]),
     "wcn_kmap_build_binned": (
@@ -351,6 +356,12 @@
         [c_void_p, c_void_p, c_void_p, c_void_p, c_void_p, c_void_p, c_int64, c_int64, c_int32, c_int32, c_int32,
          c_int32, c_int32, c_void_p, c_void_p, c_size_t, c_void_p],
     ),
+    "wcn_conv_wgrad_teams": (
+        c_int,
+        [c_void_p, c_void_p, c_void_p, c_void_p, c_void_p, c_void_p, c_void_p, c_int64, c_int64, c_int32, c_int32, c_int32,
+         c_int32, c_int32, c_void_p, c_void_p, c_size_t, c_void_p],
+    ),
+    "wcn_wgrad_plan_host": (c_int, [c_void_p, c_void_p, c_int32, c_int32, c_int32, c_int32, c_int32, c_void_p]),
     "wcn_lattice_chunk_rows": (c_int32, []),
     "wcn_hash128_insert": (c_int, [c_void_p, c_void_p, c_int64, c_void_p, c_int64, c_int32, c_void_p, c_void_p]),
     "wcn_hash128_search": (c_int, [c_void_p, c_void_p, c_int64, c_void_p, c_void_p, c_int64, c_int32, c_int32, c_void_p,
@@ -464,7 +475,7 @@
         return False
 
 
-_HOST_ONLY = {"wcn_status_string"}
+_HOST_ONLY = {"wcn_status_string", "wcn_wgrad_plan_host"}
 _CALL_DEVICE = threading.local()
 
 
diff --git a/warpconvnet_amd/csrc/conv_api.hip b/warpconvnet_amd/csrc/conv_api.hip
--- a/warpconvnet_amd/csrc/conv_api.hip
+++ b/warpconvnet_amd/csrc/conv_api.hip
@@ -1,4 +1,5 @@
 #include "gather_gemm.h"
+#include "wgrad_plan.h"
 
 namespace wcn {
 int conv_gather_gemm_ref(const void* in, const void* w, void* out, const int32_t* nbr, const float* bias, int64_t n_out,
@@ -12,7 +13,7 @@
 bool mfma_wgrad_bias_supported(int cin, int cout, int dtype);
 int conv_wgrad_mfma(const void* x, const void* dy, float* dw, const int32_t* in_maps, const int32_t* out_maps,
                     const int32_t* offsets, int cin, int cout, int K, int dtype, void* workspace, size_t workspace_bytes,
-                    int cs_k, float* bias_grad, int64_t pair_bound, hipStream_t s);
+                    int cs_k, float* bias_grad, int64_t pair_bound, const int32_t* bounds, hipStream_t s);
 int dwconv_gather(const void* in, const void* w, void* out, const int32_t* tbl, const float* bias, int64_t n_out, int C,
                   int K, int dtype, int k_flip, hipStream_t s);
 size_t dwconv_wgrad_workspace(int K, int C);
@@ -191,7 +192,7 @@
       return conv_wgrad_ref(x, dy, dw, in_maps, out_maps, offsets, cin, cout, num_offsets, dtype, s);
     case WCN_ALGO_MFMA:
       return conv_wgrad_mfma(x, dy, dw, in_maps, out_maps, offsets, cin, cout, num_offsets, dtype, workspace,
-                             workspace_bytes, -1, nullptr, (int64_t)num_offsets * (n_in < n_out ? n_in : n_out), s);
+                             workspace_bytes, -1, nullptr, (int64_t)num_offsets * (n_in < n_out ? n_in : n_out), nullptr, s);
     default:
       return WCN_ERROR_INVALID_PARAMETERS;
   }
@@ -215,6 +216,20 @@
                             float* dw, void* wgrad_workspace, size_t wgrad_workspace_bytes, int64_t n_in, int64_t n_out,
                             int32_t cin, int32_t cout, int32_t num_offsets, int32_t dtype, void* bn_workspace,
                             size_t bn_workspace_bytes, wcn_stream_t stream) {
+  return wcn_conv_bn_backward_teams(grad_out, grad_out_ld, x, y, z, relu, stats, gamma, training, sums, dy_conv, dres, w_packed_dgrad,
+                                    rev_nbr, rev_mask, rev_perm, flip, dx, in_maps, out_maps, offsets, nullptr, dw, wgrad_workspace,
+                                    wgrad_workspace_bytes, n_in, n_out, cin, cout, num_offsets, dtype, bn_workspace,
+                                    bn_workspace_bytes, stream);
+}
+
+int wcn_conv_bn_backward_teams(const void* grad_out, int64_t grad_out_ld, const void* x, const void* y, const void* z, int32_t relu,
+                               const float* stats, const float* gamma, int32_t training, float* sums, void* dy_conv, void* dres,
+                               const void* w_packed_dgrad, const int32_t* rev_nbr, const uint32_t* rev_mask,
+                               const int32_t* rev_perm, int32_t flip, void* dx, const int32_t* in_maps, const int32_t* out_maps,
+                               const int32_t* offsets, const int32_t* slab_bounds, float* dw, void* wgrad_workspace,
+                               size_t wgrad_workspace_bytes, int64_t n_in, int64_t n_out, int32_t cin, int32_t cout,
+                               int32_t num_offsets, int32_t dtype, void* bn_workspace, size_t bn_workspace_bytes,
+                               wcn_stream_t stream) {
   if (!dy_conv || (dtype != WCN_F16 && dtype != WCN_BF16)) return WCN_ERROR_INVALID_PARAMETERS;
   int rc = wcn_bn_train_backward_ld(grad_out, grad_out_ld, y, z, relu, n_out, cout, dtype, stats, gamma, training, sums, dy_conv, dres,
                                     bn_workspace, bn_workspace_bytes, stream);
@@ -226,8 +241,8 @@
     if (rc != WCN_SUCCESS) return rc;
   }
   if (dw)
-    rc = wcn_conv_wgrad(x, dy_conv, dw, in_maps, out_maps, offsets, n_in, n_out, cin, cout, num_offsets, dtype, WCN_ALGO_MFMA,
-                        wgrad_workspace, wgrad_workspace_bytes, stream);
+    rc = wcn_conv_wgrad_teams(x, dy_conv, dw, in_maps, out_maps, offsets, slab_bounds, n_in, n_out, cin, cout, num_offsets, dtype, -1,
+                              nullptr, wgrad_workspace, wgrad_workspace_bytes, stream);
   return rc;
 }
 
@@ -243,7 +258,34 @@
     return WCN_ERROR_INVALID_PARAMETERS;
   if (self_offset < 0 || self_offset >= num_offsets) return WCN_ERROR_INVALID_PARAMETERS;
   return conv_wgrad_mfma(x, dy, dw, in_maps, out_maps, offsets, cin, cout, num_offsets, dtype, workspace, workspace_bytes,
-                         self_offset, bias_grad, (int64_t)num_offsets * (n_in < n_out ? n_in : n_out), (hipStream_t)stream);
+                         self_offset, bias_grad, (int64_t)num_offsets * (n_in < n_out ? n_in : n_out), nullptr,
+                         (hipStream_t)stream);
+}
+
+int wcn_conv_wgrad_teams(const void* x, const void* dy, float* dw, const int32_t* in_maps, const int32_t* out_maps,
+                         const int32_t* offsets, const int32_t* slab_bounds, int64_t n_in, int64_t n_out, int32_t cin,
+                         int32_t cout, int32_t num_offsets, int32_t dtype, int32_t self_offset, float* bias_grad,
+                         void* workspace, size_t workspace_bytes, wcn_stream_t stream) {
+  if (n_in < 0 || n_out < 0 || cin < 1 || cout < 1 || num_offsets < 1 || !dtype_ok(dtype) || !dw || !offsets)
+    return WCN_ERROR_INVALID_PARAMETERS;
+  if (bias_grad && (self_offset < 0 || self_offset >= num_offsets)) return WCN_ERROR_INVALID_PARAMETERS;
+  return conv_wgrad_mfma(x, dy, dw, in_maps, out_maps, offsets, cin, cout, num_offsets, dtype, workspace, workspace_bytes,
+                         bias_grad ? self_offset : -1, bias_grad, (int64_t)num_offsets * (n_in < n_out ? n_in : n_out),
+                         slab_bounds, (hipStream_t)stream);
+}
+
+int wcn_wgrad_plan_host(const int32_t* offsets, const int32_t* slab_bounds, int32_t num_offsets, int32_t grid, int32_t tiles,
+                        int32_t mode, int32_t g, int64_t* out) {
+  if (!offsets || !out || num_offsets < 1 || g < 0 || g >= grid) return WCN_ERROR_INVALID_PARAMETERS;
+  if (!wgrad_team_rule_all(offsets, slab_bounds, num_offsets, grid, tiles, mode)) return 0;
+  WgradSeg seg[2];
+  const int n = wgrad_team_plan(offsets, slab_bounds, num_offsets, grid, g, seg);
+  for (int i = 0; i < n; ++i) {
+    out[3 * i] = seg[i].k;
+    out[3 * i + 1] = seg[i].begin;
+    out[3 * i + 2] = seg[i].end;
+  }
+  return n;
 }
 
 int wcn_dwconv_gather(const void* in, const void* w, void* out, const int32_t* nbr, const float* bias, int64_t n_in,
diff --git a/warpconvnet_amd/csrc/kmap_bucket.hip b/warpconvnet_amd/csrc/kmap_bucket.hip
--- a/warpconvnet_amd/csrc/kmap_bucket.hip
+++ b/warpconvnet_amd/csrc/kmap_bucket.hip
@@ -1,11 +1,13 @@
 #include "kmap_cells.h"
 #include "mask_sort.h"
+#include "wgrad_plan.h"
 
 namespace wcn {
 
 constexpr int kTileRows = 256;
 constexpr int kBkThreads = 256;
 constexpr int kTallyThreads = (kRsTile / kTileRows) * 64;
+constexpr int kBoundsGap = 64;
 constexpr int kStageCap = 3072;
 
 static_assert(kRsTile % kTileRows == 0, "a sort tile is a whole number of bucket tiles");
@@ -104,6 +106,12 @@
     return;
   }
   const int total = scan_counts_in_place<kBkThreads, 16>(counts + (int64_t)blockIdx.x * ntile, ntile, s_wave);
+  if (tid <= kPlanSlabs) {
+    const int64_t tile = tid * ((ntile + kPlanSlabs - 1) / kPlanSlabs);
+    int32_t* bounds = counts + (int64_t)K * (ntile + 1) + kBoundsGap;
+    bounds[tid * K + blockIdx.x] =
+        tile < ntile ? __hip_atomic_load(&counts[(int64_t)blockIdx.x * ntile + tile], __ATOMIC_RELAXED, __HIP_MEMORY_SCOPE_AGENT) : total;
+  }
   if (tid == 0) {
     __hip_atomic_store(&totals[blockIdx.x], total, __ATOMIC_RELAXED, __HIP_MEMORY_SCOPE_AGENT);
     __threadfence();
@@ -444,7 +452,11 @@
 int64_t wcn_kmap_num_blocks(int64_t m) { return (ceil_div(m > 0 ? m : 0, kTileRows) + 3) & ~(int64_t)3; }
 
 size_t wcn_kmap_counts_bytes(int64_t m, int32_t num_offsets) {
-  return ((size_t)num_offsets * (size_t)(wcn_kmap_num_blocks(m) + 1) + 64) * 4;
+  return ((size_t)num_offsets * (size_t)(wcn_kmap_num_blocks(m) + 1) + kBoundsGap + (size_t)(kPlanSlabs + 1) * num_offsets) * 4;
+}
+
+int64_t wcn_kmap_slab_bounds_offset(int64_t m, int32_t num_offsets) {
+  return (int64_t)num_offsets * (wcn_kmap_num_blocks(m) + 1) + kBoundsGap;
 }
 
 static void launch_tally(uint32_t* mask, int32_t* nbr, int64_t m, int K, int32_t* counts, bool hist, int nblk_sort,
diff --git a/warpconvnet_amd/csrc/wgrad_mfma.hip b/warpconvnet_amd/csrc/wgrad_mfma.hip
--- a/warpconvnet_amd/csrc/wgrad_mfma.hip
+++ b/warpconvnet_amd/csrc/wgrad_mfma.hip
@@ -1,4 +1,8 @@
 #include "wcn_common.h"
+#include "wgrad_plan.h"
+
+#include <cstdlib>
+#include <cstring>
 
 namespace wcn {
 
@@ -80,13 +84,33 @@
   static_assert(X_UNITS % 4 == 0 && Y_UNITS % 4 == 0, "every wave must issue the same number of DMA instructions");
 };
 
+__device__ __forceinline__ bool wgrad_team_rule_block(const int32_t* __restrict__ offsets, const int32_t* __restrict__ bounds,
+                                                      int K, int G, int tiles, int mode, int* s_wave, int& o0, int& o1,
+                                                      int& own_total) {
+  static_assert(kPlanGrid == 2 * 256, "two workgroups of the plan per thread");
+  o0 = o1 = own_total = 0;
+  if (!wgrad_team_rule(offsets, bounds, K, G, tiles, mode)) return false;
+  const int tid = threadIdx.x;
+  const int64_t centre = (int64_t)offsets[K / 2 + 1] - offsets[K / 2];
+  o0 = (int)wgrad_own_steps(offsets, bounds, K, tid);
+  o1 = (int)wgrad_own_steps(offsets, bounds, K, tid + 256);
+  block_excl_scan<256>(o0 + o1, s_wave, &own_total);
+  own_total = __builtin_amdgcn_readfirstlane(own_total);
+  __syncthreads();
+  if (mode == kTeamsForce) return true;
+  const bool ok = wgrad_level_holds(centre, own_total, o0, G, tid) && wgrad_level_holds(centre, own_total, o1, G, tid + 256);
+  return __syncthreads_and(ok) != 0;
+}
+
 template <typename T, int CIT, int COT, bool CS>
 __global__ __launch_bounds__(256, 2) void wgrad_mfma_kernel(const T* __restrict__ x, const T* __restrict__ dy,
                                                          const int32_t* __restrict__ in_maps,
                                                          const int32_t* __restrict__ out_maps,
                                                          const int32_t* __restrict__ offsets, int K, int cin, int cout,
                                                          const char* __restrict__ zero_page, float* __restrict__ slabs,
-                                                         float* __restrict__ cs_slabs, int cs_k) {
+                                                         float* __restrict__ cs_slabs, int cs_k,
+                                                         const int32_t* __restrict__ bounds, int teams_mode,
+                                                         int32_t* __restrict__ sweep_word) {
   typedef Wgrad<T, CIT, COT> W;
   extern __shared__ __attribute__((aligned(16))) char smem[];
   char* s_idx = smem + (size_t)kStages * W::STAGE_BYTES;
@@ -95,15 +119,35 @@
   const int tiles_co = cout / COT;
   const int ci0 = (blockIdx.y / tiles_co) * CIT, co0 = (blockIdx.y % tiles_co) * COT;
 
-  const int64_t L = offsets[K];
-  int64_t Q = (L + G - 1) / G;
-  Q = ((Q + kPairs - 1) / kPairs) * kPairs;
-  const int64_t r_begin = (int64_t)g * Q;
-  const int64_t r_end = (r_begin + Q < L) ? (r_begin + Q) : L;
-  if (r_begin >= r_end) return;
-
+  int o0, o1, own_total;
+  const bool team = wgrad_team_rule_block(offsets, bounds, K, G, (int)gridDim.y, teams_mode, reinterpret_cast<int*>(s_idx), o0, o1,
+                                          own_total);
+  if (g == 0 && blockIdx.y == 0 && tid == 0) *sweep_word = team ? 1 : 0;
+  WgradSeg own, centre_piece;
+  int ti = 2;
+  int64_t r_begin = 0, r_end = 0;
   int k = 0;
-  {
+  if (team) {
+    static_assert(kPlanStep == kPairs, "the plan counts in pipeline steps");
+    int* s_wave = reinterpret_cast<int*>(s_idx);
+    const int64_t centre = (int64_t)offsets[K / 2 + 1] - offsets[K / 2];
+    int before;
+    const int c0 = tid < g ? (int)wgrad_centre_steps(centre, own_total, o0, G, tid) : 0;
+    const int c1 = tid + 256 < g ? (int)wgrad_centre_steps(centre, own_total, o1, G, tid + 256) : 0;
+    block_excl_scan<256>(c0 + c1, s_wave, &before);
+    before = __builtin_amdgcn_readfirstlane(before);
+    __syncthreads();
+    const bool member = wgrad_own_range(offsets, bounds, K, g, &own);
+    wgrad_centre_piece(offsets, K, before, wgrad_centre_steps(centre, own_total, wgrad_steps(own.end - own.begin), G, g),
+                       &centre_piece);
+    ti = member ? 0 : 1;
+  } else {
+    const int64_t L = offsets[K];
+    int64_t Q = (L + G - 1) / G;
+    Q = ((Q + kPairs - 1) / kPairs) * kPairs;
+    r_begin = (int64_t)g * Q;
+    r_end = (r_begin + Q < L) ? (r_begin + Q) : L;
+    if (r_begin >= r_end) return;
     int lo = 0, hi = K;
     while (hi - lo > 1) {
       const int mid = (lo + hi) >> 1;
@@ -129,8 +173,8 @@
   };
   const bool cs_tile = CS && (blockIdx.y / tiles_co) == 0;
   const s16x8 ones = ones_row_frag<T>(lane);
-  auto flush = [&](int kk) {
-    float* slab = slabs + (int64_t)(g + kk) * cin * cout;
+  auto flush = [&](int slab_id) {
+    float* slab = slabs + (int64_t)slab_id * cin * cout;
     const int h = lane >> 5, n = lane & 31;
 #pragma unroll
     for (int j = 0; j < W::PER_WAVE; ++j) {
@@ -224,38 +268,51 @@
   };
 
   int64_t pos = r_begin;
-  while (pos < r_end) {
-    while ((int64_t)offsets[k + 1] <= pos) ++k;
-    const int64_t seg_end = ((int64_t)offsets[k + 1] < r_end) ? (int64_t)offsets[k + 1] : r_end;
+  while (team ? ti < 2 : pos < r_end) {
+    int64_t seg_end;
+    int slab_id;
+    if (team) {
+      k = ti == 0 ? own.k : centre_piece.k;
+      pos = ti == 0 ? own.begin : centre_piece.begin;
+      seg_end = ti == 0 ? own.end : centre_piece.end;
+      slab_id = 2 * g + ti;
+      ++ti;
+    } else {
+      while ((int64_t)offsets[k + 1] <= pos) ++k;
+      seg_end = ((int64_t)offsets[k + 1] < r_end) ? (int64_t)offsets[k + 1] : r_end;
+      slab_id = g + k;
+    }
     const int nsteps = (int)((seg_end - pos + kPairs - 1) / kPairs);
     const bool do_cs = cs_tile && k == cs_k;
     zero_acc();
-    dma_idx(0, pos, seg_end);
-    if (nsteps > 1) dma_idx(1, pos, seg_end);
-    if (nsteps > 2) dma_idx(2, pos, seg_end);
-    wait_vmcnt<0>();
-    barrier();
-    dma_data(0, pos, seg_end);
-    if (nsteps > 1) {
-      dma_data(1, pos, seg_end);
-      wait_vmcnt<W::DATA_OPS>();
-    } else {
+    if (nsteps > 0) {
+      dma_idx(0, pos, seg_end);
+      if (nsteps > 1) dma_idx(1, pos, seg_end);
+      if (nsteps > 2) dma_idx(2, pos, seg_end);
       wait_vmcnt<0>();
-    }
-    barrier();
-    for (int i = 0; i < nsteps; ++i) {
-      if (i + 3 < nsteps) dma_idx(i + 3, pos, seg_end);
-      const bool more = i + 2 < nsteps;
-      if (more) dma_data(i + 2, pos, seg_end);
-      compute(i, do_cs);
-      if (more) {
+      barrier();
+      dma_data(0, pos, seg_end);
+      if (nsteps > 1) {
+        dma_data(1, pos, seg_end);
         wait_vmcnt<W::DATA_OPS>();
       } else {
         wait_vmcnt<0>();
       }
       barrier();
-    }
-    flush(k);
+      for (int i = 0; i < nsteps; ++i) {
+        if (i + 3 < nsteps) dma_idx(i + 3, pos, seg_end);
+        const bool more = i + 2 < nsteps;
+        if (more) dma_data(i + 2, pos, seg_end);
+        compute(i, do_cs);
+        if (more) {
+          wait_vmcnt<W::DATA_OPS>();
+        } else {
+          wait_vmcnt<0>();
+        }
+        barrier();
+      }
+    }
+    flush(slab_id);
     if (CS && do_cs && (wave >> 1) == 0 && lane < 32) {
 #pragma unroll
       for (int b = 0; b < W::NB; ++b)
@@ -268,7 +325,8 @@
 __global__ __launch_bounds__(256) void wgrad_reduce_kernel(const float* __restrict__ slabs,
                                                            const int32_t* __restrict__ offsets, int K, int64_t ce, int G,
                                                            float* __restrict__ dw, const float* __restrict__ cs_slabs,
-                                                           int cs_k, int cout, float* __restrict__ bias_grad) {
+                                                           int cs_k, int cout, float* __restrict__ bias_grad,
+                                                           const int32_t* __restrict__ sweep_word) {
   __shared__ float4 s_part[16][16];
   const int part = threadIdx.x >> 4, el = threadIdx.x & 15;
   const int64_t e = (int64_t)blockIdx.x * 64 + el * 4;
@@ -276,12 +334,15 @@
   const int64_t L = offsets[K];
   int64_t Q = (L + G - 1) / G;
   Q = ((Q + kPairs - 1) / kPairs) * kPairs;
+  const bool team = *sweep_word != 0;
   if (k == K) {
     const int co = blockIdx.x * 4 + (threadIdx.x >> 6), lane = threadIdx.x & 63;
     if (co >= cout) return;
     const int64_t b = offsets[cs_k], en = offsets[cs_k + 1];
     float s = 0.f;
-    if (en > b && Q > 0) {
+    if (team) {
+      for (int g = lane; g < G; g += 64) s += cs_slabs[(int64_t)g * cout + co];
+    } else if (en > b && Q > 0) {
       const int g_lo = (int)(b / Q), g_hi = (int)((en - 1) / Q);
       for (int g = g_lo + lane; g <= g_hi; g += 64) s += cs_slabs[(int64_t)g * cout + co];
     }
@@ -292,7 +353,26 @@
   }
   const int64_t b = offsets[k], en = offsets[k + 1];
   float4 s = make_float4(0.f, 0.f, 0.f, 0.f);
-  if (e < ce && en > b && Q > 0) {
+  if (team) {
+    if (e < ce) {
+      if (k == K / 2) {
+        constexpr int kBatch = 8;
+        for (int g0 = part; g0 < G; g0 += 16 * kBatch) {
+          float4 v[kBatch];
+#pragma unroll
+          for (int j = 0; j < kBatch; ++j) {
+            const int g = g0 + 16 * j;
+            v[j] = g < G ? *reinterpret_cast<const float4*>(slabs + (int64_t)(2 * g + 1) * ce + e) : make_float4(0.f, 0.f, 0.f, 0.f);
+          }
+#pragma unroll
+          for (int j = 0; j < kBatch; ++j) { s.x += v[j].x; s.y += v[j].y; s.z += v[j].z; s.w += v[j].w; }
+        }
+      } else {
+        static_assert(kPlanSlabs == 16, "one team per part");
+        s = *reinterpret_cast<const float4*>(slabs + (int64_t)(2 * wgrad_member_g(part, k < K / 2 ? k : k - 1)) * ce + e);
+      }
+    }
+  } else if (e < ce && en > b && Q > 0) {
     const int g_lo = (int)(b / Q), g_hi = (int)((en - 1) / Q);
     for (int g = g_lo + part; g <= g_hi; g += 16) {
       const float4 v = *reinterpret_cast<const float4*>(slabs + (int64_t)(g + k) * ce + e);
@@ -330,8 +410,23 @@
   return (wgrad_tile(cin) / 32) % 2 == 0 && (wgrad_tile(cout) / 32) % 2 == 0;
 }
 
+static bool wgrad_one_tile(int cin, int cout) {
+  const int cit = wgrad_tile(cin) == 128 ? 64 : wgrad_tile(cin);
+  return cit == cin && wgrad_tile(cout) == cout;
+}
+static size_t wgrad_slab_count(int K, int cin, int cout) {
+  return (size_t)(K == kPlanK && wgrad_one_tile(cin, cout) ? 2 * kWgradGrid : kWgradGrid + K);
+}
+
 size_t wgrad_mfma_workspace(int K, int cin, int cout) {
-  return (size_t)kZeroPage + (size_t)(kWgradGrid + K) * cin * cout * sizeof(float) + (size_t)kWgradGrid * cout * sizeof(float);
+  return (size_t)kZeroPage + wgrad_slab_count(K, cin, cout) * cin * cout * sizeof(float) + (size_t)kWgradGrid * cout * sizeof(float);
+}
+
+static int wgrad_teams_mode() {
+  const char* e = getenv("WARPCONVNET_AMD_WGRAD_TEAMS");
+  if (!e || !*e || !strcmp(e, "auto")) return kTeamsAuto;
+  if (!strcmp(e, "force")) return kTeamsForce;
+  return kTeamsOff;
 }
 
 static int wgrad_ranges(int64_t pair_bound, int tiles) {
@@ -349,7 +444,7 @@
 template <typename T, int CIT, int COT>
 static int launch_wgrad(const void* x, const void* dy, float* dw, const int32_t* in_maps, const int32_t* out_maps,
                         const int32_t* offsets, int cin, int cout, int K, void* workspace, int cs_k, float* bias_grad,
-                        int64_t pair_bound, hipStream_t s) {
+                        int64_t pair_bound, const int32_t* bounds, hipStream_t s) {
   typedef Wgrad<T, CIT, COT> W;
   static unsigned long long attr_done = 0ull;
   const int rc = once_per_device(attr_done, [] {
@@ -374,65 +469,68 @@
     if (dev >= 0 && dev < 64) __atomic_store_n(&zero_pages[dev], zero_page, __ATOMIC_RELAXED);
   }
   float* slabs = (float*)((char*)workspace + kZeroPage);
-  float* cs_slabs = slabs + (size_t)(kWgradGrid + K) * cin * cout;
-  const int G = wgrad_ranges(pair_bound, (cin / CIT) * (cout / COT));
+  float* cs_slabs = slabs + wgrad_slab_count(K, cin, cout) * cin * cout;
+  const int tiles = (cin / CIT) * (cout / COT);
+  const int teams = (bounds && !(bias_grad && cs_k != K / 2)) ? wgrad_teams_mode() : kTeamsOff;
+  const int G = wgrad_ranges(pair_bound, tiles);
   const dim3 grid(G, (cin / CIT) * (cout / COT));
   if (bias_grad) {
     if constexpr (W::GRID) {
       hipLaunchKernelGGL((wgrad_mfma_kernel<T, CIT, COT, true>), grid, dim3(256), W::LDS_BYTES, s, (const T*)x,
                          (const T*)dy, in_maps, out_maps, offsets, K, cin, cout, (const char*)zero_page, slabs, cs_slabs,
-                         cs_k);
+                         cs_k, bounds, teams, (int32_t*)workspace);
     } else {
       return WCN_ERROR_UNSUPPORTED_CONFIG;
     }
   } else {
     hipLaunchKernelGGL((wgrad_mfma_kernel<T, CIT, COT, false>), grid, dim3(256), W::LDS_BYTES, s, (const T*)x,
-                       (const T*)dy, in_maps, out_maps, offsets, K, cin, cout, (const char*)zero_page, slabs, nullptr, -1);
+                       (const T*)dy, in_maps, out_maps, offsets, K, cin, cout, (const char*)zero_page, slabs, nullptr, -1,
+                       bounds, teams, (int32_t*)workspace);
   }
   const int64_t ce = (int64_t)cin * cout;
   const unsigned gx = (unsigned)ceil_div(ce, 64);
   if (bias_grad && (int64_t)gx * 4 < cout) return WCN_ERROR_UNSUPPORTED_CONFIG;
   hipLaunchKernelGGL(wgrad_reduce_kernel, dim3(gx, bias_grad ? K + 1 : K), dim3(256), 0, s, (const float*)slabs, offsets, K, ce,
-                     G, dw, (const float*)cs_slabs, cs_k, cout, bias_grad);
+                     G, dw, (const float*)cs_slabs, cs_k, cout, bias_grad, (const int32_t*)workspace);
   return launch_status();
 }
 
 template <typename T, int CIT>
 static int dispatch_wgrad_co(int cot, const void* x, const void* dy, float* dw, const int32_t* in_maps,
                              const int32_t* out_maps, const int32_t* offsets, int cin, int cout, int K, void* workspace,
-                             int cs_k, float* bias_grad, int64_t pair_bound, hipStream_t s) {
+                             int cs_k, float* bias_grad, int64_t pair_bound, const int32_t* bounds, hipStream_t s) {
   switch (cot) {
-    case 32: return launch_wgrad<T, CIT, 32>(x, dy, dw, in_maps, out_maps, offsets, cin, cout, K, workspace, cs_k, bias_grad, pair_bound, s);
-    case 64: return launch_wgrad<T, CIT, 64>(x, dy, dw, in_maps, out_maps, offsets, cin, cout, K, workspace, cs_k, bias_grad, pair_bound, s);
-    case 96: return launch_wgrad<T, CIT, 96>(x, dy, dw, in_maps, out_maps, offsets, cin, cout, K, workspace, cs_k, bias_grad, pair_bound, s);
-    default: return launch_wgrad<T, CIT, 128>(x, dy, dw, in_maps, out_maps, offsets, cin, cout, K, workspace, cs_k, bias_grad, pair_bound, s);
+    case 32: return launch_wgrad<T, CIT, 32>(x, dy, dw, in_maps, out_maps, offsets, cin, cout, K, workspace, cs_k, bias_grad, pair_bound, bounds, s);
+    case 64: return launch_wgrad<T, CIT, 64>(x, dy, dw, in_maps, out_maps, offsets, cin, cout, K, workspace, cs_k, bias_grad, pair_bound, bounds, s);
+    case 96: return launch_wgrad<T, CIT, 96>(x, dy, dw, in_maps, out_maps, offsets, cin, cout, K, workspace, cs_k, bias_grad, pair_bound, bounds, s);
+    default: return launch_wgrad<T, CIT, 128>(x, dy, dw, in_maps, out_maps, offsets, cin, cout, K, workspace, cs_k, bias_grad, pair_bound, bounds, s);
   }
 }
 
 template <typename T>
 static int dispatch_wgrad(const void* x, const void* dy, float* dw, const int32_t* in_maps, const int32_t* out_maps,
                           const int32_t* offsets, int cin, int cout, int K, void* workspace, int cs_k, float* bias_grad,
-                          int64_t pair_bound, hipStream_t s) {
+                          int64_t pair_bound, const int32_t* bounds, hipStream_t s) {
   const int cot = wgrad_tile(cout);
   int cit = wgrad_tile(cin);
   if (cit == 128) cit = 64;
   switch (cit) {
-    case 32: return dispatch_wgrad_co<T, 32>(cot, x, dy, dw, in_maps, out_maps, offsets, cin, cout, K, workspace, cs_k, bias_grad, pair_bound, s);
-    case 64: return dispatch_wgrad_co<T, 64>(cot, x, dy, dw, in_maps, out_maps, offsets, cin, cout, K, workspace, cs_k, bias_grad, pair_bound, s);
-    case 96: return dispatch_wgrad_co<T, 96>(cot, x, dy, dw, in_maps, out_maps, offsets, cin, cout, K, workspace, cs_k, bias_grad, pair_bound, s);
-    default: return dispatch_wgrad_co<T, 128>(cot, x, dy, dw, in_maps, out_maps, offsets, cin, cout, K, workspace, cs_k, bias_grad, pair_bound, s);
+    case 32: return dispatch_wgrad_co<T, 32>(cot, x, dy, dw, in_maps, out_maps, offsets, cin, cout, K, workspace, cs_k, bias_grad, pair_bound, bounds, s);
+    case 64: return dispatch_wgrad_co<T, 64>(cot, x, dy, dw, in_maps, out_maps, offsets, cin, cout, K, workspace, cs_k, bias_grad, pair_bound, bounds, s);
+    case 96: return dispatch_wgrad_co<T, 96>(cot, x, dy, dw, in_maps, out_maps, offsets, cin, cout, K, workspace, cs_k, bias_grad, pair_bound, bounds, s);
+    default: return dispatch_wgrad_co<T, 128>(cot, x, dy, dw, in_maps, out_maps, offsets, cin, cout, K, workspace, cs_k, bias_grad, pair_bound, bounds, s);
   }
 }
 
 int conv_wgrad_mfma(const void* x, const void* dy, float* dw, const int32_t* in_maps, const int32_t* out_maps,
                     const int32_t* offsets, int cin, int cout, int K, int dtype, void* workspace, size_t workspace_bytes,
-                    int cs_k, float* bias_grad, int64_t pair_bound, hipStream_t s) {
+                    int cs_k, float* bias_grad, int64_t pair_bound, const int32_t* bounds, hipStream_t s) {
   if (!mfma_wgrad_supported(cin, cout, dtype)) return WCN_ERROR_UNSUPPORTED_CONFIG;
   if (bias_grad && (!mfma_wgrad_bias_supported(cin, cout, dtype) || cs_k < 0 || cs_k >= K)) return WCN_ERROR_UNSUPPORTED_CONFIG;
   if (!workspace || workspace_bytes < wgrad_mfma_workspace(K, cin, cout)) return WCN_ERROR_INVALID_PARAMETERS;
   return with_dtype16(dtype, [&](auto t) {
     return dispatch_wgrad<decltype(t)>(x, dy, dw, in_maps, out_maps, offsets, cin, cout, K, workspace, cs_k, bias_grad, pair_bound,
-                                       s);
+                                       bounds, s);
   });
 }
 
diff --git a/warpconvnet_amd/csrc/wgrad_plan.h b/warpconvnet_amd/csrc/wgrad_plan.h
--- /dev/null
+++ b/warpconvnet_amd/csrc/wgrad_plan.h
@@ -0,0 +1,127 @@
+#pragma once
+#include <stdint.h>
+
+#if defined(__HIPCC__)
+#define WCN_PLAN_FN __host__ __device__ inline
+#else
+#define WCN_PLAN_FN inline
+#endif
+
+namespace wcn {
+
+constexpr int kPlanSlabs = 16;
+constexpr int kPlanGrid = 512;
+constexpr int kPlanK = 27;
+constexpr int kPlanXcd = 8;
+constexpr int kPlanStep = 64;
+constexpr int kPlanMembers = kPlanK - 1;
+enum { kTeamsOff = 0, kTeamsAuto = 1, kTeamsForce = 2 };
+
+struct WgradSeg {
+  int k;
+  int64_t begin, end;
+};
+
+WCN_PLAN_FN bool wgrad_team_rule(const int32_t* offsets, const int32_t* bounds, int K, int G, int tiles, int mode) {
+  if (mode == kTeamsOff || !bounds || K != kPlanK || G != kPlanGrid || tiles != 1) return false;
+  if (mode != kTeamsForce && (int64_t)offsets[K] - offsets[0] < (int64_t)512 * G) return false;
+  int64_t off_sum = 0, off_max = 0;
+  bool ok = true;
+#pragma unroll
+  for (int k = 0; k < kPlanK; ++k) {
+    const int64_t cnt = (int64_t)offsets[k + 1] - offsets[k];
+    ok = ok & (cnt >= 0) & (bounds[k] == 0) & (bounds[kPlanSlabs * kPlanK + k] == cnt);
+    if (k != kPlanK / 2) {
+      off_sum += cnt;
+      off_max = cnt > off_max ? cnt : off_max;
+    }
+  }
+  if (!ok) return false;
+  if (mode == kTeamsForce) return true;
+  return off_max * (K - 1) * 10 <= off_sum * 11;
+}
+
+WCN_PLAN_FN int wgrad_member_g(int t, int m) { return (t % kPlanXcd) + kPlanXcd * ((t / kPlanXcd) * kPlanMembers + m); }
+WCN_PLAN_FN bool wgrad_member(int g, int* t, int* m) {
+  const int x = g % kPlanXcd, j = g / kPlanXcd;
+  if (j >= 2 * kPlanMembers) return false;
+  *t = x + kPlanXcd * (j / kPlanMembers);
+  *m = j % kPlanMembers;
+  return true;
+}
+WCN_PLAN_FN int wgrad_member_offset(int m) { return m < kPlanK / 2 ? m : m + 1; }
+
+WCN_PLAN_FN int64_t plan_clamp(int64_t v, int64_t hi) { return v < 0 ? 0 : (v > hi ? hi : v); }
+
+WCN_PLAN_FN bool wgrad_own_range(const int32_t* offsets, const int32_t* bounds, int K, int g, WgradSeg* seg) {
+  int t, m;
+  seg->k = K / 2;
+  seg->begin = seg->end = offsets[K / 2];
+  if (!wgrad_member(g, &t, &m)) return false;
+  const int k = wgrad_member_offset(m);
+  const int64_t cnt = (int64_t)offsets[k + 1] - offsets[k];
+  const int64_t lo = plan_clamp(bounds[t * K + k], cnt);
+  int64_t hi = plan_clamp(bounds[(t + 1) * K + k], cnt);
+  if (hi < lo) hi = lo;
+  seg->k = k;
+  seg->begin = offsets[k] + lo;
+  seg->end = offsets[k] + hi;
+  return true;
+}
+
+WCN_PLAN_FN int64_t wgrad_steps(int64_t pairs) { return (pairs + kPlanStep - 1) / kPlanStep; }
+
+WCN_PLAN_FN int64_t wgrad_own_steps(const int32_t* offsets, const int32_t* bounds, int K, int g) {
+  WgradSeg s;
+  wgrad_own_range(offsets, bounds, K, g, &s);
+  return wgrad_steps(s.end - s.begin);
+}
+
+WCN_PLAN_FN int64_t wgrad_level(int64_t centre_pairs, int64_t own_total, int G, int g) {
+  const int64_t n = wgrad_steps(centre_pairs) + own_total;
+  const int64_t s0 = (n + G - 1) / G;
+  const int64_t r = n - (s0 - 1) * G;
+  return g < r ? s0 : s0 - 1;
+}
+
+WCN_PLAN_FN int64_t wgrad_centre_steps(int64_t centre_pairs, int64_t own_total, int64_t own_steps, int G, int g) {
+  const int64_t target = wgrad_level(centre_pairs, own_total, G, g);
+  return target > own_steps ? target - own_steps : 0;
+}
+
+WCN_PLAN_FN bool wgrad_level_holds(int64_t centre_pairs, int64_t own_total, int64_t own_steps, int G, int g) {
+  return own_steps <= wgrad_level(centre_pairs, own_total, G, g);
+}
+
+WCN_PLAN_FN bool wgrad_team_rule_all(const int32_t* offsets, const int32_t* bounds, int K, int G, int tiles, int mode) {
+  if (!wgrad_team_rule(offsets, bounds, K, G, tiles, mode)) return false;
+  if (mode == kTeamsForce) return true;
+  const int64_t centre = (int64_t)offsets[K / 2 + 1] - offsets[K / 2];
+  int64_t own_total = 0;
+  for (int q = 0; q < G; ++q) own_total += wgrad_own_steps(offsets, bounds, K, q);
+  for (int q = 0; q < G; ++q)
+    if (!wgrad_level_holds(centre, own_total, wgrad_own_steps(offsets, bounds, K, q), G, q)) return false;
+  return true;
+}
+
+WCN_PLAN_FN void wgrad_centre_piece(const int32_t* offsets, int K, int64_t before, int64_t steps, WgradSeg* seg) {
+  const int64_t c0 = offsets[K / 2], cnt = (int64_t)offsets[K / 2 + 1] - c0;
+  seg->k = K / 2;
+  seg->begin = c0 + plan_clamp(before * kPlanStep, cnt);
+  seg->end = c0 + plan_clamp((before + steps) * kPlanStep, cnt);
+}
+
+WCN_PLAN_FN int wgrad_team_plan(const int32_t* offsets, const int32_t* bounds, int K, int G, int g, WgradSeg seg[2]) {
+  const int64_t centre = (int64_t)offsets[K / 2 + 1] - offsets[K / 2];
+  int64_t own_total = 0;
+  for (int q = 0; q < G; ++q) own_total += wgrad_own_steps(offsets, bounds, K, q);
+  int64_t before = 0;
+  for (int q = 0; q < g; ++q)
+    before += wgrad_centre_steps(centre, own_total, wgrad_own_steps(offsets, bounds, K, q), G, q);
+  const bool member = wgrad_own_range(offsets, bounds, K, g, &seg[0]);
+  const int64_t own = wgrad_steps(seg[0].end - seg[0].begin);
+  wgrad_centre_piece(offsets, K, before, wgrad_centre_steps(centre, own_total, own, G, g), &seg[member ? 1 : 0]);
+  return member ? 2 : 1;
+}
+
+}
diff --git a/warpconvnet_amd/geometry/coords/search/search_results.py b/warpconvnet_amd/geometry/coords/search/search_results.py
--- a/warpconvnet_amd/geometry/coords/search/search_results.py
+++ b/warpconvnet_amd/geometry/coords/search/search_results.py
@@ -72,6 +72,7 @@
         self._mask: Optional[Tensor] = None
         self._perm: Optional[Tensor] = None
         self._offsets_dev: Optional[Tensor] = None
+        self._wgrad_bounds: Optional[Tensor] = None
         self._symmetric: bool = False
         self._self_exact: bool = False
         self._has_duplicates: bool = False
diff --git a/warpconvnet_amd/geometry/coords/search/torch_discrete.py b/warpconvnet_amd/geometry/coords/search/torch_discrete.py
--- a/warpconvnet_amd/geometry/coords/search/torch_discrete.py
+++ b/warpconvnet_amd/geometry/coords/search/torch_discrete.py
@@ -388,6 +388,8 @@
         else:
             result._nbr = b["nbr"]
         result._offsets_dev = b["meta"][: K + 1]
+        bo = L.wcn_kmap_slab_bounds_offset(M, K) if use_binned else 0
+        result._wgrad_bounds = b["block_counts"][bo : bo + 17 * K] if use_binned else None
         result._hashtable = b["table"]
         result._keepalive = b
 
diff --git a/warpconvnet_amd/nn/functional/sparse_conv/block.py b/warpconvnet_amd/nn/functional/sparse_conv/block.py
--- a/warpconvnet_amd/nn/functional/sparse_conv/block.py
+++ b/warpconvnet_amd/nn/functional/sparse_conv/block.py
@@ -105,12 +105,16 @@
             ws_bytes = hip_gemm._wgrad_workspace(K, cin, cout, _lib.WCN_ALGO_MFMA)
             wws = torch.empty(ws_bytes, dtype=torch.uint8, device=dev)
         bws = bn_workspace(cout, dev)
-        _lib.check(L.wcn_conv_bn_backward_ld(
-            _lib.ptr(g), g_ld, _lib.ptr(x), _lib.ptr(y), _lib.ptr(z) if masked else None, int(plan.relu), stats.data_ptr(), _lib.ptr(gamma),
-            int(plan.bn[0]), sums.data_ptr(), _lib.ptr(dyc), _lib.ptr(dres), _lib.ptr(wpd), _lib.ptr(tbl), _lib.ptr(msk),
-            _lib.ptr(perm), int(flip), _lib.ptr(dx), _lib.ptr(km.in_maps_device) if need_dw else None,
-            _lib.ptr(km.out_maps_device) if need_dw else None, _lib.ptr(km._offsets_dev) if need_dw else None, _lib.ptr(dw),
-            _lib.ptr(wws), ws_bytes, plan.num_in, M, cin, cout, K, code, _lib.ptr(bws), bws.numel(), stream), "wcn_conv_bn_backward_ld")
+        bounds = hip_gemm._team_bounds(km, K) if need_dw else None
+        head = (_lib.ptr(g), g_ld, _lib.ptr(x), _lib.ptr(y), _lib.ptr(z) if masked else None, int(plan.relu), stats.data_ptr(),
+                _lib.ptr(gamma), int(plan.bn[0]), sums.data_ptr(), _lib.ptr(dyc), _lib.ptr(dres), _lib.ptr(wpd), _lib.ptr(tbl),
+                _lib.ptr(msk), _lib.ptr(perm), int(flip), _lib.ptr(dx), _lib.ptr(km.in_maps_device) if need_dw else None,
+                _lib.ptr(km.out_maps_device) if need_dw else None, _lib.ptr(km._offsets_dev) if need_dw else None)
+        tail = (_lib.ptr(dw), _lib.ptr(wws), ws_bytes, plan.num_in, M, cin, cout, K, code, _lib.ptr(bws), bws.numel(), stream)
+        if bounds is not None:
+            _lib.check(L.wcn_conv_bn_backward_teams(*head, _lib.ptr(bounds), *tail), "wcn_conv_bn_backward_teams")
+        else:
+            _lib.check(L.wcn_conv_bn_backward_ld(*head, *tail), "wcn_conv_bn_backward_ld")
         if need_dres and not masked:
             dres = g
         if dw is not None and dw.dtype != w.dtype:
diff --git a/warpconvnet_amd/nn/functional/sparse_conv/detail/hip_gemm.py b/warpconvnet_amd/nn/functional/sparse_conv/detail/hip_gemm.py
--- a/warpconvnet_amd/nn/functional/sparse_conv/detail/hip_gemm.py
+++ b/warpconvnet_amd/nn/functional/sparse_conv/detail/hip_gemm.py
@@ -1,4 +1,5 @@
 import functools
+import os
 from typing import Optional, Tuple
 
 import torch
@@ -375,6 +376,18 @@
     return (dw, db) if want_bias_grad else dw
 
 
+def _team_bounds(kernel_map: IntSearchResult, K: int) -> Optional[Tensor]:
+    bounds = kernel_map._wgrad_bounds
+    if bounds is None or K != 27:
+        return None
+    mode = os.environ.get("WARPCONVNET_AMD_WGRAD_TEAMS") or "auto"
+    if mode == "force":
+        return bounds
+    if mode != "auto" or int(kernel_map.offsets[-1]) < 512 * 512:
+        return None
+    return bounds
+
+
 def _wgrad_launch(x: Tensor, dy: Tensor, kernel_map: IntSearchResult, K: int, cin: int, cout: int, code: int,
                   out: Optional[Tensor], want_bias_grad: bool):
     dev = x.device
@@ -387,6 +400,17 @@
     fuse = (want_bias_grad and code == _lib.WCN_ALGO_MFMA and kernel_map._self_exact
             and x.shape[0] == dy.shape[0] and dy.shape[0] > 0
             and _wgrad_bias_ok(cin, cout, _lib.dtype_code(x.dtype)))
+    bounds = _team_bounds(kernel_map, K) if code == _lib.WCN_ALGO_MFMA else None
+    if bounds is not None:
+        db = torch.empty(cout, dtype=torch.float32, device=dev) if fuse else None
+        _lib.check(
+            L.wcn_conv_wgrad_teams(_lib.ptr(x), _lib.ptr(dy), _lib.ptr(dw), _lib.ptr(kernel_map.in_maps_device),
+                                   _lib.ptr(kernel_map.out_maps_device), _lib.ptr(kernel_map._offsets_dev), _lib.ptr(bounds),
+                                   x.shape[0], dy.shape[0], cin, cout, K, _lib.dtype_code(x.dtype), K // 2, _lib.ptr(db),
+                                   _lib.ptr(ws), ws_bytes, _lib.stream_handle(dev)),
+            "wcn_conv_wgrad_teams",
+        )
+        return dw, db
     if fuse:
         db = torch.empty(cout, dtype=torch.float32, device=dev)
         _lib.check(
```

New measurement: 1174 M voxels/s, median of 6. 1.06x the previous value.
